# SamArgt/AudioSourceSep

Measured on AMD Instinct MI355X. Metric: Glow fwd+logdet passes/sec on 64×64×1 mel tiles (K=32,L=3), 1→8 MI355X, higher is better.
Workload: dtype f16x3

## Files before the change

__graft_entry__.py:

```python
import os
import subprocess
import sys

ROOT = os.path.dirname(os.path.abspath(__file__))
CSRC = os.path.join(ROOT, "audiosourcesep_amd", "csrc")
LIB = os.path.join(ROOT, "audiosourcesep_amd", "libglowk.so")


def _newer(target, sources):
    if not os.path.exists(target):
        return False
    t = os.path.getmtime(target)
    return all(os.path.getmtime(s) <= t for s in sources)


NET_SHAPES = [(ci, nf) for nf in (16, 12, 8, 4) for ci in (2, 4, 8, 16)]


def build(force=False, extra_flags=(), tag=None):
    from concurrent.futures import ThreadPoolExecutor
    hdr = os.path.join(ROOT, "include", "glowk.h")
    net_src = [os.path.join(CSRC, f) for f in ("glowk_act_scale.h", "glowk_kernels.h", "glowk_co.h", "glowk_q.h", "glowk_launch.h",
                                                "glowk_net_inst.hip")]
    eng_src = [os.path.join(CSRC, f) for f in sorted(os.listdir(CSRC)) if f.endswith((".hip", ".h")) and f != "glowk_net_inst.hip"] + [hdr]
    hipcc = os.environ.get("HIPCC", "/opt/rocm/bin/hipcc")
    objdir = os.path.join(CSRC, "_obj" + ("_" + tag if tag else ""))
    lib = LIB if not tag else LIB.replace("libglowk.so", "libglowk_%s.so" % tag)
    os.makedirs(objdir, exist_ok=True)
    flags = ["--offload-arch=gfx950", "-O3", "-std=c++17", "-fno-slp-vectorize", "-fPIC", "-pthread", "-Wno-unused-value"] + list(extra_flags)
    jobs, objs = [], []
    for unit in ("glowk", "glowk_training", "glowk_aux"):
        o = os.path.join(objdir, unit + ".o")
        objs.append(o)
        if force or not _newer(o, eng_src):
            jobs.append([hipcc] + flags + ["-c", os.path.join(CSRC, unit + ".hip"), "-o", o])
    for ci, nf in NET_SHAPES:
        o = os.path.join(objdir, "net_%d_%d.o" % (ci, nf))
        objs.append(o)
        if force or not _newer(o, net_src):
            jobs.append([hipcc] + flags + ["-DGLOWK_INST_CI=%d" % ci, "-DGLOWK_INST_NF=%d" % nf, "-c",
                                           os.path.join(CSRC, "glowk_net_inst.hip"), "-o", o])
    if jobs:
        workers = max(1, min(len(jobs), len(os.sched_getaffinity(0))))
        with ThreadPoolExecutor(workers) as pool:
            for r in pool.map(lambda c: subprocess.run(c, cwd=CSRC, capture_output=True, text=True), jobs):
                if r.returncode != 0:
                    sys.stderr.write(r.stderr)
                    raise RuntimeError("hipcc failed: " + " ".join(r.args[-4:]))
                if r.stderr.strip():
                    sys.stderr.write(r.stderr)
    if jobs or not _newer(lib, objs):
        subprocess.run([hipcc, "--offload-arch=gfx950", "-shared", "-fPIC", "-pthread"] + objs + ["-o", lib], check=True, cwd=CSRC)
    if tag:
        return lib
    if ROOT not in sys.path:
        sys.path.insert(0, ROOT)
    import audiosourcesep_amd
    from audiosourcesep_amd import _lib
    _lib.load()


def smoke():
    if ROOT not in sys.path:
        sys.path.insert(0, ROOT)
    import numpy as np
    import torch
    from audiosourcesep_amd.config import GlowConfig
    from audiosourcesep_amd.synthetic import calibrated_engine, synthetic_mel_tiles
    from oracle import glowref

    cfg = GlowConfig(H=16, W=16, C=1, L=2, K=2, F=128)
    eng, params = calibrated_engine(cfg, device=0)
    x = synthetic_mel_tiles(3, cfg)
    lp = eng.log_prob(torch.from_numpy(x).cuda()).cpu().numpy()
    ref = glowref.log_prob(x.astype(np.float64), glowref.cast_params(params, np.float64), cfg.as_dict())
    rel = np.max(np.abs(lp - ref) / np.abs(ref))
    print("smoke: log_prob", lp, "oracle", ref, "max rel err %.3e" % rel)
    assert rel < 1e-4, rel


if __name__ == "__main__":
    build()
    if len(sys.argv) > 1 and sys.argv[1] == "smoke":
        smoke()
```

audiosourcesep_amd/_lib.py:

```python
import ctypes
import os

_HERE = os.path.dirname(os.path.abspath(__file__))
LIB_PATH = os.environ.get("GLOWK_LIB") or os.path.join(_HERE, "libglowk.so")


class GlowkLibraryMissing(RuntimeError):
    pass


class GlowkError(RuntimeError):
    pass


class GlowkRangeError(GlowkError):
    """GLOWK_ERR_RANGE: a call in a split arithmetic (f16x3 / f16x2) left the fp16 range; its outputs are not usable."""


class GlowkConfigStruct(ctypes.Structure):
    _fields_ = [
        ("H", ctypes.c_int32), ("W", ctypes.c_int32), ("C", ctypes.c_int32),
        ("L", ctypes.c_int32), ("K", ctypes.c_int32), ("F", ctypes.c_int32),
        ("learntop", ctypes.c_int32), ("use_logit", ctypes.c_int32),
        ("minval", ctypes.c_float), ("maxval", ctypes.c_float), ("alpha", ctypes.c_float),
        ("bn_eps", ctypes.c_float),
    ]


class GlowkProfile(ctypes.Structure):
    _fields_ = [("net_ms", ctypes.c_double * 4), ("net_launches", ctypes.c_int64 * 4)]


STEP_TENSOR_IDS = {
    "actnorm/log_scale": 0, "actnorm/shift": 1,
    "inv1x1/P": 2, "inv1x1/sign_S": 3, "inv1x1/L": 4, "inv1x1/log_S": 5, "inv1x1/U": 6,
    "nn/conv1/kernel": 7, "nn/conv1/bias": 8,
    "nn/bn1/gamma": 9, "nn/bn1/beta": 10, "nn/bn1/mean": 11, "nn/bn1/var": 12,
    "nn/conv2/kernel": 13, "nn/conv2/bias": 14,
    "nn/bn2/gamma": 15, "nn/bn2/beta": 16, "nn/bn2/mean": 17, "nn/bn2/var": 18,
    "nn/conv3/kernel": 19, "nn/conv3/bias": 20,
    "inv1x1/P_inv": 21,
}
PRIOR_TENSOR_IDS = {"prior/loc": 100, "prior/log_scale": 101}
PREC_F32, PREC_F16X3, PREC_F16X2 = 0, 1, 2
OK, ERR, ERR_RANGE = 0, 1, 2
RANGE_IGNORE, RANGE_ERROR, RANGE_FALLBACK = 0, 1, 2
MIX_DB, MIX_MEAN = 0, 1

_vp, _i, _fp = ctypes.c_void_p, ctypes.c_int, ctypes.POINTER(ctypes.c_float)

SYMBOLS = {
    "glowk_version": (_i, []),
    "glowk_last_error": (ctypes.c_char_p, []),
    "glowk_reload_env": (None, []),
    "glowk_create": (_i, [ctypes.POINTER(GlowkConfigStruct), _i, ctypes.POINTER(_vp)]),
    "glowk_destroy": (_i, [_vp]),
    "glowk_tensor_size": (ctypes.c_size_t, [_vp, _i, _i]),
    "glowk_set_tensor": (_i, [_vp, _i, _i, _i, _fp, ctypes.c_size_t]),
    "glowk_get_tensor": (_i, [_vp, _i, _i, _i, _fp, ctypes.c_size_t]),
    "glowk_finalize_weights": (_i, [_vp]),
    "glowk_actnorm_data_init": (_i, [_vp, _vp, _i, _i, _i, _vp]),
    "glowk_set_precision": (_i, [_vp, _i]),
    "glowk_get_precision": (_i, [_vp]),
    "glowk_set_range_policy": (_i, [_vp, _i]),
    "glowk_get_range_policy": (_i, [_vp]),
    "glowk_range_status": (_i, [_vp, ctypes.POINTER(_i), ctypes.POINTER(ctypes.c_int64), _vp]),
    "glowk_range_probe_begin": (_i, [_vp]),
    "glowk_range_probe_end": (_i, [_vp, ctypes.POINTER(ctypes.c_float), ctypes.POINTER(ctypes.c_float), _vp]),
    "glowk_workspace_bytes": (ctypes.c_size_t, [_vp, _i, _i]),
    "glowk_reserve": (_i, [_vp, _i, _i]),
    "glowk_max_tiles": (_i, [_vp]),
    "glowk_forward": (_i, [_vp, _vp, _i, _vp, _vp, _vp]),
    "glowk_inverse": (_i, [_vp, _vp, _i, _vp, _vp]),
    "glowk_log_prob": (_i, [_vp, _vp, _i, _vp, _vp, _vp]),
    "glowk_log_prob_sum": (_i, [_vp, _vp, _i, _vp, _vp, _vp, _i, _vp]),
    "glowk_sum_f64": (_i, [_vp, ctypes.c_size_t, _vp, _i, ctypes.c_double, _vp]),
    "glowk_log_prob_grad": (_i, [_vp, _vp, _i, _vp, _vp, _vp]),
    "glowk_sample": (_i, [_vp, _vp, _i, _vp, _vp]),
    "glowk_prior_log_prob": (_i, [_vp, _vp, _i, _vp, _vp]),
    "glowk_fused_steps": (ctypes.c_int64, [_vp]),
    "glowk_kernel_families": (_i, [_vp, ctypes.POINTER(ctypes.c_int64)]),
    "glowk_profile_begin": (_i, [_vp]),
    "glowk_profile_end": (_i, [_vp, ctypes.POINTER(GlowkProfile)]),
    "glowk_squeeze": (_i, [_vp, _i, _i, _i, _i, _vp, _vp]),
    "glowk_unsqueeze": (_i, [_vp, _i, _i, _i, _i, _vp, _vp]),
    "glowk_preprocess_forward": (_i, [_vp, _vp, _i, _vp, _vp, _vp]),
    "glowk_preprocess_inverse": (_i, [_vp, _vp, _i, _vp, _vp]),
    "glowk_step_forward": (_i, [_vp, _i, _i, _vp, _i, _vp, _vp, _vp]),
    "glowk_step_inverse": (_i, [_vp, _i, _i, _vp, _i, _vp, _vp]),
    "glowk_coupling_net": (_i, [_vp, _i, _i, _vp, _i, _vp, _vp, _vp]),
    "glowk_param_vector_size": (ctypes.c_size_t, [_vp]),
    "glowk_param_offset": (_i, [_vp, _i, _i, _i, ctypes.POINTER(ctypes.c_size_t), ctypes.POINTER(ctypes.c_size_t)]),
    "glowk_param_grad": (_i, [_vp, _vp, _i, ctypes.c_float, _vp, _vp, _vp]),
    "glowk_apply_gradients": (_i, [_vp, _vp, _i, ctypes.c_float, _vp]),
    "glowk_crc32c": (ctypes.c_uint32, [_vp, ctypes.c_size_t]),
    "glowk_basis_update": (_i, [_vp, _vp, _vp, _vp, _vp, ctypes.c_size_t, ctypes.c_float, ctypes.c_float, _vp, _vp,
                                ctypes.c_uint64, ctypes.c_uint64, ctypes.c_uint64, _vp, _vp]),
    "glowk_basis_mix": (_i, [_vp, _vp, _vp, ctypes.c_size_t, _vp]),
    "glowk_basis_update_n": (_i, [_vp, _vp, _vp, _i, _vp, ctypes.c_size_t, _i, ctypes.c_float, ctypes.c_float,
                                  ctypes.c_uint64, ctypes.c_uint64, ctypes.c_uint64, _vp, _vp]),
    "glowk_basis_mix_n": (_i, [_vp, _i, _vp, ctypes.c_size_t, _i, _vp]),
    "glowk_random_source": (_i, [_vp, ctypes.c_size_t, ctypes.c_uint64, ctypes.c_uint64, _i, _i, _i, ctypes.c_uint64, _vp]),
    "glowk_random": (_i, [_vp, ctypes.c_size_t, ctypes.c_uint64, ctypes.c_uint64, _i, _i, ctypes.c_uint64, _vp]),
    "glowk_add_noise": (_i, [_vp, _vp, ctypes.c_size_t, ctypes.c_float, ctypes.c_uint64, ctypes.c_uint64, _i, ctypes.c_uint64, _vp]),
    "glowk_mel_filterbank": (_i, [_fp]),
    "glowk_mel_frontend": (_i, [_vp, _i, _i, ctypes.c_float, _vp, _vp, _vp]),
    "glowk_mel_to_power": (_i, [_vp, _i, _i, _i, _vp, _vp]),
    "glowk_masked_istft": (_i, [_vp, _i, _vp, _i, _i, _i, _vp, _vp]),
    "glowk_griffinlim": (_i, [_vp, _vp, _i, _i, _i, ctypes.c_float, _vp, _vp]),
    "glowk_resample_length": (ctypes.c_int64, [ctypes.c_int64, _i, _i]),
    "glowk_resample_filter": (_i, [ctypes.POINTER(ctypes.c_double)]),
    "glowk_resample": (_i, [_vp, _i, ctypes.c_int64, _i, _i, _vp, _vp]),
    "glowk_bss_xcorr":(_i, [_vp, _i, ctypes.c_int64, _vp, _i, ctypes.c_int64, _vp, _i, _i, _vp, _vp]),
    "glowk_bss_solve": (_i, [_vp, _i, _i, _i, _i, _i, _vp, _i, _vp, _vp, _vp]),
    "glowk_bss_project": (_i, [_vp, ctypes.c_int64, _i, _i, _i, _vp, _i, ctypes.c_int64, _vp, _i, _vp, _i, _vp, _vp]),
    "glowk_sp_stft": (_i, [_vp, _i, ctypes.c_int64, _vp, _vp]),
    "glowk_sp_istft": (_i, [_vp, _i, _i, ctypes.c_int64, _vp, _vp]),
    "glowk_oracle_mask": (_i, [_vp, _i, _i, _i, _i, ctypes.c_double, ctypes.c_double, _vp, _vp]),
    "glowk_mwf": (_i, [_vp, _i, _i, _vp]),
    "glowk_oracle_mel": (_i, [_vp, _vp, _i, ctypes.c_int64, _i, _i, ctypes.c_double, _vp, _vp]),
    "glowk_mwf_em": (_i, [_vp, _vp, _i, _i, _i, _i, _vp, _vp, _vp]),
}

_lib = None


def load():
    global _lib
    if _lib is not None:
        return _lib
    if not os.path.exists(LIB_PATH):
        raise GlowkLibraryMissing(
            "HIP library %s not found: build it first (python -c 'import __graft_entry__ as g; g.build()'). "
            "There is no CPU fallback for the compute path." % LIB_PATH)
    import torch
    lib = ctypes.CDLL(LIB_PATH)
    for name, (res, args) in SYMBOLS.items():
        fn = getattr(lib, name)
        fn.restype = res
        fn.argtypes = args
    _lib = lib
    return lib


def check(rc):
    if rc != 0:
        msg = load().glowk_last_error()
        raise (GlowkRangeError if rc == ERR_RANGE else GlowkError)(msg.decode() if msg else "glowk error %d" % rc)
```

audiosourcesep_amd/csrc/glowk.hip:

```cpp
#include "glowk_engine.h"
#include "glowk_light.h"

namespace glowk_eng {
thread_local std::string g_err;
}
using namespace glowk_eng;

namespace glowk_eng {

}

namespace glowk_detail {
int num_cus() {
  static int n = 0;
  if (n == 0) {
    int dev = 0; hipDeviceProp_t prop;
    if (hipGetDevice(&dev) == hipSuccess && hipGetDeviceProperties(&prop, dev) == hipSuccess) n = prop.multiProcessorCount;
    if (n <= 0) n = 256;
  }
  return n;
}
void launch_fail(const std::string& m) { fail(m); }
static EnvSwitches read_env() {
  auto on = [](const char* n) { return getenv(n) != nullptr; };
  return EnvSwitches{on("GLOWK_BWD_LIGHT_4"), on("GLOWK_NO_FUSE"), on("GLOWK_WGRAD_PLAIN"), on("GLOWK_CO_OFF"), on("GLOWK_Q_OFF"), on("GLOWK_CO_TRAIN_OFF"),
                     on("GLOWK_TRAIN_RECOMPUTE"), on("GLOWK_TRAIN_PERSTEP"), on("GLOWK_PG_JOIN")};
}
static EnvSwitches g_env = read_env();
const EnvSwitches& env() { return g_env; }
void reload_env() { g_env = read_env(); }
#define GLOWK_EXTERN_NET(CI_, NF_) extern template NetLaunch launch_net_t<CI_, NF_>(const NetArgs&, NetCall, hipStream_t, bool);
GLOWK_NET_SHAPES(GLOWK_EXTERN_NET)
#undef GLOWK_EXTERN_NET
}

namespace glowk_eng {
using glowk_detail::num_cus;
using glowk_detail::launch_net_t;

NetCall net_call(const glowk_handle* h, int dir, bool store, bool split) {
  if (h->precision == GLOWK_PREC_F32 || !split) return NetCall{dir, NET_EXACT, store};
  return NetCall{dir, h->precision == GLOWK_PREC_F16X2 && dir == NET_FWD && !store ? NET_SPLIT2 : NET_SPLIT3, store};
}

int* flagp(const glowk_handle* h) { return h->precision == GLOWK_PREC_F32 ? nullptr : h->d_flag; }

float bwd_norm_target(float xlim_b) {
  if (!(xlim_b >= 0.125f)) return 0.0f;
  int e = 0;
  std::frexp(xlim_b * 0.5f, &e);
  return std::ldexp(1.0f, std::min(e - 1, 10));
}

NetLaunch launch_net_raw(int c, int F, const NetArgs& a, NetCall call, hipStream_t s, bool dry) {
#define NETCASE(CI_, NF_) if (c == 2 * CI_ && F == 32 * NF_) return launch_net_t<CI_, NF_>(a, call, s, dry);
  GLOWK_NET_SHAPES(NETCASE)
#undef NETCASE
  return glowk_detail::net_failed("unsupported (channels, n_filters) combination: c=" + std::to_string(c) + " F=" + std::to_string(F));
}

int launch_net(glowk_handle* h, int level, int c, int F, const NetArgs& a, hipStream_t s, NetCall call, NetLaunch* out = nullptr) {
  if (h->profiling) {
    while (h->ev_pool.size() < h->ev_used + 2) {
      OwnedEvent e;
      HIPCHK(event_create(e, hipEventDefault));
      h->ev_pool.push_back(std::move(e));
    }
    HIPCHK(hipEventRecord(h->ev_pool[h->ev_used], s));
  }
  const NetLaunch r = launch_net_raw(c, F, a, call, s);
  if (!r.failed) {
    ++h->family_launches[r.family];
    if (r.co) ++h->family_launches[FAM_CO];
    if (r.q) ++h->family_launches[FAM_Q];
  }
  if (h->profiling) {
    HIPCHK(hipEventRecord(h->ev_pool[h->ev_used + 1], s));
    h->ev_used += 2;
    h->ev_level.push_back(level);
  }
  if (out) *out = r;
  return r.failed ? 1 : 0;
}


int launch_bwd_light(int c, const BwdArgs& a, int N, hipStream_t s) {
  const bool wide = c >= 8 && (a.Q + 15) / 16 <= 8 * num_cus() && !glowk_detail::env().bwd_light_4;
  auto al16 = [](const void* p) { return (reinterpret_cast<uintptr_t>(p) & 15) == 0; };
  const bool one = (a.Q + 255) / 256 >= 2 * num_cus() && al16(a.ghalf_in) && al16(a.v) && al16(a.osave) && al16(a.g_o) && al16(a.ghalf_out) &&
                   al16(a.gu_out) && al16(a.gv_out) && !glowk_detail::env().bwd_light_4;
  if (one) { CDISPATCH(c, hipLaunchKernelGGL((k_bwd_light<CC, 1>), dim3((a.Q + 255) / 256), dim3(256), 0, s, a)); }
  else if (wide) { CDISPATCH(c, hipLaunchKernelGGL((k_bwd_light<CC, 16>), dim3((a.Q + 15) / 16), dim3(256), 0, s, a)); }
  else { CDISPATCH(c, hipLaunchKernelGGL((k_bwd_light<CC, 4>), dim3((a.Q + 63) / 64), dim3(256), 0, s, a)); }
  LAUNCHCHK("k_bwd_light");
  return 0;
}

struct FlatLd { double* slot; int stride, base; };

int launch_couple(int c, const CoupleArgs& a, int N, hipStream_t s, const FlatLd* fl = nullptr, bool* flat_used = nullptr) {
  const int hw = a.h * a.w;
  if (N < 2 * num_cus() && hw % 64 == 0 && (!a.logdet || (fl && fl->slot))) {
    CoupleArgs b = a;
    b.logdet = nullptr;
    double* slots = a.logdet ? fl->slot : (double*)nullptr;
    const bool wide = c >= 8 && (a.Q + 15) / 16 <= 8 * num_cus();
    if (wide) { CDISPATCH(c, hipLaunchKernelGGL((k_couple_flat<CC, 16>), dim3((a.Q + 15) / 16), dim3(256), 0, s, b, slots, fl ? fl->stride : 0, fl ? fl->base : 0)); }
    else { CDISPATCH(c, hipLaunchKernelGGL((k_couple_flat<CC, 4>), dim3((a.Q + 63) / 64), dim3(256), 0, s, b, slots, fl ? fl->stride : 0, fl ? fl->base : 0)); }
    LAUNCHCHK("k_couple_flat");
    if (flat_used && a.logdet) *flat_used = true;
    return 0;
  }
  if (N >= 2 * num_cus()) {
    CDISPATCH(c, hipLaunchKernelGGL((k_couple<CC, false>), dim3(N), dim3(256), 0, s, a));
  } else {
    const int threads = hw >= 256 ? 1024 : hw > 64 ? 512 : 256;
    CDISPATCH(c, hipLaunchKernelGGL((k_couple<CC, true>), dim3(N), dim3(threads), 0, s, a));
  }
  LAUNCHCHK("k_couple");
  return 0;
}

bool fuse_geometry_ok(int h, int w, int pxw = 256) {
  const int hw = h * w;
  if (w < 4 || w > FUSE_EW || (w & (w - 1)) || pxw % w) return false;
  if (hw % pxw == 0) return true;
  return hw >= 32 && hw < pxw && (hw & (hw - 1)) == 0;
}

int net_and_couple(glowk_handle* h, int lvl, int c, int F, NetArgs na, CoupleArgs ca, int N, hipStream_t s, NetCall call, const FlatLd* fl = nullptr,
                   bool* flat_used = nullptr) {
  const bool no_fuse = glowk_detail::env().no_fuse;
  const bool fusable = call.arith != NET_EXACT && call.dir != NET_BWD && !call.store;
  const int hw = ca.h * ca.w;
  if (!no_fuse && c == 4 && fusable && na.RSp && ca.vin && !ca.log_s_out && ca.out && na.in_stride == 4 &&
      ca.out_stride % 4 == 0 && ca.out_off % 4 == 0 && fuse_geometry_ok(ca.h, ca.w) && na.P == h->bufP) {
    const size_t pxw = (na.co && fuse_geometry_ok(ca.h, ca.w, CO_PX)) ? CO_PX : 256;
    if (pxw == 256) na.co = 0;
    const size_t wgs = ((size_t)ca.Q + pxw - 1) / pxw;
    const size_t edge_floats = (wgs * 4 * FUSE_EW * 4 + 3) & ~(size_t)3;
    const size_t nld = wgs * (pxw / 32);
    if ((edge_floats + 2 * nld + 4) <= 4 * h->pstride) {
      na.fuse = 1;
      na.fz_b3 = ca.b3; na.fz_A = ca.A; na.fz_b = ca.b; na.fz_out = ca.out; na.fz_out_stride = ca.out_stride; na.fz_out_off = ca.out_off;
      na.fz_inverse = ca.inverse;
      na.fz_osave = ca.o_save;
      na.fz_edge = h->bufP;
      na.fz_ldpart = ca.logdet ? reinterpret_cast<double*>(h->bufP + edge_floats) : nullptr;
    }
  }
  NetLaunch r;
  if (int rc = launch_net(h, lvl, c, F, na, s, call, &r)) return rc;
  if (!r.fused_px) {
    ca.P = na.P; ca.np = r.np; ca.pstride = na.pstride;
    return launch_couple(c, ca, N, s, fl, flat_used);
  }
  ++h->fused_steps;
  const int pxw = r.fused_px;
  if (hw > pxw || ca.logdet) {
    EdgeArgs ea;
    ea.vin = ca.vin; ea.edge = na.fz_edge; ea.ldpart = na.fz_ldpart; ea.A = ca.A; ea.b = ca.b; ea.out = ca.out; ea.out_stride = ca.out_stride;
    ea.out_off = ca.out_off; ea.inverse = ca.inverse; ea.logdet = ca.logdet; ea.osave = ca.o_save; ea.h = ca.h; ea.w = ca.w; ea.flag = ca.flag; ea.pxw = pxw;
    hipLaunchKernelGGL(k_couple_edge, dim3(N), dim3(256), 0, s, ea);
    LAUNCHCHK("k_couple_edge");
  }
  return 0;
}

PreArgs pre_args(const glowk_config& cfg) {
  PreArgs p;
  p.minval = cfg.minval; p.maxval = cfg.maxval; p.alpha = cfg.alpha; p.use_logit = cfg.use_logit;
  return p;
}

struct WsSizes {
  size_t act, P, ld;
  size_t slots;
  size_t total() const { return 3 * act + P + ld + slots; }
};
int ld_slots_per_sample(const glowk_handle* h) {
  int n = 0;
  for (const Level& lv : h->levels) n += h->cfg.K * ((lv.h * lv.w + 15) / 16);
  return n;
}
WsSizes ws_sizes(const glowk_handle* h, size_t N) {
  const size_t E = (size_t)h->cfg.H * h->cfg.W * h->cfg.C;
  return WsSizes{N * E * 4, 4 * 9 * N * E * 4, N * 8, std::min(N, (size_t)2 * num_cus()) * ld_slots_per_sample(h) * 8};
}
size_t mask_blocks(const Level& lv, size_t Q) {
  const size_t b256 = ((Q + 255) / 256) * 8;
  if (lv.c == 32) return ((Q + 127) / 128) * 8;
  const size_t Qh = (size_t)256 * (size_t)(num_cus() / 8);
  return std::max(b256, ((std::min(Q, Qh) + 127) / 128) * 8);
}

struct SaveSizes {
  size_t v, p, m;
  int np;
  size_t gz, c;
  size_t total() const { return v * 4 + (size_t)np * p * 4 + m * 2 + gz + c; }
};
SaveSizes save_sizes(const glowk_handle* h, size_t N, std::vector<size_t>* offV = nullptr, std::vector<size_t>* offP = nullptr,
                     std::vector<size_t>* offM = nullptr) {
  const int K = h->cfg.K, L = h->cfg.L, NF = h->cfg.F / 32;
  SaveSizes S{0, 0, 0, 1, 0, 0};
  if (offV) { offV->assign((size_t)L * K, 0); offP->assign((size_t)L * K, 0); offM->assign((size_t)L * K, 0); }
  for (int lvl = 0; lvl < L; ++lvl) {
    const Level& lv = h->levels[lvl];
    const size_t Q = N * lv.h * lv.w;
    const size_t blocks = mask_blocks(lv, Q);
    for (int j = 0; j < K; ++j) {
      const size_t sidx = (size_t)lvl * K + j;
      if (offV) { (*offV)[sidx] = S.v; (*offP)[sidx] = S.p; (*offM)[sidx] = S.m; }
      S.v += Q * lv.c;
      S.p += Q * (lv.c / 2);
      S.m += 2 * blocks * NF * 64;
    }
  }
  const size_t E = (size_t)h->cfg.H * h->cfg.W * h->cfg.C;
  S.gz = N * E * 4;
  S.c = N * E * 4;
  return S;
}

int ensure_flag(glowk_handle* h) {
  if (h->d_flag) return 0;
  DeviceMem<int> d_flag;
  PinnedMem<int> h_flag;
  HIPCHK(dev_alloc(d_flag, 16));
  HIPCHK(hipMemset(d_flag, 0, 16));
  HIPCHK(pinned_alloc(h_flag, 16));
  h_flag[0] = 0;
  h->d_flag = std::move(d_flag);
  h->h_flag = std::move(h_flag);
  return 0;
}

int ensure_ws(glowk_handle* h, int N) {
  if (int rc = ensure_flag(h)) return rc;
  if (N <= h->wsN) return 0;
  HIPCHK(hipDeviceSynchronize());
  h->bufA.reset(); h->bufB.reset(); h->bufP.reset(); h->bufZ.reset(); h->bufLd.reset(); h->bufLdSlot.reset(); h->wsN = 0;
  const WsSizes W = ws_sizes(h, (size_t)N);
  HIPCHK(dev_alloc(h->bufA, W.act));
  HIPCHK(dev_alloc(h->bufB, W.act));
  h->pstride = W.P / 16;
  HIPCHK(dev_alloc(h->bufP, W.P));
  HIPCHK(dev_alloc(h->bufZ, W.act));
  HIPCHK(dev_alloc(h->bufLd, W.ld));
  HIPCHK(dev_alloc(h->bufLdSlot, W.slots));
  h->wsN = N;
  return 0;
}

int ensure_c(glowk_handle* h, int N) {
  if ((size_t)N <= h->cN) return 0;
  HIPCHK(hipDeviceSynchronize());
  h->bufC.reset(); h->cN = 0;
  HIPCHK(dev_alloc(h->bufC, (size_t)N * h->cfg.H * h->cfg.W * h->cfg.C * 4));
  h->cN = (size_t)N;
  return 0;
}

int max_tiles(const glowk_handle* h) {
  const long long E = (long long)h->cfg.H * h->cfg.W * h->cfg.C;
  const long long m = (1LL << 28) / E;
  return m < 1 ? 1 : (int)m;
}


int check_batch(const glowk_handle* h, int N) {
  if (N <= 0) return fail("batch size must be positive");
  if (N > max_tiles(h)) return fail("batch of " + std::to_string(N) + " tiles exceeds glowk_max_tiles() = " + std::to_string(max_tiles(h)) +
                                    " (32-bit indices within one call): split the batch");
  return 0;
}

int check_ready(glowk_handle* h, int N) {
  if (!h) return fail("null handle");
  if (h->finalized && h->split_stale && h->precision != GLOWK_PREC_F32)
    if (int rc = glowk_finalize_weights(h)) return rc;
  if (!h->finalized) return fail("glowk_finalize_weights has not been called");
  if (int rc = check_batch(h, N)) return rc;
  return ensure_ws(h, N);
}

NetArgs net_args(glowk_handle* h, const Level& lv, const StepDev& sd, const float* vin, int in_stride, int in_off, int N) {
  NetArgs a;
  a.vin = vin; a.in_stride = in_stride; a.in_off = in_off;
  a.Q = N * lv.h * lv.w; a.h = lv.h; a.w = lv.w;
  a.K1p = sd.K1p; a.ep = sd.ep; a.R0p = sd.R0p; a.mask1 = nullptr; a.mask2 = nullptr; a.P = h->bufP;
  a.RHp = sd.RHp; a.RSp = sd.RSp; a.fam16 = (sd.RSp && sd.RSBp) ? 1 : 0; a.eph = sd.epH; a.pstride = h->pstride; a.max_np = 4; a.sc1 = sd.sc1; a.sc2 = sd.sc2; a.sc3 = sd.sc3;
  a.flag = flagp(h); a.xlim = sd.xlim_f; a.st1 = nullptr; a.st2 = nullptr;
  a.bnorm = 1.0f;
  a.fuse = 0; a.co = glowk_detail::env().co_off ? 0 : 1; a.fz_osave = nullptr; a.fz_b3 = nullptr; a.fz_A = nullptr; a.fz_b = nullptr; a.fz_out = nullptr; a.fz_out_stride = 0; a.fz_out_off = 0; a.fz_inverse = 0;
  a.fz_edge = nullptr; a.fz_ldpart = nullptr;
  a.pad = nullptr;
  a.xmax_out = h->d_probe ? h->d_probe + ((&lv - h->levels.data()) * h->cfg.K + (&sd - lv.dev.data())) : nullptr;
  return a;
}

int ensure_save(glowk_handle* h, int N) {
  if (int rc = ensure_c(h, N)) return rc;
  if (N <= h->saveN) return 0;
  const int Na = std::max(N, h->saveN);
// ... 602 lines not shown
  std::vector<float> v((size_t)2 * LK);
  HIPCHK(hipStreamSynchronize((hipStream_t)stream));
  HIPCHK(hipMemcpy(v.data(), h->d_probe, v.size() * sizeof(float), hipMemcpyDeviceToHost));
  h->d_probe.reset();
  float rf = 0.f, rb = 0.f;
  for (int l = 0; l < h->cfg.L; ++l)
    for (int k = 0; k < h->cfg.K; ++k) {
      const StepDev& sd = h->levels[l].dev[k];
      const int i = l * h->cfg.K + k;
      if (sd.xlim_f > 0.f) rf = std::max(rf, v[i] / sd.xlim_f);
      if (sd.xlim_b > 0.f && v[LK + i] > 0.f) rb = std::max(rb, 0.125f / sd.xlim_b);
    }
  if (fwd_ratio) *fwd_ratio = rf;
  if (bwd_ratio) *bwd_ratio = rb;
  return 0;
}

size_t glowk_workspace_bytes(const glowk_handle* h, int N, int with_grad) {
  if (!h || N <= 0) return 0;
  size_t b = ws_sizes(h, (size_t)N).total() + 16 ;
  if (with_grad) b += save_sizes(h, (size_t)N).total();
  return b;
}

int glowk_max_tiles(const glowk_handle* h) { return h ? max_tiles(h) : 0; }

int glowk_reserve(glowk_handle* h, int N, int with_grad) {
  if (!h) return fail("null handle");
  DeviceGuard dg(h->device);
  if (int rc = check_batch(h, N)) return rc;
  if (int rc = ensure_ws(h, N)) return rc;
  if (with_grad) {
    if (!h->finalized) return fail("glowk_finalize_weights must run before reserving the gradient path (its size depends on the launch policy)");
    return ensure_save(h, N);
  }
  return 0;
}

int glowk_forward(glowk_handle* h, const float* x_dev, int N, float* z_dev, float* logdet_dev, void* stream) {
  if (!h) return fail("null handle");
  DeviceGuard dg(h->device);
  if (int rc = check_ready(h, N)) return rc;
  if (!x_dev || !z_dev) return fail("null tensor");
  hipStream_t s = (hipStream_t)stream;
  return guarded(h, s, [&]() -> int {
    if (int rc = run_forward(h, x_dev, N, z_dev, s)) return rc;
    if (logdet_dev) {
      hipLaunchKernelGGL(k_prior, dim3(N), dim3(256), 0, s, (const float*)nullptr, 0, (const float*)nullptr, (const float*)nullptr,
                         (const double*)h->bufLd, (float*)nullptr, logdet_dev);
      LAUNCHCHK("k_prior(logdet)");
    }
    return 0;
  });
}

int glowk_inverse(glowk_handle* h, const float* z_dev, int N, float* x_dev, void* stream) {
  if (!h) return fail("null handle");
  DeviceGuard dg(h->device);
  if (int rc = check_ready(h, N)) return rc;
  if (!x_dev || !z_dev) return fail("null tensor");
  hipStream_t s = (hipStream_t)stream;
  return guarded(h, s, [&]() -> int { return run_inverse(h, z_dev, N, x_dev, s); });
}

int glowk_log_prob(glowk_handle* h, const float* x_dev, int N, float* logp_dev, float* z_dev, void* stream) {
  if (!h) return fail("null handle");
  DeviceGuard dg(h->device);
  if (int rc = check_ready(h, N)) return rc;
  if (!x_dev || !logp_dev) return fail("null tensor");
  hipStream_t s = (hipStream_t)stream;
  float* z = z_dev ? z_dev : h->bufZ;
  return guarded(h, s, [&]() -> int {
    if (int rc = run_forward(h, x_dev, N, z, s)) return rc;
    hipLaunchKernelGGL(k_prior, dim3(N), dim3(256), 0, s, (const float*)z, h->Hl * h->Wl * h->Cl, h->d_loc, h->d_log_scale,
                       (const double*)h->bufLd, logp_dev, (float*)nullptr);
    LAUNCHCHK("k_prior");
    return 0;
  });
}

int glowk_log_prob_sum(glowk_handle* h, const float* x_dev, int N, float* logp_dev, float* z_dev, double* sum_dev, int accumulate, void* stream) {
  if (!h) return fail("null handle");
  DeviceGuard dg(h->device);
  if (int rc = check_ready(h, N)) return rc;
  if (!x_dev || !logp_dev || !sum_dev) return fail("null tensor");
  hipStream_t s = (hipStream_t)stream;
  float* z = z_dev ? z_dev : h->bufZ;
  const int rc = guarded(h, s, [&]() -> int {
    if (int rc = run_forward(h, x_dev, N, z, s)) return rc;
    hipLaunchKernelGGL(k_prior, dim3(N), dim3(256), 0, s, (const float*)z, h->Hl * h->Wl * h->Cl, h->d_loc, h->d_log_scale,
                       (const double*)h->bufLd, logp_dev, (float*)nullptr);
    LAUNCHCHK("k_prior");
    return 0;
  });
  if (rc) return rc;
  hipLaunchKernelGGL(k_sum_f64, dim3(1), dim3(1024), 0, s, (const float*)logp_dev, (size_t)N, sum_dev, accumulate, 1.0);
  LAUNCHCHK("k_sum_f64");
  return 0;
}

int glowk_sum_f64(const float* v_dev, size_t n, double* out_dev, int accumulate, double scale, void* stream) {
  if (!out_dev || (!v_dev && n)) return fail("null tensor");
  DeviceGuard dg(ptr_device(out_dev));
  hipLaunchKernelGGL(k_sum_f64, dim3(1), dim3(1024), 0, (hipStream_t)stream, v_dev, n, out_dev, accumulate, scale);
  LAUNCHCHK("k_sum_f64");
  return 0;
}

int glowk_log_prob_grad(glowk_handle* h, const float* x_dev, int N, float* logp_dev, float* dx_dev, void* stream) {
  if (!h) return fail("null handle");
  DeviceGuard dg(h->device);
  if (int rc = check_ready(h, N)) return rc;
  if (!x_dev || !logp_dev || !dx_dev) return fail("null tensor");
  if (int rc = ensure_save(h, N)) return rc;
  hipStream_t s = (hipStream_t)stream;
  float* z = h->bufGz;
  return guarded(h, s, [&]() -> int {
    if (int rc = run_forward(h, x_dev, N, z, s, true)) return rc;
    hipLaunchKernelGGL(k_prior, dim3(N), dim3(256), 0, s, (const float*)z, h->Hl * h->Wl * h->Cl, h->d_loc, h->d_log_scale,
                       (const double*)h->bufLd, logp_dev, (float*)nullptr);
    LAUNCHCHK("k_prior");
    return run_backward(h, x_dev, z, N, dx_dev, s);
  });
}

int glowk_sample(glowk_handle* h, const float* eps_dev, int N, float* x_dev, void* stream) {
  if (!h) return fail("null handle");
  DeviceGuard dg(h->device);
  if (int rc = check_ready(h, N)) return rc;
  if (!eps_dev || !x_dev) return fail("null tensor");
  hipStream_t s = (hipStream_t)stream;
  const int E = h->Hl * h->Wl * h->Cl;
  const size_t total = (size_t)N * E;
  return guarded(h, s, [&]() -> int {
    hipLaunchKernelGGL(k_prior_sample, dim3((unsigned)((total + 255) / 256)), dim3(256), 0, s, eps_dev, total, E, h->d_loc, h->d_log_scale,
                       h->bufZ);
    LAUNCHCHK("k_prior_sample");
    return run_inverse(h, h->bufZ, N, x_dev, s);
  });
}

int glowk_prior_log_prob(glowk_handle* h, const float* z_dev, int N, float* logp_dev, void* stream) {
  if (!h) return fail("null handle");
  DeviceGuard dg(h->device);
  if (int rc = check_ready(h, N)) return rc;
  if (!z_dev || !logp_dev) return fail("null tensor");
  hipLaunchKernelGGL(k_prior, dim3(N), dim3(256), 0, (hipStream_t)stream, z_dev, h->Hl * h->Wl * h->Cl, h->d_loc, h->d_log_scale,
                     (const double*)nullptr, logp_dev, (float*)nullptr);
  LAUNCHCHK("k_prior");
  return 0;
}

int64_t glowk_fused_steps(const glowk_handle* h) { return h ? h->fused_steps : -1; }

int glowk_kernel_families(const glowk_handle* h, int64_t* out7) {
  if (!h || !out7) return fail("null argument");
  for (int i = 0; i < FAM_COUNT; ++i) out7[i] = h->family_launches[i];
  return 0;
}

int glowk_profile_begin(glowk_handle* h) {
  if (!h) return fail("null handle");
  h->profiling = true;
  h->ev_used = 0;
  h->ev_level.clear();
  return 0;
}

int glowk_profile_end(glowk_handle* h, glowk_profile* out) {
  if (!h || !out) return fail("null argument");
  std::memset(out, 0, sizeof(*out));
  h->profiling = false;
  DeviceGuard dg(h->device);
  HIPCHK(hipDeviceSynchronize());
  for (size_t i = 0; i < h->ev_level.size(); ++i) {
    float ms = 0.0f;
    HIPCHK(hipEventElapsedTime(&ms, h->ev_pool[2 * i], h->ev_pool[2 * i + 1]));
    const int l = h->ev_level[i];
    if (l >= 0 && l < 4) { out->net_ms[l] += ms; out->net_launches[l] += 1; }
  }
  h->ev_used = 0;
  h->ev_level.clear();
  return 0;
}

int glowk_squeeze(const float* x_dev, int N, int H, int W, int C, float* y_dev, void* stream) {
  if (!x_dev || !y_dev) return fail("null tensor");
  if (N <= 0 || H <= 0 || W <= 0 || H % 2 || W % 2) return fail("squeeze needs even H and W");
  if ((long long)N * H * W * C > (1LL << 28)) return fail("squeeze: more than 2^28 elements in one call; split the batch");
  DeviceGuard dg(ptr_device(x_dev));
  PreArgs p = {0, 1, 0, 0};
  const int c = 4 * C;
  CDISPATCH(c, hipLaunchKernelGGL((k_in<CC>), dim3(N), dim3(256), 0, (hipStream_t)stream, x_dev, H, W, p, 0, (const float*)nullptr,
                                  (const float*)nullptr, y_dev, (double*)nullptr, 0.0));
  LAUNCHCHK("k_in(squeeze)");
  return 0;
}

int glowk_unsqueeze(const float* y_dev, int N, int hh, int ww, int c4, float* x_dev, void* stream) {
  if (!x_dev || !y_dev) return fail("null tensor");
  if (N <= 0 || hh <= 0 || ww <= 0 || c4 % 4) return fail("unsqueeze needs a channel count divisible by 4");
  if ((long long)N * hh * ww * c4 > (1LL << 28)) return fail("unsqueeze: more than 2^28 elements in one call; split the batch");
  DeviceGuard dg(ptr_device(y_dev));
  PreArgs p = {0, 1, 0, 0};
  CDISPATCH(c4, hipLaunchKernelGGL((k_out<CC>), dim3(N), dim3(256), 0, (hipStream_t)stream, y_dev, hh, ww, p, 0, x_dev));
  LAUNCHCHK("k_out(unsqueeze)");
  return 0;
}

int glowk_preprocess_forward(glowk_handle* h, const float* x_dev, int N, float* y_dev, float* logdet_dev, void* stream) {
  if (!h || !x_dev || !y_dev) return fail("null argument");
  DeviceGuard dg(h->device);
  if (int rc = check_batch(h, N)) return rc;
  const int E = h->cfg.H * h->cfg.W * h->cfg.C;
  double ldc = -(double)E * std::log((double)h->cfg.maxval - (double)h->cfg.minval);
  if (h->cfg.use_logit) ldc += (double)E * std::log(1.0 - 2.0 * (double)h->cfg.alpha);
  hipLaunchKernelGGL(k_pre_only, dim3(N), dim3(256), 0, (hipStream_t)stream, x_dev, E, pre_args(h->cfg), 0, y_dev, logdet_dev, ldc);
  LAUNCHCHK("k_pre_only");
  return 0;
}

int glowk_preprocess_inverse(glowk_handle* h, const float* y_dev, int N, float* x_dev, void* stream) {
  if (!h || !x_dev || !y_dev) return fail("null argument");
  DeviceGuard dg(h->device);
  if (int rc = check_batch(h, N)) return rc;
  const int E = h->cfg.H * h->cfg.W * h->cfg.C;
  hipLaunchKernelGGL(k_pre_only, dim3(N), dim3(256), 0, (hipStream_t)stream, y_dev, E, pre_args(h->cfg), 1, x_dev, (float*)nullptr, 0.0);
  LAUNCHCHK("k_pre_only");
  return 0;
}

int glowk_step_forward(glowk_handle* h, int level, int step, const float* u_dev, int N, float* y_dev, float* logdet_dev, void* stream) {
  if (!h) return fail("null handle");
  DeviceGuard dg(h->device);
  if (int rc = check_ready(h, N)) return rc;
  if (level < 0 || level >= h->cfg.L || step < 0 || step >= h->cfg.K) return fail("no such step");
  if (!u_dev || !y_dev) return fail("null tensor");
  hipStream_t s = (hipStream_t)stream;
  const Level& lv = h->levels[level];
  const StepDev& sd = lv.dev[step];
  const int Q = N * lv.h * lv.w;
  return guarded(h, s, [&]() -> int {
    CDISPATCH(lv.c, hipLaunchKernelGGL((k_affine<CC>), dim3((Q + 255) / 256), dim3(256), 0, s, u_dev, Q, sd.Afwd, sd.bfwd, h->bufA));
    LAUNCHCHK("k_affine");
    NetLaunch r;
    if (int rc = launch_net(h, level, lv.c, h->cfg.F, net_args(h, lv, sd, h->bufA, lv.c, lv.c / 2, N), s, net_call(h, NET_FWD), &r)) return rc;
    if (logdet_dev) {
      std::vector<double> init(N, h->ld_step[(size_t)level * h->cfg.K + step]);
      HIPCHK(hipMemcpyAsync(h->bufLd, init.data(), (size_t)N * 8, hipMemcpyHostToDevice, s));
      HIPCHK(hipStreamSynchronize(s));
    }
    CoupleArgs ca;
    ca.o_save = nullptr;
    ca.vin = h->bufA; ca.P = h->bufP; ca.np = r.np; ca.pstride = h->pstride; ca.b3 = sd.b3; ca.A = nullptr; ca.b = nullptr;
    ca.out = y_dev; ca.out_stride = lv.c; ca.out_off = 0;
    ca.logdet = logdet_dev ? h->bufLd : nullptr; ca.log_s_out = nullptr; ca.t_out = nullptr;
    ca.Q = Q; ca.h = lv.h; ca.w = lv.w; ca.inverse = 0; ca.flag = flagp(h);
    if (int rc = launch_couple(lv.c, ca, N, s)) return rc;
    if (logdet_dev) {
      hipLaunchKernelGGL(k_prior, dim3(N), dim3(256), 0, s, (const float*)nullptr, 0, (const float*)nullptr, (const float*)nullptr,
                         (const double*)h->bufLd, (float*)nullptr, logdet_dev);
      LAUNCHCHK("k_prior(logdet)");
    }
    return 0;
  });
}

int glowk_step_inverse(glowk_handle* h, int level, int step, const float* y_dev, int N, float* u_dev, void* stream) {
  if (!h) return fail("null handle");
  DeviceGuard dg(h->device);
  if (int rc = check_ready(h, N)) return rc;
  if (level < 0 || level >= h->cfg.L || step < 0 || step >= h->cfg.K) return fail("no such step");
  if (!u_dev || !y_dev) return fail("null tensor");
  hipStream_t s = (hipStream_t)stream;
  const Level& lv = h->levels[level];
  const StepDev& sd = lv.dev[step];
  return guarded(h, s, [&]() -> int {
    NetLaunch r;
    if (int rc = launch_net(h, level, lv.c, h->cfg.F, net_args(h, lv, sd, y_dev, lv.c, lv.c / 2, N), s, net_call(h, NET_FWD), &r)) return rc;
    CoupleArgs ca;
    ca.o_save = nullptr;
    ca.vin = y_dev; ca.P = h->bufP; ca.np = r.np; ca.pstride = h->pstride; ca.b3 = sd.b3; ca.A = sd.Ainv; ca.b = sd.binv;
    ca.out = u_dev; ca.out_stride = lv.c; ca.out_off = 0;
    ca.logdet = nullptr; ca.log_s_out = nullptr; ca.t_out = nullptr;
    ca.Q = N * lv.h * lv.w; ca.h = lv.h; ca.w = lv.w; ca.inverse = 1; ca.flag = flagp(h);
    return launch_couple(lv.c, ca, N, s);
  });
}

int glowk_coupling_net(glowk_handle* h, int level, int step, const float* xb_dev, int N, float* log_s_dev, float* t_dev, void* stream) {
  if (!h) return fail("null handle");
  DeviceGuard dg(h->device);
  if (int rc = check_ready(h, N)) return rc;
  if (level < 0 || level >= h->cfg.L || step < 0 || step >= h->cfg.K) return fail("no such step");
  if (!xb_dev || !log_s_dev || !t_dev) return fail("null tensor");
  hipStream_t s = (hipStream_t)stream;
  const Level& lv = h->levels[level];
  const StepDev& sd = lv.dev[step];
  return guarded(h, s, [&]() -> int {
    NetLaunch r;
    if (int rc = launch_net(h, level, lv.c, h->cfg.F, net_args(h, lv, sd, xb_dev, lv.c / 2, 0, N), s, net_call(h, NET_FWD), &r)) return rc;
    CoupleArgs ca;
    ca.o_save = nullptr;
    ca.vin = nullptr; ca.P = h->bufP; ca.np = r.np; ca.pstride = h->pstride; ca.b3 = sd.b3; ca.A = nullptr; ca.b = nullptr;
    ca.out = nullptr; ca.out_stride = 0; ca.out_off = 0;
    ca.logdet = nullptr; ca.log_s_out = log_s_dev; ca.t_out = t_dev;
// ... 8 lines not shown
```

audiosourcesep_amd/csrc/glowk_engine.h:

```cpp
#pragma once
#include "../../include/glowk.h"
#include "glowk_kernels.h"
#include "glowk_pack.h"
#include "glowk_launch.h"

#include <algorithm>
#include <atomic>
#include <cmath>
#include <cstdio>
#include <cstdlib>
#include <cstring>
#include <sched.h>
#include <string>
#include <thread>
#include <vector>

namespace glowk_eng {

extern thread_local std::string g_err;

inline int fail(const std::string& m) {
  g_err = m;
  return GLOWK_ERR;
}

struct DeviceGuard {
  int prev = -1;
  bool changed = false;
  explicit DeviceGuard(int dev) {
    if (hipGetDevice(&prev) == hipSuccess && prev != dev) changed = hipSetDevice(dev) == hipSuccess;
  }
  ~DeviceGuard() {
    if (changed) (void)hipSetDevice(prev);
  }
  DeviceGuard(const DeviceGuard&) = delete;
  DeviceGuard& operator=(const DeviceGuard&) = delete;
};

#define HIPCHK(expr)                                                                           \
  do {                                                                                         \
    hipError_t e_ = (expr);                                                                    \
    if (e_ != hipSuccess) return glowk_eng::fail(std::string(#expr) + ": " + hipGetErrorString(e_));      \
  } while (0)

#define LAUNCHCHK(name)                                                                        \
  do {                                                                                         \
    hipError_t e_ = hipGetLastError();                                                         \
    if (e_ != hipSuccess) return glowk_eng::fail(std::string("launch ") + name + ": " + hipGetErrorString(e_)); \
  } while (0)

template <class T, class Release>
class Owner {
 public:
  Owner() = default;
  explicit Owner(Release r) : r_(r) {}
  Owner(Owner&& o) noexcept : p_(o.release()), r_(o.r_) {}
  Owner& operator=(Owner&& o) noexcept { reset(o.release()); r_ = o.r_; return *this; }
  ~Owner() { reset(); }
  operator T() const { return p_; }
  const Release& releaser() const { return r_; }
  T release() { T p = p_; p_ = nullptr; return p; }
  void reset(T p = nullptr) { if (p_) r_(p_); p_ = p; }
 private:
  T p_ = nullptr;
  Release r_{};
};
struct HipFree { void operator()(void* p) const { (void)hipFree(p); } };
struct HipHostFree { void operator()(void* p) const { (void)hipHostFree(p); } };
struct HipFreeAsync { hipStream_t s; void operator()(void* p) const { (void)hipFreeAsync(p, s); } };
struct HipStreamDestroy { void operator()(hipStream_t s) const { (void)hipStreamDestroy(s); } };
struct HipEventDestroy { void operator()(hipEvent_t e) const { (void)hipEventDestroy(e); } };
template <class T> using DeviceMem = Owner<T*, HipFree>;
template <class T> using PinnedMem = Owner<T*, HipHostFree>;
template <class T> using Scratch = Owner<T*, HipFreeAsync>;
using OwnedStream = Owner<hipStream_t, HipStreamDestroy>;
using OwnedEvent = Owner<hipEvent_t, HipEventDestroy>;

template <class T, class R, class Create>
hipError_t create_into(Owner<T, R>& o, Create create) {
  o.reset();
  T p = nullptr;
  const hipError_t e = create(&p);
  if (e == hipSuccess) o.reset(p);
  return e;
}
template <class T> hipError_t dev_alloc(DeviceMem<T>& o, size_t bytes) { return create_into(o, [&](T** p) { return hipMalloc(p, bytes); }); }
template <class T> hipError_t pinned_alloc(PinnedMem<T>& o, size_t bytes) { return create_into(o, [&](T** p) { return hipHostMalloc(p, bytes); }); }
template <class T> hipError_t scratch_alloc(Scratch<T>& o, size_t bytes) {
  return create_into(o, [&](T** p) { return hipMallocAsync(reinterpret_cast<void**>(p), bytes, o.releaser().s); });
}
inline hipError_t stream_create(OwnedStream& o) { return create_into(o, [](hipStream_t* s) { return hipStreamCreateWithFlags(s, hipStreamNonBlocking); }); }
inline hipError_t event_create(OwnedEvent& o, unsigned flags) { return create_into(o, [&](hipEvent_t* e) { return hipEventCreateWithFlags(e, flags); }); }

}
using glowk_eng::DeviceMem; using glowk_eng::PinnedMem; using glowk_eng::OwnedStream; using glowk_eng::OwnedEvent;

struct glowk_handle {
  glowk_config cfg;
  int device = 0;
  int precision = GLOWK_PREC_F32;
  int range_policy = GLOWK_RANGE_ERROR;
  int64_t range_fallbacks = 0;
  int64_t family_launches[FAM_COUNT] = {};
  int64_t fused_steps = 0;
  DeviceMem<int> d_flag;
  PinnedMem<int> h_flag;
  DeviceMem<unsigned> d_probe;
  std::vector<Level> levels;
  int Hl = 0, Wl = 0, Cl = 0;
  std::vector<float> prior_loc, prior_log_scale;
  bool finalized = false;
  double ld_const = 0.0;
  double ld_pre_const = 0.0;
  std::vector<double> ld_step;
  DeviceMem<float> arena;
  const float* d_loc = nullptr;
  const float* d_log_scale = nullptr;
  int wsN = 0;
  DeviceMem<float> bufA, bufB, bufP, bufZ, bufC;
  size_t pstride = 0;
  DeviceMem<double> bufLd;
  DeviceMem<double> bufLdSlot;
  DeviceMem<double> bufStat;
  int saveN = 0;
  size_t cN = 0;
  DeviceMem<float> saveV, saveP, bufGz;
  DeviceMem<unsigned short> saveM;
  std::vector<size_t> offV, offP, offM;
  bool tr_active = false;
  bool host_stale = false;
  bool split_stale = false;
  DeviceMem<float> tr_params, tr_m, tr_v;
  size_t tr_n = 0;
  long tr_t = 0;
  std::vector<size_t> tr_level_off;
  size_t tr_prior_off = 0;
  std::vector<DeviceMem<int>> tr_map;
  std::vector<size_t> tr_map_n;
  std::vector<DeviceMem<int>> tr_map16;
  std::vector<size_t> tr_map16_n;
  DeviceMem<float> tr16_src;
  DeviceMem<int> tr16_S;
  DeviceMem<float> tr16_scales;
  size_t tr16_src_max = 0;
  PinnedMem<float> tr_pinned;
  std::vector<size_t> tr_pin_off;
  std::vector<OwnedStream> tr_streams;
  std::vector<OwnedEvent> tr_events;
  std::vector<float> tr_bfac;
  DeviceMem<unsigned> tr_gmax;
  PinnedMem<float> h_gmax;
  OwnedStream tr_side;
  OwnedEvent tr_ev_sums, tr_ev_up;
  PinnedMem<double> h_sums;
  PinnedMem<float> h_up;
  int trN = 0;
  DeviceMem<float> trR1, trM1, trM2, trXcol, trGcol, trCpart, trC1, trC2, trC3, trGv, trGo;
  int trNB = 1;
  DeviceMem<double> trAffPart, trAffSum;
  DeviceMem<float> trKeep;
  std::vector<size_t> trKeepOff;
  int trKeepN = 0;
  bool profiling = false;
  std::vector<OwnedEvent> ev_pool;
  size_t ev_used = 0;
  std::vector<int> ev_level;
};

#define CDISPATCH(c, CALL)                                                                     \
  switch (c) {                                                                                 \
    case 4: { constexpr int CC = 4; CALL; } break;                                             \
    case 8: { constexpr int CC = 8; CALL; } break;                                             \
    case 16: { constexpr int CC = 16; CALL; } break;                                           \
    case 32: { constexpr int CC = 32; CALL; } break;                                           \
    default: return glowk_eng::fail("unsupported channel count " + std::to_string(c));         \
  }

namespace glowk_eng {

struct TrainCtx {
  float* grad;
  float scale;
  bool split;
  hipEvent_t sums_ready = nullptr;
};

int check_ready(glowk_handle* h, int N);
int ensure_save(glowk_handle* h, int N);
NetArgs net_args(glowk_handle* h, const Level& lv, const StepDev& sd, const float* vin, int in_stride, int in_off, int N);
NetCall net_call(const glowk_handle* h, int dir, bool store = false, bool split = true);
NetLaunch launch_net_raw(int c, int F, const NetArgs& a, NetCall call, hipStream_t s, bool dry = false);
int run_forward(glowk_handle* h, const float* x, int N, float* z_dst, hipStream_t s, bool save = false, bool keep_hidden = false);
int run_backward(glowk_handle* h, const float* x, const float* z, int N, float* dx, hipStream_t s, TrainCtx* tc = nullptr);
int launch_prior(glowk_handle* h, const float* z, int N, float* logp_dev, hipStream_t s);
int ptr_device(const void* p);

int sync_host(glowk_handle* h);
int train_network_grads(glowk_handle* h, TrainCtx* tc, int lvl, int k0, int nb, const float* v, ptrdiff_t v_bs, const float* g_o, ptrdiff_t go_bs,
                        const float* R1, ptrdiff_t r_bs, const float* M1, const float* M2, ptrdiff_t m_bs, int N, hipStream_t s, float bfac = 1.0f);
int train_affine_sums(glowk_handle* h, int lvl, int k0, int nb, const float* v, ptrdiff_t v_bs, const float* gv, ptrdiff_t gv_bs, int N, hipStream_t s);

}
```

audiosourcesep_amd/csrc/glowk_kernels.h:

```cpp
#pragma once
#include "glowk_act_scale.h"

#include <hip/hip_runtime.h>
#include <utility>
#include <stdint.h>

typedef float f32x16 __attribute__((ext_vector_type(16)));

#define GLOWK_GPTR(p) ((const __attribute__((address_space(1))) void*)(p))
#define GLOWK_LPTR(p) ((__attribute__((address_space(3))) void*)(p))

__device__ __forceinline__ int mfma_row(int r, int hh) { return (r & 3) + 8 * (r >> 2) + 4 * hh; }

struct NetArgs {
  const float* vin;
  int in_stride, in_off;
  int Q, h, w;
  const float* K1p;
  const float* ep;
  const float4* R0p;
  unsigned short* mask1;
  unsigned short* mask2;
  float* P;
  size_t pstride;
  int max_np;
  const float4* RHp;
  const float* eph;
  const float4* RSp;
  int fam16;
  float sc1, sc2, sc3;
  int* flag;
  float xlim;
  float bnorm;
  int fuse;
  int co;
  const float* fz_b3;
  const float* fz_A;
  const float* fz_b;
  float* fz_out;
  int fz_out_stride, fz_out_off, fz_inverse;
  float* fz_osave;
  float* fz_edge;
  double* fz_ldpart;
  unsigned* xmax_out;
  float* st1;
  float* st2;
  void* pad;
};

#define GLOWK_ST_MOD " nt"
__device__ __forceinline__ void st_tile_planar(float* blk_base, unsigned lane_byte, unsigned row_bytes, const f32x16& v) {
  const unsigned long long base = reinterpret_cast<unsigned long long>(blk_base);
  unsigned off = lane_byte;
#pragma unroll
  for (int r = 0; r < 16; ++r) {
    asm volatile("global_store_dword %0, %1, %2" GLOWK_ST_MOD ::"v"(off), "v"(v[r]), "s"(base) : "memory");
    off += ((r & 3) == 3 ? 5u : 1u) * row_bytes;
  }
}

template <int C>
__device__ __forceinline__ void affine_cc(const float* __restrict__ A, const float* __restrict__ b, const float (&x)[C], float (&y)[C]) {
#pragma unroll
  for (int co = 0; co < C; ++co) y[co] = b[co];
#pragma unroll
  for (int ci = 0; ci < C; ++ci)
#pragma unroll
    for (int co = 0; co < C; ++co) y[co] = fmaf(x[ci], A[ci * C + co], y[co]);
}

__device__ __forceinline__ void glds16(const float4* src_lane, float4* lds_wave_base) {
  __builtin_amdgcn_global_load_lds(GLOWK_GPTR(src_lane), GLOWK_LPTR(lds_wave_base), 16, 0, 0);
}

__device__ __forceinline__ float* uniform_fptr(float* p) {
  const unsigned long long b = reinterpret_cast<unsigned long long>(p);
  const unsigned lo = __builtin_amdgcn_readfirstlane((unsigned)b);
  const unsigned hi = __builtin_amdgcn_readfirstlane((unsigned)(b >> 32));
  return reinterpret_cast<float*>(((unsigned long long)hi << 32) | lo);
}
__device__ __forceinline__ const char* uniform_ptr(const void* p) {
  const unsigned long long b = reinterpret_cast<unsigned long long>(p);
  const unsigned lo = __builtin_amdgcn_readfirstlane((unsigned)b);
  const unsigned hi = __builtin_amdgcn_readfirstlane((unsigned)(b >> 32));
  return reinterpret_cast<const char*>(((unsigned long long)hi << 32) | lo);
}

template <int P>
__device__ __forceinline__ float4* ring_slot(float4* s0, float4* s1) { return P ? s1 : s0; }

template <int KIN, int NF>
struct Ring1 {
  static constexpr int KS1 = (9 * KIN) / 2;
  static constexpr int MAIN4 = NF * 256;
  static constexpr int K1PIECES_FULL = (KS1 * 256 + 1023) / 1024;
  static constexpr bool K1_IN_RING = (size_t)2 * (MAIN4 + K1PIECES_FULL * 64) * 16 + (size_t)6 * NF * 32 * 4 <= 160 * 1024;
  static constexpr int K1PIECES = K1_IN_RING ? K1PIECES_FULL : 0;
  static constexpr bool K1_IN_BUF = !K1_IN_RING && (size_t)2 * MAIN4 * 16 + (size_t)6 * NF * 32 * 4 + (size_t)K1PIECES_FULL * 1024 <= 160 * 1024;
  static constexpr int K1HALF_KS = KS1 / 2;
  static constexpr int K1HALF_PIECES = (K1HALF_KS * 256 + 1023) / 1024;
  static constexpr bool K1_IN_HALF = !K1_IN_RING && !K1_IN_BUF && KS1 % 2 == 0 && (K1HALF_KS * 256) % 1024 == 0 &&
                                     (size_t)2 * MAIN4 * 16 + (size_t)6 * NF * 32 * 4 + (size_t)K1HALF_PIECES * 1024 <= 160 * 1024;
  static constexpr int K1BUF4 = K1_IN_BUF ? K1PIECES_FULL * 64 : K1_IN_HALF ? K1HALF_PIECES * 64 : 1;
  static constexpr int SLOT4 = MAIN4 + K1PIECES * 64;
  static constexpr int PIECES = NF * 4 + K1PIECES;
  static constexpr size_t LDS_BYTES = (size_t)2 * SLOT4 * 16 + (size_t)6 * NF * 32 * 4 + ((K1_IN_BUF || K1_IN_HALF) ? (size_t)K1BUF4 * 16 : 0);
  static constexpr bool FITS = LDS_BYTES <= 160 * 1024;
};

template <int P0, int N>
__device__ __forceinline__ void stage_range(const float4* __restrict__ src, float4* dst, int wave, unsigned voff) {
  const char* gb = uniform_ptr(src);
#pragma unroll
  for (int i = 0; i < (N + 3) / 4; ++i) {
    int p = i * 4 + wave;
    p = P0 + (p < N ? p : N - 1);
    glds16(reinterpret_cast<const float4*>(gb + (size_t)p * 1024 + voff), dst + p * 64);
  }
}

enum { NET_FWD = 0, NET_FWD_SAVE = 1, NET_BWD = 2,
       NET_FWD2 = 3 };
constexpr int NET_STORE = 8;
constexpr int NET_FUSE = 16;
constexpr int NET_HALF = 32;
template <int MODE>
constexpr int net_dir = MODE & 7;

template <int N>
__device__ __forceinline__ unsigned pick_word(const unsigned (&w)[N], int j) {
  unsigned r = 0;
#pragma unroll
  for (int i = 0; i < N; ++i) r = (j == i) ? w[i] : r;
  return r;
}

template <int KIN, int NF, int P, int MODE, bool STORE>
__device__ __forceinline__ void net_step(const NetArgs& a, int fi, bool first, const float4* nsrc, float4* s0, float4* s1, float4* k1buf,
                                         const float* epl, const float (&xcol)[(9 * KIN) / 2], f32x16 (&acc2)[NF],
                                         const unsigned (&mk)[NF / 2], size_t wblk, int wave, unsigned voff, int lane, int hh, int q, bool qok, bool wok) {
  using G = Ring1<KIN, NF>;
  constexpr int KS1 = G::KS1;
  constexpr int F = NF * 32;
  f32x16 h1;
#pragma unroll
  for (int r = 0; r < 16; ++r) h1[r] = 0.0f;
  if constexpr (G::K1_IN_HALF) {
    constexpr int KH = G::K1HALF_KS;
    if (!first) {
      asm volatile("s_waitcnt vmcnt(0)" ::: "memory");
      __syncthreads();
    }
    const float* k1 = reinterpret_cast<const float*>(k1buf) + lane;
#pragma unroll
    for (int ks = 0; ks < KH; ++ks) h1 = __builtin_amdgcn_mfma_f32_32x32x2f32(k1[ks * 64], xcol[ks], h1, 0, 0, 0);
    __syncthreads();
    stage_range<0, G::K1HALF_PIECES>(reinterpret_cast<const float4*>(a.K1p + ((size_t)fi * KS1 + KH) * 64), k1buf, wave, voff);
    asm volatile("s_waitcnt vmcnt(0)" ::: "memory");
    __syncthreads();
#pragma unroll
    for (int ks = 0; ks < KH; ++ks) h1 = __builtin_amdgcn_mfma_f32_32x32x2f32(k1[ks * 64], xcol[KH + ks], h1, 0, 0, 0);
  } else {
    if (G::K1_IN_BUF && !first) {
      asm volatile("s_waitcnt vmcnt(0)" ::: "memory");
      __syncthreads();
    }
    const float* k1 = G::K1_IN_RING ? reinterpret_cast<const float*>(ring_slot<P ^ 1>(s0, s1) + G::MAIN4) + lane
                      : G::K1_IN_BUF ? reinterpret_cast<const float*>(k1buf) + lane
                                     : a.K1p + (size_t)fi * KS1 * 64 + lane;
#pragma unroll
    for (int ks = 0; ks < KS1; ++ks) h1 = __builtin_amdgcn_mfma_f32_32x32x2f32(k1[ks * 64], xcol[ks], h1, 0, 0, 0);
  }
  float* st_blk = STORE ? uniform_fptr(a.st1 + (size_t)fi * 32 * a.Q) : nullptr;
  const unsigned st_lane = STORE ? ((unsigned)(4 * hh) * (unsigned)a.Q + (unsigned)q) * 4u : 0u;
  const unsigned st_row = (unsigned)a.Q * 4u;
  if (MODE == NET_BWD) {
    const unsigned w = pick_word<NF / 2>(mk, fi >> 1) >> ((fi & 1) * 16);
#pragma unroll
    for (int r = 0; r < 16; ++r) h1[r] = ((w >> r) & 1u) ? h1[r] : 0.0f;
    if (STORE && qok) st_tile_planar(st_blk, st_lane, st_row, h1);
#pragma unroll
    for (int r = 0; r < 16; ++r) h1[r] *= epl[4 * F + fi * 32 + mfma_row(r, hh)];
  } else {
    unsigned bits = 0;
#pragma unroll
    for (int r = 0; r < 16; ++r) {
      const int f = fi * 32 + mfma_row(r, hh);
      const float pre = h1[r] + epl[f];
      if (MODE == NET_FWD_SAVE) bits |= (pre > 0.0f ? 1u : 0u) << r;
      h1[r] = fmaxf(pre, 0.0f);
    }
    if (STORE && qok) st_tile_planar(st_blk, st_lane, st_row, h1);
#pragma unroll
    for (int r = 0; r < 16; ++r) {
      const int f = fi * 32 + mfma_row(r, hh);
      h1[r] = fmaf(epl[F + f], h1[r], epl[2 * F + f]);
    }
    if (MODE == NET_FWD_SAVE) a.mask1[(wblk * NF + fi) * 64 + lane] = (unsigned short)bits;
  }
  {
    constexpr int NST = (STORE ? 16 : 0) + (MODE == NET_FWD_SAVE ? 1 : 0);
    if (!first || G::K1_IN_BUF) {
      if (NST && wok) asm volatile("s_waitcnt vmcnt(%0)" ::"n"(NST) : "memory");
      else asm volatile("s_waitcnt vmcnt(0)" ::: "memory");
    }
    __syncthreads();
  }
  stage_range<0, G::PIECES>(nsrc, ring_slot<P ^ 1>(s0, s1), wave, voff);
  if (G::K1_IN_BUF && fi + 1 < NF)
    stage_range<0, G::K1PIECES_FULL>(reinterpret_cast<const float4*>(a.K1p + (size_t)(fi + 1) * KS1 * 64), k1buf, wave, voff);
  if constexpr (G::K1_IN_HALF) {
    if (fi + 1 < NF) stage_range<0, G::K1HALF_PIECES>(reinterpret_cast<const float4*>(a.K1p + (size_t)(fi + 1) * KS1 * 64), k1buf, wave, voff);
  }
  const float4* buf = ring_slot<P>(s0, s1);
#pragma unroll
  for (int r = 0; r < 16; ++r) {
#pragma unroll
    for (int g = 0; g < NF / 4; ++g) {
      const float4 wv = buf[(r * (NF / 4) + g) * 64 + lane];
      acc2[4 * g + 0] = __builtin_amdgcn_mfma_f32_32x32x2f32(wv.x, h1[r], acc2[4 * g + 0], 0, 0, 0);
      acc2[4 * g + 1] = __builtin_amdgcn_mfma_f32_32x32x2f32(wv.y, h1[r], acc2[4 * g + 1], 0, 0, 0);
      acc2[4 * g + 2] = __builtin_amdgcn_mfma_f32_32x32x2f32(wv.z, h1[r], acc2[4 * g + 2], 0, 0, 0);
      acc2[4 * g + 3] = __builtin_amdgcn_mfma_f32_32x32x2f32(wv.w, h1[r], acc2[4 * g + 3], 0, 0, 0);
    }
  }
}

template <int KIN, int MOUT, int NF, int MODE, bool STORE = false>
__global__ __launch_bounds__(256, 1) void k_net_f32(NetArgs a) {
  using G = Ring1<KIN, NF>;
  constexpr int KS1 = G::KS1;
  constexpr int NMT = (MOUT + 31) / 32;
  constexpr int F = NF * 32;
  constexpr int SLOT4 = G::SLOT4;
  constexpr int SGN = (MODE == NET_BWD) ? -1 : 1;
  static_assert(KIN % 2 == 0 && NF % 4 == 0 && G::FITS, "shape");

  __shared__ float4 slot0[SLOT4];
  __shared__ float4 slot1[SLOT4];
  __shared__ float epl[6 * F];
  __shared__ float4 k1buf[G::K1BUF4];

  const int tid = threadIdx.x;
  const int lane = tid & 63;
  const int wave = __builtin_amdgcn_readfirstlane(tid >> 6);
  const unsigned voff = (unsigned)lane * 16u;
  const int pix = lane & 31;
  const int hh = lane >> 5;
  const size_t wblk = (size_t)blockIdx.x * 4 + (tid >> 6);
  const int q = (int)wblk * 32 + pix;
  const bool qok = q < a.Q;
  const bool wok = (long)(blockIdx.x * 4 + wave) * 32 < a.Q;
  const float4* ring = a.R0p;

  float xcol[KS1];
  {
    const int hw = a.h * a.w;
    const int qq = qok ? q : 0;
    const int rem = qq % hw;
    const int i = rem / a.w, j = rem % a.w;
    const float* base = a.vin + (long)qq * a.in_stride + a.in_off;
#pragma unroll
    for (int ks = 0; ks < KS1; ++ks) {
      const int k = 2 * ks + hh;
      const int tap = k / KIN, cin = k % KIN;
      const int dy = SGN * (tap / 3 - 1), dx = SGN * (tap % 3 - 1);
      const int ii = i + dy, jj = j + dx;
      const bool ok = qok && ii >= 0 && ii < a.h && jj >= 0 && jj < a.w;
      const int off = ok ? ((dy * a.w + dx) * a.in_stride + cin) : 0;
      const float v = base[off];
      xcol[ks] = ok ? v : 0.0f;
    }
  }
  unsigned mk1[NF / 2], mk2[NF / 2];
#pragma unroll
  for (int j = 0; j < NF / 2; ++j) { mk1[j] = 0; mk2[j] = 0; }
  if (MODE == NET_BWD) {
#pragma unroll
// ... 475 lines not shown
                                        const h8 (&xh)[(RingH<KIN, MOUT, NF, MODE, NP>::KS)], const h8 (&xl)[(RingH<KIN, MOUT, NF, MODE, NP>::KS)],
                                        int g, int q, bool qok, int lane, int hh) {
  using G = RingH<KIN, MOUT, NF, MODE, NP>;
  constexpr int NFH = G::NFH, NMT = G::NMT;
  constexpr int f2base = PASS * NFH * 32;
  f32x16 acc2[NFH];
#pragma unroll
  for (int fo = 0; fo < NFH; ++fo)
#pragma unroll
    for (int r = 0; r < 16; ++r) acc2[fo][r] = net_dir<MODE> == NET_BWD ? 0.0f : epl[f2base + fo * 32 + mfma_row(r, hh)];

  h8 bh[2], bl[2];
#pragma nounroll
  for (int i0 = 0; i0 < NF; i0 += 2) {
    h3_X<KIN, MOUT, NF, MODE, NP, 0, PASS>(a, c, i0, xh, xl, lane, bh, bl);
    h3_x_end<MODE, PASS>(c);
    if (PASS >= 1 && !SOLO && NMT == 1 && i0 == 0 && !g)
      stage4<G::MAINP, 50>(G::out_chunk(c.img, PASS, 0), c.sD, c.w4, c.voff);
    h3_Y<KIN, MOUT, NF, MODE, NP, 1>(P0 ? c.sB : c.sA, bh, bl, acc2, lane, g, true, G::main_chunk(c.img, PASS, i0 + 1), P0 ? c.sA : c.sB,
                                     c.k1img + (size_t)((i0 + 2) % NF) * G::K14, c.k1s0, c.w4, c.voff);
    h3_barrier();
    h3_X<KIN, MOUT, NF, MODE, NP, 1, PASS>(a, c, i0 + 1, xh, xl, lane, bh, bl);
    h3_x_end<MODE, PASS>(c);
    h3_Y<KIN, MOUT, NF, MODE, NP, 2>(P0 ? c.sA : c.sB, bh, bl, acc2, lane, g, i0 + 2 < NF || NMT >= 2,
                                     i0 + 2 < NF ? G::main_chunk(c.img, PASS, i0 + 2) : G::out_chunk(c.img, PASS, 1), P0 ? c.sB : c.sA,
                                     c.k1img + (size_t)((i0 + 3) % NF) * G::K14, c.k1s1, c.w4, c.voff);
    h3_barrier();
  }

  f32x16 acc3[G::G0N];
  h3_tail<KIN, MOUT, NF, MODE, NP, P0, PASS, SOLO>(a, c, epl, acc2, acc3, bh, bl, g, q, qok, lane, hh, std::make_integer_sequence<int, 2 * NMT>());
}

template <int KIN, int MOUT, int NF, int MODE, int NP, int PASS, int P0>
__device__ __forceinline__ void h3_passes(const NetArgs& a, const H3Ctx& c, const float* epl,
                                          const h8 (&xh)[(RingH<KIN, MOUT, NF, MODE, NP>::KS)], const h8 (&xl)[(RingH<KIN, MOUT, NF, MODE, NP>::KS)],
                                          int g, int q, bool qok, int lane, int hh) {
  h3_pass<KIN, MOUT, NF, MODE, NP, P0, PASS, false>(a, c, epl, xh, xl, g, q, qok, lane, hh);
  if constexpr (PASS + 1 < NP)
    h3_passes<KIN, MOUT, NF, MODE, NP, PASS + 1, (RingH<KIN, MOUT, NF, MODE, NP>::NMT + 1 + P0) & 1>(a, c, epl, xh, xl, g, q, qok, lane, hh);
}

template <int KIN, int MOUT, int NF, int MODE, int NP, bool SPLIT>
__global__ __launch_bounds__(512, 2) void k_net_h3(NetArgs a) {
  using G = RingH<KIN, MOUT, NF, MODE, NP>;
  constexpr int K1 = G::K1;
  constexpr int KS = G::KS;
  constexpr int SGN = (net_dir<MODE> == NET_BWD) ? -1 : 1;
  static_assert(G::FITS, "shape");

  __shared__ float4 slotA[G::MAIN4];
  __shared__ float4 slotB[G::MAIN4];
  __shared__ float4 slotD[G::MAIN4];
  __shared__ float4 k1slot0[G::K14];
  __shared__ float4 k1slot1[G::K14];
  __shared__ float epl[G::EPN];
  __shared__ __attribute__((aligned(16))) unsigned short mkl[G::MASK2B / 2 + 8];

  const int tid = threadIdx.x;
  const int lane = tid & 63;
  const int wave = __builtin_amdgcn_readfirstlane(tid >> 6);
  const int g = wave >> 2;
  const int pix = lane & 31;
  const int hh = lane >> 5;
  const int q = (blockIdx.x * 8 + (tid >> 6)) * 32 + pix;
  const bool qok = q < a.Q;

  H3Ctx c;
  c.sA = slotA; c.sB = slotB; c.sD = slotD; c.k1s0 = k1slot0; c.k1s1 = k1slot1;
  c.k1img = a.RHp;
  const int solo_pass = SPLIT ? (int)blockIdx.y : 0;
  c.img = a.RHp;
  c.mkl = mkl;
  c.wblk = (size_t)blockIdx.x * 8 + wave;
  c.wok = (long)c.wblk * 32 < a.Q;
  c.w4 = wave & 3;
  c.voff = (unsigned)lane * 16u;
  c.ub[0] = c.ub[1] = 1.0f;

  if (!g) {
    stage4<G::MAINP, 60>(G::main_chunk(c.img, solo_pass, 0), slotA, c.w4, c.voff);
    stage4<G::MAINP, 61>(G::out_chunk(c.img, solo_pass, 0), slotD, c.w4, c.voff);
    if (net_dir<MODE> == NET_BWD)
      stage4<NF, 64>(reinterpret_cast<const float4*>(a.mask1 + (size_t)blockIdx.x * 8 * NF * 64), reinterpret_cast<float4*>(mkl), c.w4, c.voff);
  } else {
    stage4<G::K1P, 62>(c.k1img, k1slot0, c.w4, c.voff);
    stage4<G::K1P, 63>(c.k1img + G::K14, k1slot1, c.w4, c.voff);
    if (net_dir<MODE> == NET_BWD)
      stage4<NF, 65>(reinterpret_cast<const float4*>(a.mask2 + (size_t)blockIdx.x * 8 * NF * 64), reinterpret_cast<float4*>(mkl + 8 * NF * 64), c.w4, c.voff);
  }
  h8 xh[KS], xl[KS];
  float xmax = 0.0f;
  {
    const int hw = a.h * a.w;
    const int qq = qok ? q : 0;
    const int rem = qq % hw;
    const int i = rem / a.w, j0 = rem % a.w;
    const float* base = a.vin + (long)qq * a.in_stride + a.in_off;
    if constexpr (net_dir<MODE> == NET_BWD) {
      float v[KS][8];
#pragma unroll
      for (int s = 0; s < KS; ++s) {
        gather8<KIN, false, SGN>(base, i, j0, a.h, a.w, a.in_stride, qok, 16 * s + 8 * hh, v[s]);
        xmax = range8(xmax, v[s]);
      }
      xmax = nan_max(xmax, __shfl_xor(xmax, 32, 64));
      const float fac = (MODE & NET_STORE) ? 1.0f : pixel_norm(xmax, a.bnorm, c.ub[0]);
#pragma unroll
      for (int s = 0; s < KS; ++s) {
#pragma unroll
        for (int j = 0; j < 8; ++j) v[s][j] *= fac;
        split8(v[s], xh[s], xl[s]);
      }
    } else {
#pragma unroll
      for (int s = 0; s < KS; ++s) {
        float v[8];
        gather8<KIN, true, SGN>(base, i, j0, a.h, a.w, a.in_stride, qok, 16 * s + 8 * hh, v);
        xmax = range8(xmax, v);
        split8(v, xh[s], xl[s]);
      }
    }
  }
  if (net_dir<MODE> != NET_BWD)
    for (int i = tid; i < G::EPN; i += 512) epl[i] = a.eph[i];
  if (((net_dir<MODE> == NET_BWD && !(MODE & NET_STORE)) ? !(xmax <= 3.0e38f) : !(xmax <= a.xlim)) && a.flag) *a.flag = 1;
  if (a.xmax_out) range_probe(a.xmax_out, xmax);
  asm volatile("s_waitcnt vmcnt(0)" ::: "memory");
  __syncthreads();

  if (g) h3_barrier();
  if constexpr (SPLIT) {
    if (solo_pass == 0) h3_pass<KIN, MOUT, NF, MODE, NP, 0, 0, true>(a, c, epl, xh, xl, g, q, qok, lane, hh);
    else if (solo_pass == 1) h3_pass<KIN, MOUT, NF, MODE, NP, 0, 1, true>(a, c, epl, xh, xl, g, q, qok, lane, hh);
    else if constexpr (NP > 2) {
      if (solo_pass == 2) h3_pass<KIN, MOUT, NF, MODE, NP, 0, 2, true>(a, c, epl, xh, xl, g, q, qok, lane, hh);
      else h3_pass<KIN, MOUT, NF, MODE, NP, 0, 3, true>(a, c, epl, xh, xl, g, q, qok, lane, hh);
    }
  } else {
    h3_passes<KIN, MOUT, NF, MODE, NP, 0, 0>(a, c, epl, xh, xl, g, q, qok, lane, hh);
  }
  if (!g) h3_barrier();
}

typedef float f32x4 __attribute__((ext_vector_type(4)));

constexpr int FUSE_PSTR = 260;
constexpr int FUSE_EW = 64;

template <int KIN, int MOUT, int NF, int MODE, int NP>
struct RingS {
  static constexpr bool BWD = net_dir<MODE> == NET_BWD;
  static constexpr bool FUSE = (MODE & NET_FUSE) != 0;
  static constexpr int PXH = (MODE & NET_HALF) ? 1 : 2;
  static constexpr int NFH = NF / NP;
  static constexpr int NRB = 2 * NFH;
  static constexpr int K1 = 9 * KIN;
  static constexpr int KS = (K1 + (BWD ? 0 : 1) + 31) / 32;
  static constexpr int MAINP = NRB * 2;
  static constexpr int MAIN4 = MAINP * 64;
  static constexpr int K1P = KS * 4;
  static constexpr int K14 = K1P * 64;
  static constexpr bool STK = !BWD && glowk_conv1_stacked(K1);
  static constexpr int KSX = STK ? glowk_conv1_ks_stacked(K1) : KS;
  static constexpr int M3 = MOUT;
  static constexpr int NMT = (M3 + 15) / 16;
  static constexpr int TPC = MAINP / 2;
  static constexpr int NT = NFH * NMT;
  static constexpr int NCH = (NT + TPC - 1) / TPC;
  static constexpr int G0N = NMT < 6 ? NMT : 6;
  static constexpr int NGRP = (NMT + 5) / 6;
  static constexpr int GT = NFH * 6;
  static constexpr int grp_n(int gi) { return NMT - 6 * gi < 6 ? NMT - 6 * gi : 6; }
  static constexpr int EPN = (NF * 32 + 16 * NMT + 3) & ~3;
  static constexpr int MASK2B = BWD ? 2 * NF * 512 * 2 : 0;
  static constexpr size_t LDS_BYTES = (size_t)3 * MAIN4 * 16 + (size_t)2 * K14 * 16 + (size_t)EPN * 4 + MASK2B;
  static constexpr bool FITS = LDS_BYTES <= 160 * 1024 && NF % 4 == 0 && NFH >= 2 && KS <= (PXH == 1 ? (NP == 2 ? 5 : 9) : NP == 2 ? 3 : 5) && NGRP <= 3 &&
                               (NGRP == 1 || GT % TPC == 0) &&
                               (!FUSE || (MOUT == 36 && NP == 2 && PXH == 2 && LDS_BYTES + (size_t)36 * FUSE_PSTR * 4 + 4096 + 128 <= 160 * 1024));
  static constexpr int K1TOT4 = NF * K14;
  static constexpr int IMGH = NF / 2;
  static constexpr int IMG_MAIN4 = IMGH * 256;
  static constexpr int IMG_NCH = (IMGH * NMT + 2 * IMGH - 1) / (2 * IMGH);
  static constexpr int IMG_PASS4 = (NF + IMG_NCH) * IMG_MAIN4;
  static constexpr int SUBS = NP / 2;
  __device__ static const float4* main_chunk(const float4* img, int pass, int ch) {
    return img + K1TOT4 + (size_t)(pass / SUBS) * IMG_PASS4 + (size_t)ch * IMG_MAIN4 + (size_t)(pass % SUBS) * MAIN4;
  }
  __device__ static const float4* out_chunk(const float4* img, int pass, int s) {
    const int sub = pass % SUBS, t4 = s * TPC;
    const int gi = t4 / GT;
    const int t2 = IMGH * 6 * gi + sub * NFH * grp_n(gi) + (t4 - GT * gi);
    return img + K1TOT4 + (size_t)(pass / SUBS) * IMG_PASS4 + (size_t)NF * IMG_MAIN4 + (size_t)t2 * 128;
  }
  static constexpr int tile_fo(int t) { return (t - GT * (t / GT)) / grp_n(t / GT); }
  static constexpr int tile_mt(int t) { return 6 * (t / GT) + (t - GT * (t / GT)) % grp_n(t / GT); }
  static constexpr bool MERGE = PXH == 2 && NP == 2 && NGRP == 1 && NMT <= 3 &&
                                (net_dir<MODE> == NET_FWD || net_dir<MODE> == NET_FWD2 || (net_dir<MODE> == NET_BWD && NMT <= 2) || (net_dir<MODE> == NET_FWD_SAVE && FUSE));
};

template <bool TWO = false>
__device__ __forceinline__ f32x4 mfma3s(const h8& ahi, const h8& alo, const h8& bhi, const h8& blo, f32x4 acc) {
  acc = __builtin_amdgcn_mfma_f32_16x16x32_f16(alo, bhi, acc, 0, 0, 0);
  if (!TWO) acc = __builtin_amdgcn_mfma_f32_16x16x32_f16(ahi, blo, acc, 0, 0, 0);
  acc = __builtin_amdgcn_mfma_f32_16x16x32_f16(ahi, bhi, acc, 0, 0, 0);
  return acc;
}

template <int MODE>
__device__ __forceinline__ unsigned h3s_act_vals(const f32x4& r0, const f32x4& r1, float sc, unsigned mask8, float (&v)[8]) {
  unsigned bits = 0;
#pragma unroll
  for (int j = 0; j < 8; j += 2) {
    const f32x2 a2 = j < 4 ? f32x2{r0[j], r0[j + 1]} : f32x2{r1[j - 4], r1[j - 3]};
    const f32x2 t2 = a2 * f32x2{sc, sc};
    const float t[2] = {t2.x, t2.y}, av[2] = {a2.x, a2.y};
#pragma unroll
    for (int e = 0; e < 2; ++e) {
      if (MODE == NET_BWD) v[j + e] = __int_as_float(__float_as_int(t[e]) & __builtin_amdgcn_sbfe((int)mask8, j + e, 1));
      else {
        v[j + e] = fmaxf(t[e], 0.0f);
        if (MODE == NET_FWD_SAVE) bits |= (av[e] > 0.0f ? 1u : 0u) << (j + e);
      }
    }
  }
  return bits;
}
template <int MODE, bool ST = false>
__device__ __forceinline__ unsigned h3s_act(const f32x4& r0, const f32x4& r1, float sc, unsigned mask8, h8& bh, h8& bl, bool do_st = false,
                                            float* st_blk = nullptr, unsigned st_lane = 0, unsigned st_row = 0) {
  float v[8];
  const unsigned bits = h3s_act_vals<MODE>(r0, r1, sc, mask8, v);
  if constexpr (ST) {
    if (do_st) {
      const unsigned long long st_base = reinterpret_cast<unsigned long long>(st_blk);
#pragma unroll
      for (int j = 0; j < 8; ++j) {
        const unsigned off = st_lane + (unsigned)((j >> 2) * 16 + (j & 3)) * st_row;
        asm volatile("global_store_dword %0, %1, %2" GLOWK_ST_MOD ::"v"(off), "v"(v[j]), "s"(st_base) : "memory");
      }
    }
  }
  if (MODE == NET_FWD2) {
#pragma unroll
    for (int j = 0; j < 8; ++j) { bh[j] = (_Float16)v[j]; bl[j] = (_Float16)0.0f; }
  } else split8(v, bh, bl);
  return bits;
}
template <int MODE, bool ST>
__device__ __forceinline__ unsigned h3s_act_pair(const f32x4& r00, const f32x4& r10, const f32x4& r01, const f32x4& r11, float sc, unsigned mask16,
                                                 h8 (&bh)[2], h8 (&bl)[2], float* st_blk, unsigned st_lane, unsigned st_row) {
  float v0[8], v1[8];
  unsigned bits = h3s_act_vals<MODE>(r00, r10, sc, mask16, v0);
  bits |= h3s_act_vals<MODE>(r01, r11, sc, mask16 >> 8, v1) << 8;
  if constexpr (ST) {
    const unsigned long long st_base = reinterpret_cast<unsigned long long>(st_blk);
#pragma unroll
    for (int j = 0; j < 8; ++j) {
      const unsigned off = st_lane + (unsigned)((j >> 2) * 16 + (j & 3)) * st_row;
      const f32x2 pr = {v0[j], v1[j]};
      asm volatile("global_store_dwordx2 %0, %1, %2" GLOWK_ST_MOD ::"v"(off), "v"(pr), "s"(st_base) : "memory");
    }
  }
  split8(v0, bh[0], bl[0]);
  split8(v1, bh[1], bl[1]);
  return bits;
}

template <int KIN, int MOUT, int NF, int MODE, int NP, int KP, int PASS, bool PAIR = false>
__device__ __forceinline__ void h3s_X(const NetArgs& a, const H3Ctx& c, int fi, const h8 (&xh)[(RingS<KIN, MOUT, NF, MODE, NP>::KS)][2],
                                      const h8 (&xl)[(RingS<KIN, MOUT, NF, MODE, NP>::KS)][2], int lane, h8 (&bh)[2], h8 (&bl)[2]) {
  using G = RingS<KIN, MOUT, NF, MODE, NP>;
  unsigned mask = 0;
  if (net_dir<MODE> == NET_BWD) mask = c.mkl[c.mk2off + ((size_t)(threadIdx.x >> 6) * NF + fi) * 64 + lane];
  f32x4 h1[2][2];
#pragma unroll
  for (int i = 0; i < 4; ++i)
#pragma unroll
    for (int r = 0; r < 4; ++r) h1[i >> 1][i & 1][r] = 0.0f;
  const h8* k1 = reinterpret_cast<const h8*>(KP ? c.k1s1 : c.k1s0) + lane;
  if constexpr (G::STK) {
    static_assert(G::KSX <= 6, "operand reads in flight");
    h8 kf[G::KSX * 2];
#pragma unroll
    for (int i = 0; i < G::KSX * 2; ++i) kf[i] = k1[i * 64];
    __builtin_amdgcn_sched_barrier(0);
#pragma unroll
    for (int s = 0; s < G::KSX; ++s)
#pragma unroll
      for (int rb = 0; rb < 2; ++rb)
#pragma unroll
        for (int hf = 0; hf < G::PXH; ++hf)
          h1[rb][hf] = __builtin_amdgcn_mfma_f32_16x16x32_f16(kf[s * 2 + rb], x_frag(xh, xl, s, hf), h1[rb][hf], 0, 0, 0);
  } else if constexpr (G::KS <= 3) {
    h8 kf[G::K1P];
#pragma unroll
    for (int i = 0; i < G::K1P; ++i) kf[i] = k1[i * 64];
    __builtin_amdgcn_sched_barrier(0);
#pragma unroll
    for (int s = 0; s < G::KS; ++s)
#pragma unroll
      for (int rb = 0; rb < 2; ++rb)
#pragma unroll
        for (int hf = 0; hf < G::PXH; ++hf)
          h1[rb][hf] = mfma3s<net_dir<MODE> == NET_FWD2>(kf[(s * 2 + rb) * 2 + 0], kf[(s * 2 + rb) * 2 + 1], xh[s][hf], xl[s][hf], h1[rb][hf]);
  } else {
#pragma unroll
    for (int s = 0; s < G::KS; ++s)
#pragma unroll
      for (int rb = 0; rb < 2; ++rb) {
        const h8 ah = k1[((s * 2 + rb) * 2 + 0) * 64], al = k1[((s * 2 + rb) * 2 + 1) * 64];
#pragma unroll
        for (int hf = 0; hf < G::PXH; ++hf) h1[rb][hf] = mfma3s<net_dir<MODE> == NET_FWD2>(ah, al, xh[s][hf], xl[s][hf], h1[rb][hf]);
      }
  }
  unsigned bits = 0;
  if constexpr (PAIR) {
    static_assert(G::PXH == 2, "pairs: two pixel halves per wave");
    const int stq = (int)c.wblk * 32 + 2 * (lane & 15);
    if constexpr ((MODE & NET_STORE) && PASS == 0)
      bits = h3s_act_pair<net_dir<MODE>, true>(h1[0][0], h1[1][0], h1[0][1], h1[1][1], a.sc1, mask, bh, bl, uniform_fptr(a.st1 + (size_t)fi * 32 * a.Q),
                                            ((unsigned)(4 * (lane >> 4)) * (unsigned)a.Q + (unsigned)stq) * 4u, (unsigned)a.Q * 4u);
    else bits = h3s_act_pair<net_dir<MODE>, false>(h1[0][0], h1[1][0], h1[0][1], h1[1][1], a.sc1, mask, bh, bl, nullptr, 0u, 0u);
  } else {
#pragma unroll
    for (int hf = 0; hf < G::PXH; ++hf) {
      const int stq = (int)c.wblk * (16 * G::PXH) + 16 * hf + (lane & 15);
      bits |= h3s_act<net_dir<MODE>, (MODE & NET_STORE) != 0>(h1[0][hf], h1[1][hf], a.sc1, mask >> (8 * hf), bh[hf], bl[hf], (MODE & NET_STORE) && PASS == 0 && stq < a.Q,
                                                   (MODE & NET_STORE) ? uniform_fptr(a.st1 + (size_t)fi * 32 * a.Q) : nullptr,
                                                   ((unsigned)(4 * (lane >> 4)) * (unsigned)a.Q + (unsigned)stq) * 4u, (unsigned)a.Q * 4u) << (8 * hf);
    }
  }
// ... 99 lines not shown
      const h8 ah = buf[(tp * 2 + 0) * 64], al = buf[(tp * 2 + 1) * 64];
      acc3[ml][0] = mfma3s<net_dir<MODE> == NET_FWD2>(ah, al, bh[0], bl[0], acc3[ml][0]);
      if constexpr (G::PXH == 2) acc3[ml][1] = mfma3s<net_dir<MODE> == NET_FWD2>(ah, al, bh[1], bl[1], acc3[ml][1]);
      if (fo == NFH - 1) {
#pragma unroll
        for (int hf = 0; hf < G::PXH; ++hf)
#pragma unroll
          for (int r = 0; r < 4; ++r) {
            const int m = mt * 16 + 4 * kq + r;
            const float val = net_dir<MODE> == NET_BWD ? acc3[ml][hf][r] * (a.sc3 * c.ub[hf])
                              : PASS == 0 ? fmaf(acc3[ml][hf][r], a.sc3, pb[m]) : acc3[ml][hf][r] * a.sc3;
            if (MERGE && PASS == 0) { keep[ml][hf][r] = val; continue; }
            if constexpr (G::FUSE) {
              if (m < M3) c.pl[m * FUSE_PSTR + (int)(threadIdx.x >> 6) * 32 + 16 * hf + (lane & 15)] = val + keep[ml][hf][r];
              continue;
            }
            if (m < M3 && qok[hf]) Pp[(size_t)m * a.Q + q[hf]] = MERGE ? val + keep[ml][hf][r] : val;
          }
      }
    }
  }
  h3_wait_barrier();
}

template <int KIN, int MOUT, int NF, int MODE, int NP, int P0, int PASS, bool SOLO, int... Z>
__device__ __forceinline__ void h3s_tail(const NetArgs& a, const H3Ctx& c, const float* epl, f32x4 (&acc2)[(RingS<KIN, MOUT, NF, MODE, NP>::NRB)][2],
                                         f32x4 (&acc3)[(RingS<KIN, MOUT, NF, MODE, NP>::G0N)][2], h8 (&bh)[2], h8 (&bl)[2], int g, const int (&q)[2],
                                         const bool (&qok)[2], int lane, int kq, f32x4 (&keep)[(RingS<KIN, MOUT, NF, MODE, NP>::G0N)][2],
                                         std::integer_sequence<int, Z...>) {
  (h3s_Z<KIN, MOUT, NF, MODE, NP, P0, PASS, SOLO, Z>(a, c, epl, acc2, acc3, bh, bl, g, q, qok, lane, kq, keep), ...);
}

template <int KIN, int MOUT, int NF, int MODE, int NP, int P0, int PASS, bool SOLO>
__device__ __forceinline__ void h3s_pass(const NetArgs& a, const H3Ctx& c, const float* epl, const h8 (&xh)[(RingS<KIN, MOUT, NF, MODE, NP>::KS)][2],
                                         const h8 (&xl)[(RingS<KIN, MOUT, NF, MODE, NP>::KS)][2], int g, const int (&q)[2], const bool (&qok)[2], int lane, int kq,
                                         f32x4 (&keep)[(RingS<KIN, MOUT, NF, MODE, NP>::G0N)][2]) {
  using G = RingS<KIN, MOUT, NF, MODE, NP>;
  constexpr int NRB = G::NRB;
  constexpr int f2base = PASS * G::NFH * 32;
  f32x4 acc2[NRB][2];
#pragma unroll
  for (int ob = 0; ob < NRB; ++ob)
#pragma unroll
    for (int r = 0; r < 4; ++r) {
      const float b = net_dir<MODE> == NET_BWD ? 0.0f : epl[f2base + ob * 16 + 4 * kq + r];
      acc2[ob][0][r] = b;
      acc2[ob][1][r] = b;
    }
  h8 bh[2], bl[2];
#pragma nounroll
  for (int i0 = 0; i0 < NF; i0 += 2) {
    h3s_X<KIN, MOUT, NF, MODE, NP, 0, PASS>(a, c, i0, xh, xl, lane, bh, bl);
    h3_x_end<MODE, PASS, 8 * G::PXH>(c);
    if (PASS >= 1 && !SOLO && G::NCH == 1 && i0 == 0 && !g)
      stage4<G::MAINP, 50>(G::out_chunk(c.img, PASS, 0), c.sD, c.w4, c.voff);
    h3s_Y<KIN, MOUT, NF, MODE, NP, 1>(P0 ? c.sB : c.sA, bh, bl, acc2, lane, g, true, G::main_chunk(c.img, PASS, i0 + 1), P0 ? c.sA : c.sB,
                         c.k1img + (size_t)((i0 + 2) % NF) * G::K14, c.k1s0, c.w4, c.voff);
    h3_barrier();
    h3s_X<KIN, MOUT, NF, MODE, NP, 1, PASS>(a, c, i0 + 1, xh, xl, lane, bh, bl);
    h3_x_end<MODE, PASS, 8 * G::PXH>(c);
    h3s_Y<KIN, MOUT, NF, MODE, NP, 2>(P0 ? c.sA : c.sB, bh, bl, acc2, lane, g, i0 + 2 < NF || G::NCH >= 2,
                         i0 + 2 < NF ? G::main_chunk(c.img, PASS, i0 + 2) : G::out_chunk(c.img, PASS, 1),
                         P0 ? c.sB : c.sA, c.k1img + (size_t)((i0 + 3) % NF) * G::K14, c.k1s1, c.w4, c.voff);
    h3_barrier();
  }
  f32x4 acc3[G::G0N][2];
  h3s_tail<KIN, MOUT, NF, MODE, NP, P0, PASS, SOLO>(a, c, epl, acc2, acc3, bh, bl, g, q, qok, lane, kq, keep, std::make_integer_sequence<int, 2 * G::NCH>());
}

template <int KIN, int MOUT, int NF, int MODE, int NP, int PASS, int P0>
__device__ __forceinline__ void h3s_passes(const NetArgs& a, const H3Ctx& c, const float* epl, const h8 (&xh)[(RingS<KIN, MOUT, NF, MODE, NP>::KS)][2],
                                           const h8 (&xl)[(RingS<KIN, MOUT, NF, MODE, NP>::KS)][2], int g, const int (&q)[2], const bool (&qok)[2], int lane, int kq,
                                           f32x4 (&keep)[(RingS<KIN, MOUT, NF, MODE, NP>::G0N)][2]) {
  h3s_pass<KIN, MOUT, NF, MODE, NP, P0, PASS, false>(a, c, epl, xh, xl, g, q, qok, lane, kq, keep);
  if constexpr (PASS + 1 < NP) h3s_passes<KIN, MOUT, NF, MODE, NP, PASS + 1, (RingS<KIN, MOUT, NF, MODE, NP>::NCH + 1 + P0) & 1>(a, c, epl, xh, xl, g, q, qok, lane, kq, keep);
}

__device__ __forceinline__ bool fz_not_finite(float v) { return !(fabsf(v) <= 3.0e38f); }

template <int PXW = 256, int PSTR = FUSE_PSTR>
__device__ __forceinline__ void fused_couple(const NetArgs& a, const float* pl, const float4* vst, int tid) {
  const int wave = tid >> 6, lane = tid & 63;
  const int px = wave * 32 + (lane & 31), k = lane >> 5;
  const int q = (int)blockIdx.x * PXW + px;
  const bool qok = q < a.Q;
  const int w = a.w, hw = a.h * a.w, nrows = PXW / w;
  const int pp = (qok ? q : 0) % hw;
  const int i = pp / w, j = pp % w, r = px / w;
  float ols = 0.0f, ot = 0.0f;
  bool missing = false;
#pragma unroll
  for (int tap = 0; tap < 9; ++tap) {
    const int dy = tap / 3 - 1, dx = tap % 3 - 1;
    const int ii = i + dy, jj = j + dx;
    if (ii < 0 || ii >= a.h || jj < 0 || jj >= w) continue;
    const int rr = r + dy;
    if (rr < 0 || rr >= nrows) { missing = true; continue; }
    const int spx = px + dy * w + dx;
    ols += pl[(tap * 4 + k) * PSTR + spx];
    ot += pl[(tap * 4 + 2 + k) * PSTR + spx];
  }
  ols += a.fz_b3[k];
  ot += a.fz_b3[2 + k];
  float lsum = 0.0f;
  const float4 v4 = vst[px];
  const float vk = k ? v4.y : v4.x;
  const float log_s = tanhf(ols);
  const float sc = expf(log_s);
  const float yk = a.fz_inverse ? (vk - ot) / sc : sc * vk + ot;
  const float yo = __shfl_xor(yk, 32, 64);
  const float y[4] = {k ? yo : yk, k ? yk : yo, v4.z, v4.w};
  if (qok && a.fz_osave) a.fz_osave[(size_t)q * 2 + k] = ols;
  if (qok && !missing) {
    lsum = log_s;
    bool bad = fz_not_finite(ols) | fz_not_finite(ot) | fz_not_finite(yk);
    if (bad && a.flag) *a.flag = 1;
    float z0, z1;
    if (a.fz_A) {
      z0 = a.fz_b[2 * k]; z1 = a.fz_b[2 * k + 1];
#pragma unroll
      for (int ci = 0; ci < 4; ++ci) {
        z0 = fmaf(y[ci], a.fz_A[ci * 4 + 2 * k], z0);
        z1 = fmaf(y[ci], a.fz_A[ci * 4 + 2 * k + 1], z1);
      }
    } else {
      z0 = y[2 * k]; z1 = y[2 * k + 1];
    }
    *reinterpret_cast<float2*>(a.fz_out + (size_t)q * a.fz_out_stride + a.fz_out_off + 2 * k) = float2{z0, z1};
  } else if (qok) {
    float* e = a.fz_edge + (((size_t)blockIdx.x * 4 + (r == 0 ? 0 : 1)) * FUSE_EW + j) * 4;
    e[k] = ols;
    e[2 + k] = ot;
  }
  for (int te = tid; te < 2 * w * 4; te += 2 * PXW) {
    const int which = te / (4 * w), jt = (te / 4) % w, ch = te & 3;
    float hsum = 0.0f;
#pragma unroll
    for (int dx = -1; dx <= 1; ++dx) {
      const int js = jt + dx;
      if (js < 0 || js >= w) continue;
      const int tap = (which ? 0 : 6) + dx + 1;
      hsum += pl[(tap * 4 + ch) * PSTR + (which ? (nrows - 1) * w : 0) + js];
    }
    a.fz_edge[(((size_t)blockIdx.x * 4 + 2 + which) * FUSE_EW + jt) * 4 + ch] = hsum;
  }
  if (a.fz_ldpart) {
    double d = (double)lsum;
#pragma unroll
    for (int o = 32; o > 0; o >>= 1) d += __shfl_down(d, o, 64);
    if (lane == 0) a.fz_ldpart[(size_t)blockIdx.x * (PXW / 32) + wave] = d;
  }
}

template <int KIN, int MOUT, int NF, int MODE, int NP, bool SPLIT>
__global__ __launch_bounds__(512, 2) void k_net_h3s(NetArgs a) {
  using G = RingS<KIN, MOUT, NF, MODE, NP>;
  constexpr int KS = G::KS;
  constexpr int SGN = (net_dir<MODE> == NET_BWD) ? -1 : 1;
  static_assert(G::FITS, "shape");

  __shared__ float4 slotA[G::MAIN4];
  __shared__ float4 slotB[G::MAIN4];
  __shared__ float4 slotD[G::MAIN4];
  __shared__ float4 k1slot0[G::K14];
  __shared__ float4 k1slot1[G::K14];
  __shared__ float epl[G::EPN];
  __shared__ __attribute__((aligned(16))) unsigned short mkl[G::MASK2B / 2 + 8];
  __shared__ float plds[G::FUSE ? 36 * FUSE_PSTR : 1];
  __shared__ float4 vstash[G::FUSE ? 256 : 1];
  static_assert(!G::FUSE || (G::MERGE && !SPLIT && MOUT == 36), "the fused coupling needs both passes in one workgroup and a 4-channel level");
  static_assert(!(MODE & NET_STORE) || G::PXH == 1, "hidden stores (training): half-wave form only -- with two pixel halves a wave whose second half lies "
                                            "beyond Q would issue fewer stores than h3_x_end's counted wait assumes");

  const int tid = threadIdx.x;
  const int lane = tid & 63;
  const int wave = __builtin_amdgcn_readfirstlane(tid >> 6);
  const int g = wave >> 2;
  const int n16 = lane & 15;
  const int kq = lane >> 4;
  const int qbase = (blockIdx.x * 8 + (tid >> 6)) * (16 * G::PXH);
  const int q[2] = {qbase + n16, G::PXH == 2 ? qbase + 16 + n16 : qbase + n16};
  const bool qok[2] = {q[0] < a.Q, G::PXH == 2 && q[1] < a.Q};

  H3Ctx c;
  c.sA = slotA; c.sB = slotB; c.sD = slotD; c.k1s0 = k1slot0; c.k1s1 = k1slot1;
  const int solo_pass = SPLIT ? (int)blockIdx.y : 0;
  c.k1img = a.RSp;
  c.img = a.RSp;
  c.mkl = mkl;
  c.mk2off = 8 * NF * 64;
  c.pl = plds;
  c.wblk = (size_t)blockIdx.x * 8 + wave;
  c.wok = (long)c.wblk * (16 * G::PXH) < a.Q;
  c.w4 = wave & 3;
  c.voff = (unsigned)lane * 16u;
  c.ub[0] = c.ub[1] = 1.0f;

  if (!g) {
    stage4<G::MAINP, 60>(G::main_chunk(c.img, solo_pass, 0), slotA, c.w4, c.voff);
    stage4<G::MAINP, 61>(G::out_chunk(c.img, solo_pass, 0), slotD, c.w4, c.voff);
    if (net_dir<MODE> == NET_BWD)
      stage4<NF, 64>(reinterpret_cast<const float4*>(a.mask1 + (size_t)blockIdx.x * 8 * NF * 64), reinterpret_cast<float4*>(mkl), c.w4, c.voff);
  } else {
    stage4<G::K1P, 62>(c.k1img, k1slot0, c.w4, c.voff);
    stage4<G::K1P, 63>(c.k1img + G::K14, k1slot1, c.w4, c.voff);
    if (net_dir<MODE> == NET_BWD)
      stage4<NF, 65>(reinterpret_cast<const float4*>(a.mask2 + (size_t)blockIdx.x * 8 * NF * 64), reinterpret_cast<float4*>(mkl + 8 * NF * 64), c.w4, c.voff);
  }
  h8 xh[KS][2], xl[KS][2];
  float xmax = 0.0f;
  {
    const int hw = a.h * a.w;
#pragma unroll
    for (int hf = 0; hf < G::PXH; ++hf) {
      const int qq = qok[hf] ? q[hf] : 0;
      const int rem = qq % hw;
      const int i = rem / a.w, j0 = rem % a.w;
      const float* base = a.vin + (long)qq * a.in_stride + a.in_off;
      if constexpr (net_dir<MODE> == NET_BWD) {
        float v[KS][8];
        float pm = 0.0f;
#pragma unroll
        for (int s = 0; s < KS; ++s) {
          gather8<KIN, false, SGN>(base, i, j0, a.h, a.w, a.in_stride, qok[hf], 32 * s + 8 * kq, v[s]);
          pm = range8(pm, v[s]);
        }
        pm = nan_max(pm, __shfl_xor(pm, 16, 64));
        pm = nan_max(pm, __shfl_xor(pm, 32, 64));
        xmax = nan_max(xmax, pm);
        const float fac = (MODE & NET_STORE) ? 1.0f : pixel_norm(pm, a.bnorm, c.ub[hf]);
#pragma unroll
        for (int s = 0; s < KS; ++s) {
#pragma unroll
          for (int j = 0; j < 8; ++j) v[s][j] *= fac;
          split8(v[s], xh[s][hf], xl[s][hf]);
        }
      } else if constexpr (G::STK) {
        xmax = gather_stacked<KIN, SGN, net_dir<MODE> == NET_FWD2, KS, G::KSX>(base, i, j0, a.h, a.w, a.in_stride, qok[hf], kq, xh, xl, hf, xmax);
      } else {
#pragma unroll
        for (int s = 0; s < KS; ++s) {
          float v[8];
          gather8<KIN, true, SGN>(base, i, j0, a.h, a.w, a.in_stride, qok[hf], 32 * s + 8 * kq, v);
          xmax = range8(xmax, v);
          split8(v, xh[s][hf], xl[s][hf]);
        }
      }
    }
  }
  if constexpr (G::FUSE) {
    if (tid < 256) {
      const int qv = (int)blockIdx.x * 256 + tid;
      vstash[tid] = qv < a.Q ? *reinterpret_cast<const float4*>(a.vin + (size_t)qv * 4) : float4{0.f, 0.f, 0.f, 0.f};
    }
  }
  if (net_dir<MODE> != NET_BWD)
    for (int i = tid; i < G::EPN; i += 512) epl[i] = a.eph[i];
  if (((net_dir<MODE> == NET_BWD && !(MODE & NET_STORE)) ? !(xmax <= 3.0e38f) : !(xmax <= a.xlim)) && a.flag) *a.flag = 1;
  if (a.xmax_out) range_probe(a.xmax_out, xmax);
  asm volatile("s_waitcnt vmcnt(0)" ::: "memory");
  __syncthreads();

  f32x4 keep[G::G0N][2];
  if (g) h3_barrier();
  if constexpr (SPLIT) {
    if (solo_pass == 0) h3s_pass<KIN, MOUT, NF, MODE, NP, 0, 0, true>(a, c, epl, xh, xl, g, q, qok, lane, kq, keep);
    else if (solo_pass == 1) h3s_pass<KIN, MOUT, NF, MODE, NP, 0, 1, true>(a, c, epl, xh, xl, g, q, qok, lane, kq, keep);
    else if constexpr (NP > 2) {
      if (solo_pass == 2) h3s_pass<KIN, MOUT, NF, MODE, NP, 0, 2, true>(a, c, epl, xh, xl, g, q, qok, lane, kq, keep);
      else h3s_pass<KIN, MOUT, NF, MODE, NP, 0, 3, true>(a, c, epl, xh, xl, g, q, qok, lane, kq, keep);
    }
  } else {
    h3s_passes<KIN, MOUT, NF, MODE, NP, 0, 0>(a, c, epl, xh, xl, g, q, qok, lane, kq, keep);
  }
  if (!g) h3_barrier();
  if constexpr (G::FUSE) {
    __syncthreads();
    fused_couple(a, plds, vstash, tid);
  }
}
```

audiosourcesep_amd/csrc/glowk_launch.h:

```cpp
#pragma once
#include "glowk_kernels.h"
#include "glowk_co.h"
#include "glowk_q.h"

#include <cstdlib>
#include <string>

#define GLOWK_NET_SHAPES(X) X(2, 16) X(4, 16) X(8, 16) X(16, 16) X(2, 12) X(4, 12) X(8, 12) X(16, 12) \
                            X(2, 8) X(4, 8) X(8, 8) X(16, 8) X(2, 4) X(4, 4) X(8, 4) X(16, 4)

enum NetArith { NET_EXACT, NET_SPLIT3, NET_SPLIT2 };
struct NetCall { int dir; NetArith arith; bool store = false; };

enum NetFamily { FAM_F32, FAM_H3, FAM_H3S, FAM_H3S_HALF, FAM_FUSED, FAM_CO, FAM_Q, FAM_COUNT };

struct NetLaunch {
  int np = 0;
  int family = FAM_F32;
  bool co = false;
  bool q = false;
  int fused_px = 0;
  bool failed = false;
  explicit operator bool() const { return np > 0 || fused_px > 0; }
};

namespace glowk_detail {

int num_cus();
void launch_fail(const std::string&);

struct EnvSwitches {
  bool bwd_light_4;
  bool no_fuse;
  bool wgrad_plain;
  bool co_off;
  bool q_off;
  bool co_train_off;
  bool train_recompute;
  bool train_perstep;
  bool pg_join;
};
const EnvSwitches& env();

template <int CI, int DIR>
struct NetShape {
  static constexpr int KIN = DIR == NET_BWD ? 2 * CI : CI;
  static constexpr int MOUT = DIR == NET_BWD ? 9 * CI : 18 * CI;
};

template <int CI, int NF, int DIR, bool STORE>
NetLaunch launch_f32(const NetArgs& a, hipStream_t s, bool dry) {
  using Sh = NetShape<CI, DIR>;
  if (!dry) hipLaunchKernelGGL((k_net_f32<Sh::KIN, Sh::MOUT, NF, DIR, STORE>), dim3((a.Q + 127) / 128), dim3(256), 0, s, a);
  return {1, FAM_F32};
}

template <int KIN, int MOUT, int NF, int MODE>
NetLaunch launch_h3(const NetArgs& a, hipStream_t s, bool dry) {
  constexpr bool F2 = RingH<KIN, MOUT, NF, MODE, 2>::FITS, F4 = RingH<KIN, MOUT, NF, MODE, 4>::FITS;
  const int wgs = (a.Q + 255) / 256, cus = num_cus();
  if constexpr (F4) {
    if (a.max_np >= 4 && (4 * wgs <= cus || !F2)) {
      const bool split = 4 * wgs <= cus;
      if (!dry) {
        if (split) hipLaunchKernelGGL((k_net_h3<KIN, MOUT, NF, MODE, 4, true>), dim3(wgs, 4), dim3(512), 0, s, a);
        else hipLaunchKernelGGL((k_net_h3<KIN, MOUT, NF, MODE, 4, false>), dim3(wgs), dim3(512), 0, s, a);
      }
      return {4, FAM_H3};
    }
  }
  if constexpr (F2) {
    if (!dry) {
      if (2 * wgs <= cus) hipLaunchKernelGGL((k_net_h3<KIN, MOUT, NF, MODE, 2, true>), dim3(wgs, 2), dim3(512), 0, s, a);
      else hipLaunchKernelGGL((k_net_h3<KIN, MOUT, NF, MODE, 2, false>), dim3(wgs), dim3(512), 0, s, a);
    }
    return {2, FAM_H3};
  }
  return {};
}

template <class Kernel>
inline bool co_two_per_cu(Kernel kernel) {
  static int blocks = -1;
  if (blocks < 0) {
    int n = 0;
    if (hipOccupancyMaxActiveBlocksPerMultiprocessor(&n, kernel, 256, 0) != hipSuccess) { (void)hipGetLastError(); n = 0; }
    blocks = n;
  }
  return blocks >= 2;
}

template <int KIN, int MOUT, int NF, int MODE>
NetLaunch launch_h3s(const NetArgs& a, hipStream_t s, bool dry) {
  static_assert(!(MODE & NET_STORE), "no storing launches here: the co-resident branch does not check Q % 128 (launch_co_train does)");
  constexpr bool F2 = RingS<KIN, MOUT, NF, MODE, 2>::FITS, F4 = RingS<KIN, MOUT, NF, MODE, 4>::FITS;
  const int wgs = (a.Q + 255) / 256, cus = num_cus();
  if constexpr (F4) {
    if (a.max_np >= 4 && (4 * wgs <= cus || !F2)) {
      const bool split = 4 * wgs <= cus;
      if (!dry) {
        if (split) hipLaunchKernelGGL((k_net_h3s<KIN, MOUT, NF, MODE, 4, true>), dim3(wgs, 4), dim3(512), 0, s, a);
        else hipLaunchKernelGGL((k_net_h3s<KIN, MOUT, NF, MODE, 4, false>), dim3(wgs), dim3(512), 0, s, a);
      }
      return {4, FAM_H3S};
    }
  }
  if constexpr (F2) {
    const bool split = 2 * wgs <= cus;
    if constexpr (RingC<KIN, MOUT, NF, MODE>::FITS) {
      const int wgc = (a.Q + CO_PX - 1) / CO_PX;
      const bool co_ok = a.co && !env().co_off;
      if (co_ok && wgc > cus) {
        if constexpr (RingC<KIN, MOUT, NF, MODE | NET_FUSE>::FITS) {
          if (a.fuse && co_two_per_cu(k_net_h3c<KIN, MOUT, NF, MODE | NET_FUSE, false>)) {
            if (!dry) hipLaunchKernelGGL((k_net_h3c<KIN, MOUT, NF, MODE | NET_FUSE, false>), dim3(wgc), dim3(256), 0, s, a);
            return {0, FAM_FUSED, true, false, CO_PX};
          }
        }
        if (!a.fuse && co_two_per_cu(k_net_h3c<KIN, MOUT, NF, MODE, false>)) {
          if (!dry) hipLaunchKernelGGL((k_net_h3c<KIN, MOUT, NF, MODE, false>), dim3(wgc), dim3(256), 0, s, a);
          return {RingC<KIN, MOUT, NF, MODE>::MERGE ? 1 : 2, FAM_H3S, true};
        }
      }
      if (co_ok && split && wgc <= cus && a.max_np >= 2 && co_two_per_cu(k_net_h3c<KIN, MOUT, NF, MODE, true>)) {
        if (!dry) hipLaunchKernelGGL((k_net_h3c<KIN, MOUT, NF, MODE, true>), dim3(wgc, 2), dim3(256), 0, s, a);
        return {2, FAM_H3S, true};
      }
    }
    if constexpr ((MODE == NET_FWD || MODE == NET_FWD2 || MODE == NET_FWD_SAVE) && MOUT == 36) {
      if constexpr (RingS<KIN, MOUT, NF, MODE | NET_FUSE, 2>::FITS && RingS<KIN, MOUT, NF, MODE | NET_FUSE, 2>::MERGE) {
        if (a.fuse && !split) {
          if (!dry) hipLaunchKernelGGL((k_net_h3s<KIN, MOUT, NF, MODE | NET_FUSE, 2, false>), dim3(wgs), dim3(512), 0, s, a);
          return {0, FAM_FUSED, false, false, 256};
        }
      }
    }
    if (!dry) {
      if (split) hipLaunchKernelGGL((k_net_h3s<KIN, MOUT, NF, MODE, 2, true>), dim3(wgs, 2), dim3(512), 0, s, a);
      else hipLaunchKernelGGL((k_net_h3s<KIN, MOUT, NF, MODE, 2, false>), dim3(wgs), dim3(512), 0, s, a);
    }
    return {(!split && RingS<KIN, MOUT, NF, MODE, 2>::MERGE) ? 1 : 2, FAM_H3S};
  }
  return {};
}

inline bool half_wave_grid(const NetArgs& a) { return 8 * ((a.Q + 255) / 256) <= num_cus(); }

template <int KIN, int MOUT, int NF, int MODE>
NetLaunch launch_h3s_half(const NetArgs& a, hipStream_t s, bool dry) {
  if constexpr (RingS<KIN, MOUT, NF, MODE | NET_HALF, 4>::FITS) {
    if (a.max_np < 4) return {};
    const int wgs = (a.Q + 127) / 128;
    if constexpr (RingQ<KIN, MOUT, NF, MODE>::FITS) {
      if (4 * wgs <= num_cus() && !env().q_off) {
        if (!dry) hipLaunchKernelGGL((k_net_h3q<KIN, MOUT, NF, MODE>), dim3(wgs, 4), dim3(512), 0, s, a);
        return {4, FAM_H3S_HALF, false, true};
      }
    }
    if (!dry) {
      if (4 * wgs <= num_cus()) hipLaunchKernelGGL((k_net_h3s<KIN, MOUT, NF, MODE | NET_HALF, 4, true>), dim3(wgs, 4), dim3(512), 0, s, a);
      else hipLaunchKernelGGL((k_net_h3s<KIN, MOUT, NF, MODE | NET_HALF, 4, false>), dim3(wgs), dim3(512), 0, s, a);
    }
    return {4, FAM_H3S_HALF};
  }
  return {};
}

template <int CI, int NF, int STORE = 0>
constexpr bool half_ok() {
  return RingS<CI, 18 * CI, NF, NET_FWD_SAVE | STORE | NET_HALF, 4>::FITS && RingS<2 * CI, 9 * CI, NF, NET_BWD | STORE | NET_HALF, 4>::FITS;
}
template <int CI, int NF>
constexpr bool half_only() {
  return half_ok<CI, NF>() && !(RingS<2 * CI, 9 * CI, NF, NET_BWD, 2>::FITS || RingS<2 * CI, 9 * CI, NF, NET_BWD, 4>::FITS) &&
         !(RingH<2 * CI, 9 * CI, NF, NET_BWD, 2>::FITS || RingH<2 * CI, 9 * CI, NF, NET_BWD, 4>::FITS);
}
template <int CI, int NF>
constexpr bool half_train_only() {
  constexpr int FS = NET_FWD_SAVE | NET_STORE, BS = NET_BWD | NET_STORE;
  return half_ok<CI, NF, NET_STORE>() && !((RingH<CI, 18 * CI, NF, FS, 2>::FITS || RingH<CI, 18 * CI, NF, FS, 4>::FITS) &&
                                           (RingH<2 * CI, 9 * CI, NF, BS, 2>::FITS || RingH<2 * CI, 9 * CI, NF, BS, 4>::FITS));
}
template <int CI, int NF>
inline bool use_half_train(const NetArgs& a) {
  if constexpr (!half_ok<CI, NF, NET_STORE>()) return false;
  return a.fam16 && a.max_np >= 4 && (half_train_only<CI, NF>() || half_wave_grid(a));
}

template <int CI, int NF>
inline bool use_half(const NetArgs& a) {
  if constexpr (!half_ok<CI, NF>()) return false;
  return a.fam16 && a.max_np >= 4 && (half_only<CI, NF>() || half_wave_grid(a));
}

inline bool big_grid(const NetArgs& a) { return 2 * ((a.Q + 255) / 256) > num_cus(); }

template <int CI, int NF>
inline bool co_split_grad(const NetArgs& a) {
  if constexpr (RingC<CI, 18 * CI, NF, NET_FWD_SAVE>::FITS && RingC<2 * CI, 9 * CI, NF, NET_BWD>::FITS) {
    const int wgc = (a.Q + CO_PX - 1) / CO_PX, cus = num_cus();
    return a.co && !env().co_off && a.fam16 && a.max_np >= 2 && 2 * ((a.Q + 255) / 256) <= cus && wgc <= cus &&
           co_two_per_cu(k_net_h3c<CI, 18 * CI, NF, NET_FWD_SAVE, true>) && co_two_per_cu(k_net_h3c<2 * CI, 9 * CI, NF, NET_BWD, true>);
  }
  return false;
}

template <int CI, int NF>
constexpr bool fam16_ok() {
  return RingS<CI, 18 * CI, NF, NET_FWD_SAVE, 2>::FITS && (RingS<2 * CI, 9 * CI, NF, NET_BWD, 2>::FITS || RingS<2 * CI, 9 * CI, NF, NET_BWD, 4>::FITS);
}

template <int CI, int NF, int DIR>
NetLaunch launch_co_train(const NetArgs& a, hipStream_t s, bool dry) {
  constexpr int FS = NET_FWD_SAVE | NET_STORE, BS = NET_BWD | NET_STORE;
  if constexpr (RingC<CI, 18 * CI, NF, FS>::FITS && RingC<2 * CI, 9 * CI, NF, BS>::FITS) {
    const int wgc = (a.Q + CO_PX - 1) / CO_PX, cus = num_cus();
    if (!(a.co && !env().co_off && !env().co_train_off && a.fam16 && a.Q % CO_PX == 0 && a.max_np >= 2)) return {};
    using Sh = NetShape<CI, DIR>;
    if (wgc > cus) {
      if (!(co_two_per_cu(k_net_h3c<CI, 18 * CI, NF, FS, false>) && co_two_per_cu(k_net_h3c<2 * CI, 9 * CI, NF, BS, false>))) return {};
      if (!dry) hipLaunchKernelGGL((k_net_h3c<Sh::KIN, Sh::MOUT, NF, DIR | NET_STORE, false>), dim3(wgc), dim3(256), 0, s, a);
      return {1, FAM_H3S, true};
    }
    if (!(co_two_per_cu(k_net_h3c<CI, 18 * CI, NF, FS, true>) && co_two_per_cu(k_net_h3c<2 * CI, 9 * CI, NF, BS, true>))) return {};
    if (!dry) hipLaunchKernelGGL((k_net_h3c<Sh::KIN, Sh::MOUT, NF, DIR | NET_STORE, true>), dim3(wgc, 2), dim3(256), 0, s, a);
    return {2, FAM_H3S, true};
  }
  return {};
}

template <int CI, int NF>
NetLaunch launch_split3_fwd(const NetArgs& a, bool half, hipStream_t s, bool dry) {
  NetLaunch r;
  if (half && a.RSp && half_wave_grid(a) && !a.fuse) r = launch_h3s_half<CI, 18 * CI, NF, NET_FWD>(a, s, dry);
  if (!r && a.RSp) r = launch_h3s<CI, 18 * CI, NF, NET_FWD>(a, s, dry);
  if (!r && a.RHp) r = launch_h3<CI, 18 * CI, NF, NET_FWD>(a, s, dry);
  if (!r) r = launch_f32<CI, NF, NET_FWD, false>(a, s, dry);
  return r;
}
template <int CI, int NF>
NetLaunch launch_split2_fwd(const NetArgs& a, hipStream_t s, bool dry) {
  NetLaunch r;
  if (a.RSp) r = launch_h3s<CI, 18 * CI, NF, NET_FWD2>(a, s, dry);
  return r ? r : launch_split3_fwd<CI, NF>(a, false, s, dry);
}

template <int CI, int NF, int DIR>
NetLaunch launch_split_grad(const NetArgs& a, hipStream_t s, bool dry) {
  using Sh = NetShape<CI, DIR>;
  NetLaunch r;
  if (use_half<CI, NF>(a)) r = launch_h3s_half<Sh::KIN, Sh::MOUT, NF, DIR>(a, s, dry);
  if constexpr (fam16_ok<CI, NF>()) {
    if (!r && a.fam16 && (big_grid(a) || co_split_grad<CI, NF>(a))) r = launch_h3s<Sh::KIN, Sh::MOUT, NF, DIR>(a, s, dry);
  }
  if (!r && a.RHp) r = launch_h3<Sh::KIN, Sh::MOUT, NF, DIR>(a, s, dry);
  if (!r) r = launch_f32<CI, NF, DIR, false>(a, s, dry);
  return r;
}

inline NetLaunch net_failed(const std::string& m) { launch_fail(m); NetLaunch r; r.failed = true; return r; }

template <int CI, int NF, int DIR>
NetLaunch launch_split_train(const NetArgs& a, hipStream_t s, bool dry) {
  using Sh = NetShape<CI, DIR>;
  constexpr int MODE = DIR | NET_STORE;
  NetLaunch r;
  if (use_half_train<CI, NF>(a)) r = launch_h3s_half<Sh::KIN, Sh::MOUT, NF, MODE>(a, s, dry);
  if (!r) r = launch_co_train<CI, NF, DIR>(a, s, dry);
  if (!r && a.RHp) r = launch_h3<Sh::KIN, Sh::MOUT, NF, MODE>(a, s, dry);
  if (!r && !dry) return net_failed("no split-arithmetic training instance for this shape");
  return r;
}

template <int CI, int NF, bool STORE>
NetLaunch launch_exact(const NetArgs& a, int dir, hipStream_t s, bool dry) {
  if (dir == NET_FWD) return launch_f32<CI, NF, NET_FWD, STORE>(a, s, dry);
  if (dir == NET_FWD_SAVE) return launch_f32<CI, NF, NET_FWD_SAVE, STORE>(a, s, dry);
  return launch_f32<CI, NF, NET_BWD, STORE>(a, s, dry);
}

template <int CI, int NF>
NetLaunch launch_net_t(const NetArgs& a, NetCall call, hipStream_t s, bool dry) {
  const bool save = call.dir == NET_FWD_SAVE;
  if (call.dir != NET_FWD && !save && call.dir != NET_BWD) return net_failed("bad k_net mode");
// ... 21 lines not shown
```

audiosourcesep_amd/csrc/glowk_light.h:

```cpp
#pragma once
#include "glowk_kernels.h"

__device__ __forceinline__ double block_sum_any(double v, double* red ) {
#pragma unroll
  for (int o = 32; o > 0; o >>= 1) v += __shfl_down(v, o, 64);
  __syncthreads();
  if ((threadIdx.x & 63) == 0) red[threadIdx.x >> 6] = v;
  __syncthreads();
  double t = 0.0;
  const int nw = (int)blockDim.x >> 6;
  for (int w = 0; w < nw; ++w) t += red[w];
  return t;
}

__device__ __forceinline__ double block_sum_256(double v, double* red ) {
#pragma unroll
  for (int o = 32; o > 0; o >>= 1) v += __shfl_down(v, o, 64);
  __syncthreads();
  if ((threadIdx.x & 63) == 0) red[threadIdx.x >> 6] = v;
  __syncthreads();
  return red[0] + red[1] + red[2] + red[3];
}


struct PreArgs {
  float minval, maxval, alpha;
  int use_logit;
};

__device__ __forceinline__ float pre_fwd(float x, const PreArgs& p, float& ld) {
  float u = (x - p.minval) / (p.maxval - p.minval);
  if (p.use_logit) {
    u = (1.0f - 2.0f * p.alpha) * u + p.alpha;
    const float lp = logf(u), lq = logf(1.0f - u);
    ld += -lp - lq;
    return lp - lq;
  }
  return u - 0.5f;
}

__device__ __forceinline__ float pre_inv(float y, const PreArgs& p) {
  if (p.use_logit) {
    y = 1.0f / (1.0f + expf(-y));
    y = (y - p.alpha) / (1.0f - 2.0f * p.alpha);
  } else {
    y += 0.5f;
  }
  return y * (p.maxval - p.minval) + p.minval;
}

template <int C>
__global__ __launch_bounds__(256) void k_in(const float* __restrict__ x, int H, int W, PreArgs pre, int do_pre,
                                           const float* __restrict__ A, const float* __restrict__ b,
                                           float* __restrict__ v, double* __restrict__ logdet, double ld_const) {
  __shared__ double red[4];
  constexpr int Cin = C / 4;
  const int n = blockIdx.x, h = H / 2, w = W / 2;
  float ld = 0.0f;
  for (int pp = threadIdx.x; pp < h * w; pp += 256) {
    const int i = pp / w, j = pp % w;
    float u[C], y[C];
#pragma unroll
    for (int cc = 0; cc < C; ++cc) {
      const int cin = cc >> 2, da = (cc >> 1) & 1, db = cc & 1;
      const float xv = x[((size_t)(n * H + 2 * i + da) * W + (2 * j + db)) * Cin + cin];
      u[cc] = do_pre ? pre_fwd(xv, pre, ld) : xv;
    }
    float* dst = v + ((size_t)n * h * w + pp) * C;
    if (A) {
      affine_cc<C>(A, b, u, y);
#pragma unroll
      for (int cc = 0; cc < C; ++cc) dst[cc] = y[cc];
    } else {
#pragma unroll
      for (int cc = 0; cc < C; ++cc) dst[cc] = u[cc];
    }
  }
  if (logdet) {
    const double tot = block_sum_256((double)ld, red);
    if (threadIdx.x == 0) logdet[n] = ld_const + tot;
  }
}

template <int C>
__global__ __launch_bounds__(256) void k_out(const float* __restrict__ u, int h, int w, PreArgs pre, int do_pre,
                                            float* __restrict__ x) {
  constexpr int Cin = C / 4;
  const int n = blockIdx.x, H = 2 * h, W = 2 * w;
  for (int pp = threadIdx.x; pp < h * w; pp += 256) {
    const int i = pp / w, j = pp % w;
    const float* src = u + ((size_t)n * h * w + pp) * C;
#pragma unroll
    for (int cc = 0; cc < C; ++cc) {
      const int cin = cc >> 2, da = (cc >> 1) & 1, db = cc & 1;
      const float val = src[cc];
      x[((size_t)(n * H + 2 * i + da) * W + (2 * j + db)) * Cin + cin] = do_pre ? pre_inv(val, pre) : val;
    }
  }
}

__global__ __launch_bounds__(256) void k_pre_only(const float* __restrict__ x, int E, PreArgs pre, int inverse,
                                                 float* __restrict__ y, float* __restrict__ logdet, double ld_const) {
  __shared__ double red[4];
  const int n = blockIdx.x;
  float ld = 0.0f;
  for (int e = threadIdx.x; e < E; e += 256) {
    const float xv = x[(size_t)n * E + e];
    y[(size_t)n * E + e] = inverse ? pre_inv(xv, pre) : pre_fwd(xv, pre, ld);
  }
  if (logdet) {
    const double tot = block_sum_256((double)ld, red);
    if (threadIdx.x == 0) logdet[n] = (float)(ld_const + tot);
  }
}

struct CoupleArgs {
  const float* vin;
  const float* P;
  int np;
  size_t pstride;
  const float* b3;
  const float* A;
  const float* b;
  float* out;
  int out_stride, out_off;
  double* logdet;
  float* log_s_out;
  float* t_out;
  float* o_save;
  int Q, h, w;
  int inverse;
  int* flag;
};

__device__ __forceinline__ bool not_finite(float v) { return !(fabsf(v) <= 3.0e38f); }

template <int C, int LPP>
__device__ __forceinline__ float couple_pixel(const CoupleArgs& a, int q, int i, int j, bool live, int r4) {
  constexpr int CI = C / 2;
  constexpr bool QUAD = LPP == 4;
  float v[C], o[C];
#pragma unroll
  for (int c = 0; c < C; ++c) o[c] = 0.0f;
  if constexpr (LPP == 16) {
    for (int idx = r4; idx < 9 * a.np; idx += 16) {
      const int tap = idx / a.np, part = idx % a.np;
      const int dy = tap / 3 - 1, dx = tap % 3 - 1;
      const int ii = i + dy, jj = j + dx;
      if (ii >= 0 && ii < a.h && jj >= 0 && jj < a.w) {
        const float* src = a.P + (size_t)part * a.pstride + (size_t)(tap * C) * a.Q + (q + dy * a.w + dx);
#pragma unroll
        for (int c = 0; c < C; ++c) o[c] += src[(size_t)c * a.Q];
      }
    }
  } else {
#pragma unroll
  for (int u = 0; u < (QUAD ? 3 : 9); ++u) {
    const int tap = QUAD ? r4 + 4 * u : u;
    const int dy = tap / 3 - 1, dx = tap % 3 - 1;
    const int ii = i + dy, jj = j + dx;
    if (tap < 9 && ii >= 0 && ii < a.h && jj >= 0 && jj < a.w) {
      const size_t off = (size_t)(tap * C) * a.Q + (q + dy * a.w + dx);
#pragma unroll
      for (int part = 0; part < 4; ++part)
        if (part < a.np) {
          const float* src = a.P + (size_t)part * a.pstride + off;
#pragma unroll
          for (int c = 0; c < C; ++c) o[c] += src[(size_t)c * a.Q];
        }
    }
  }
  }
#pragma unroll
  for (int c = 0; c < C; ++c) {
#pragma unroll
    for (int m = 1; m < LPP; m <<= 1) o[c] += __shfl_xor(o[c], m, 64);
    o[c] += a.b3[c];
  }
  if constexpr (LPP == 16) {
    constexpr int CPL = (C + 15) / 16;
    float yo[CPL], ls_sum = 0.0f;
    bool bad = false;
#pragma unroll
    for (int e = 0; e < CPL; ++e) {
      const int ch = r4 + 16 * e;
      float oc = 0.0f, ot = 0.0f;
#pragma unroll
      for (int c = 0; c < C; ++c) oc = (c == ch) ? o[c] : oc;
#pragma unroll
      for (int c = 0; c < CI; ++c) ot = (c == ch) ? o[CI + c] : ot;
      const bool mine = ch < C, first = ch < CI;
      const float vch = (a.vin && mine) ? a.vin[(size_t)q * C + ch] : 0.0f;
      float y = vch;
      if (first) {
        const float log_s = tanhf(oc);
        if (a.log_s_out && live) { a.log_s_out[(size_t)q * CI + ch] = log_s; a.t_out[(size_t)q * CI + ch] = ot; }
        if (a.o_save && live) a.o_save[(size_t)q * CI + ch] = oc;
        if (a.vin) {
          const float sc = expf(log_s);
          y = a.inverse ? (vch - ot) / sc : sc * vch + ot;
        }
        if (live) ls_sum += log_s;
      }
      bad |= mine && (not_finite(oc) | not_finite(y));
      yo[e] = y;
    }
    if (bad && live && a.flag) *a.flag = 1;
    if (a.out) {
      float z[CPL];
      const int lane0 = (int)(threadIdx.x & 63) & ~15;
      if (a.A) {
#pragma unroll
        for (int e = 0; e < CPL; ++e) z[e] = (r4 + 16 * e < C) ? a.b[r4 + 16 * e] : 0.0f;
#pragma unroll
        for (int ci = 0; ci < C; ++ci) {
          const float yc = __shfl(yo[ci / 16], lane0 + (ci & 15), 64);
#pragma unroll
          for (int e = 0; e < CPL; ++e)
            if (r4 + 16 * e < C) z[e] = fmaf(yc, a.A[ci * C + r4 + 16 * e], z[e]);
        }
      } else {
#pragma unroll
        for (int e = 0; e < CPL; ++e) z[e] = yo[e];
      }
      if (live) {
        float* dst = a.out + (size_t)q * a.out_stride + a.out_off;
#pragma unroll
        for (int e = 0; e < CPL; ++e)
          if (r4 + 16 * e < C) dst[r4 + 16 * e] = z[e];
      }
    }
    return ls_sum;
  }
  if (r4 != 0 || !live) return 0.0f;
  if (a.flag) {
    bool bad = false;
#pragma unroll
    for (int c = 0; c < C; ++c) bad |= not_finite(o[c]);
    if (bad) *a.flag = 1;
  }
  if (a.o_save) {
#pragma unroll
    for (int k = 0; k < CI; ++k) a.o_save[(size_t)q * CI + k] = o[k];
  }
  if (a.vin) {
#pragma unroll
    for (int c = 0; c < C; ++c) v[c] = a.vin[(size_t)q * C + c];
  }
  float y[C];
  float lsum = 0.0f;
#pragma unroll
  for (int k = 0; k < CI; ++k) {
    const float log_s = tanhf(o[k]);
    const float t = o[CI + k];
    if (a.log_s_out) { a.log_s_out[(size_t)q * CI + k] = log_s; a.t_out[(size_t)q * CI + k] = t; }
    if (a.vin) {
      const float s = expf(log_s);
      y[k] = a.inverse ? (v[k] - t) / s : s * v[k] + t;
      y[CI + k] = v[CI + k];
    }
    lsum += log_s;
  }
  if (a.flag && a.vin) {
    bool bad = false;
#pragma unroll
    for (int c = 0; c < C; ++c) bad |= not_finite(y[c]);
    if (bad) *a.flag = 1;
  }
  if (a.out) {
    float* dst = a.out + (size_t)q * a.out_stride + a.out_off;
    if (a.A) {
      float z[C];
      affine_cc<C>(a.A, a.b, y, z);
#pragma unroll
      for (int c = 0; c < C; ++c) dst[c] = z[c];
    } else {
#pragma unroll
      for (int c = 0; c < C; ++c) dst[c] = y[c];
    }
  }
  return lsum;
}

template <int C, bool QUAD>
__global__ __launch_bounds__(1024) void k_couple(CoupleArgs a) {
  __shared__ double red[16];
  const int n = blockIdx.x;
  const int hw = a.h * a.w;
  float lsum = 0.0f;
  const int r4 = QUAD ? (threadIdx.x & 3) : 0;
  const int qpb = QUAD ? (int)blockDim.x >> 2 : (int)blockDim.x;
  for (int pp0 = QUAD ? threadIdx.x >> 2 : threadIdx.x; pp0 < (hw + qpb - 1) / qpb * qpb; pp0 += qpb) {
    const bool live = pp0 < hw;
    const int pp = live ? pp0 : hw - 1;
    lsum += couple_pixel<C, QUAD ? 4 : 1>(a, n * hw + pp, pp / a.w, pp % a.w, live, r4);
  }
  if (a.logdet) {
    const double tot = block_sum_any((double)lsum, red);
    if (threadIdx.x == 0) a.logdet[n] += tot;
  }
}

template <int C, int LPP>
__global__ __launch_bounds__(256) void k_couple_flat(CoupleArgs a, double* slot, int sample_stride, int slot_base) {
  __shared__ double red[4];
  constexpr int PPB = 256 / LPP;
  const int hw = a.h * a.w;
  const int q0 = (int)blockIdx.x * PPB + ((int)threadIdx.x / LPP);
  const bool live = q0 < a.Q;
  const int q = live ? q0 : a.Q - 1;
  const int pp = q % hw;
  const float lsum = couple_pixel<C, LPP>(a, q, pp / a.w, pp % a.w, live, threadIdx.x & (LPP - 1));
  if (slot) {
    const double tot = block_sum_256((double)lsum, red);
    const int first = (int)blockIdx.x * PPB;
    if (threadIdx.x == 0) slot[(size_t)(first / hw) * sample_stride + slot_base + (first % hw) / 16] = tot;
  }
}

__global__ __launch_bounds__(64) void k_ld_fold(double* __restrict__ logdet, const double* __restrict__ slot, int nslots) {
  const int n = blockIdx.x;
  double acc = 0.0;
  for (int i = threadIdx.x; i < nslots; i += 64) acc += slot[(size_t)n * nslots + i];
#pragma unroll
  for (int o = 32; o > 0; o >>= 1) acc += __shfl_down(acc, o, 64);
  if (threadIdx.x == 0) logdet[n] += acc;
}

struct EdgeArgs {
  const float* vin;
  const float* edge;
  const double* ldpart;
  const float *A, *b;
  float* out;
  int out_stride, out_off, inverse;
  double* logdet;
  float* osave;
  int h, w;
  int* flag;
  int pxw;
};

__global__ __launch_bounds__(256) void k_couple_edge(EdgeArgs a) {
  __shared__ double red[4];
  const int n = blockIdx.x, w = a.w, hw = a.h * a.w;
  const int pxw = a.pxw;
  const int nb = hw >= pxw ? hw / pxw : 1, rows = pxw / w;
  float lsum = 0.0f;
  const int nedge = hw > pxw ? 2 * w * (nb - 1) : 0;
  for (int t = threadIdx.x; t < nedge; t += 256) {
    const int b = 1 + t / (2 * w), lower = (t / w) & 1, j = t % w;
    const size_t wgA = (size_t)n * nb + b - 1, wgB = wgA + 1;
    const float4 part = *reinterpret_cast<const float4*>(a.edge + (((lower ? wgB : wgA) * 4 + (lower ? 0 : 1)) * FUSE_EW + j) * 4);
    const float4 halo = *reinterpret_cast<const float4*>(a.edge + (((lower ? wgA : wgB) * 4 + (lower ? 3 : 2)) * FUSE_EW + j) * 4);
    const size_t q = (size_t)n * hw + (size_t)(b * rows - 1 + lower) * w + j;
    const float o[4] = {part.x + halo.x, part.y + halo.y, part.z + halo.z, part.w + halo.w};
    const float4 v4 = *reinterpret_cast<const float4*>(a.vin + q * 4);
    const float v[4] = {v4.x, v4.y, v4.z, v4.w};
    if (a.osave) { a.osave[q * 2] = o[0]; a.osave[q * 2 + 1] = o[1]; }
    float y[4];
    bool bad = false;
#pragma unroll
    for (int k = 0; k < 2; ++k) {
      const float log_s = tanhf(o[k]), sc = expf(log_s), tt = o[2 + k];
      y[k] = a.inverse ? (v[k] - tt) / sc : sc * v[k] + tt;
      y[2 + k] = v[2 + k];
      lsum += log_s;
      bad |= fz_not_finite(o[k]) | fz_not_finite(tt) | fz_not_finite(y[k]);
    }
    if (bad && a.flag) *a.flag = 1;
    float z[4];
    if (a.A) {
#pragma unroll
      for (int co = 0; co < 4; ++co) z[co] = a.b[co];
#pragma unroll
      for (int ci = 0; ci < 4; ++ci)
#pragma unroll
        for (int co = 0; co < 4; ++co) z[co] = fmaf(y[ci], a.A[ci * 4 + co], z[co]);
    } else {
#pragma unroll
      for (int co = 0; co < 4; ++co) z[co] = y[co];
    }
    *reinterpret_cast<float4*>(a.out + q * a.out_stride + a.out_off) = float4{z[0], z[1], z[2], z[3]};
  }
  if (a.logdet) {
    double d = (double)lsum;
#pragma unroll
    for (int o = 32; o > 0; o >>= 1) d += __shfl_down(d, o, 64);
    if ((threadIdx.x & 63) == 0) red[threadIdx.x >> 6] = d;
    __syncthreads();
    if (threadIdx.x == 0) {
      double tot = red[0] + red[1] + red[2] + red[3];
      const size_t i0 = (size_t)n * (hw / 32);
      for (int x = 0; x < hw / 32; ++x) tot += a.ldpart[i0 + x];
      a.logdet[n] += tot;
    }
  }
}

template <int C>
__global__ __launch_bounds__(256) void k_affine(const float* __restrict__ in, int Q, const float* __restrict__ A,
                                               const float* __restrict__ b, float* __restrict__ out) {
  const int q = blockIdx.x * 256 + threadIdx.x;
  if (q >= Q) return;
  float x[C], y[C];
#pragma unroll
  for (int c = 0; c < C; ++c) x[c] = in[(size_t)q * C + c];
  affine_cc<C>(A, b, x, y);
#pragma unroll
  for (int c = 0; c < C; ++c) out[(size_t)q * C + c] = y[c];
}

template <int C>
__global__ __launch_bounds__(256) void k_split(const float* __restrict__ o, int h, int w,
                                              float* __restrict__ latent, int HWl, int Cl, int off, int Cz,
                                              const float* __restrict__ A, const float* __restrict__ b,
                                              float* __restrict__ vnext) {
  constexpr int CH = C / 2;
  constexpr int C2 = 2 * C;
  const int n = blockIdx.x, hw = h * w;
  const float* on = o + (size_t)n * hw * C;
  if (latent) {
    for (int e = threadIdx.x; e < hw * CH; e += 256) {
      const int pp = e / CH, k = e % CH;
      latent[((size_t)n * HWl + e / Cz) * Cl + off + e % Cz] = on[(size_t)pp * C + k];
    }
  }
  const int h2 = h / 2, w2 = w / 2;
  for (int pp = threadIdx.x; pp < h2 * w2; pp += 256) {
    const int i = pp / w2, j = pp % w2;
    float u[C2], y[C2];
#pragma unroll
    for (int cc = 0; cc < C2; ++cc) {
      const int cin = cc >> 2, da = (cc >> 1) & 1, db = cc & 1;
// ... 419 lines not shown
```

audiosourcesep_amd/engine.py:

```python
import ctypes
import os
import warnings

import numpy as np
import torch

from . import _lib
from .config import GlowConfig


def _stream_ptr(device):
    return ctypes.c_void_p(torch.cuda.current_stream(device).cuda_stream)


def _ptr(t):
    return ctypes.c_void_p(t.data_ptr()) if t is not None else ctypes.c_void_p(0)


class GlowEngine:
    _reserved_grad = 0
    _grad_cap = None
    _ran_grad = 0
    _grad_chunk = (None, 0)

# ... 19 lines not shown
    def close(self):
        if getattr(self, "h", None):
            self.lib.glowk_destroy(self.h)
            self.h = None

    def __del__(self):
        try:
            self.close()
        except Exception:
            pass

    @staticmethod
    def _split_name(name):
        if name in _lib.PRIOR_TENSOR_IDS:
            return -1, 0, _lib.PRIOR_TENSOR_IDS[name]
        lvl, stp, rest = name.split("/", 2)
        return int(lvl[1:]), int(stp[1:]), _lib.STEP_TENSOR_IDS[rest]

    def set_tensor(self, name, value):
        level, step, tid = self._split_name(name)
        a = np.ascontiguousarray(np.asarray(value, dtype=np.float32)).ravel()
        _lib.check(self.lib.glowk_set_tensor(self.h, level, step, tid, a.ctypes.data_as(_lib._fp), a.size))
        self._finalized = False

    def get_tensor(self, name):
        level, step, tid = self._split_name(name)
        n = self.lib.glowk_tensor_size(self.h, level, tid)
        a = np.empty(n, dtype=np.float32)
        _lib.check(self.lib.glowk_get_tensor(self.h, level, step, tid, a.ctypes.data_as(_lib._fp), a.size))
        return a

    def load_params(self, params):
        for name, value in params.items():
            self.set_tensor(name, value)
        self.finalize()

    def finalize(self):
        _lib.check(self.lib.glowk_finalize_weights(self.h))
        self._finalized = True

    def actnorm_data_init(self, minibatch, runtime_order=False, raw_minibatch_quirk=True):
        x = self._in(minibatch, self.data_shape)
        _lib.check(self.lib.glowk_actnorm_data_init(self.h, _ptr(x), x.shape[0], int(runtime_order), int(raw_minibatch_quirk),
                                                    self._stream()))

    def actnorm_params(self):
        out = {}
        for lvl in range(self.cfg.L):
            for k in range(self.cfg.K):
                for t in ("actnorm/log_scale", "actnorm/shift"):
                    name = "b%d/s%d/%s" % (lvl, k, t)
                    out[name] = self.get_tensor(name)
        return out

    def set_precision(self, mode):
        _lib.check(self.lib.glowk_set_precision(self.h, int(mode)))

    def get_precision(self):
        return int(self.lib.glowk_get_precision(self.h))

    def set_range_policy(self, policy):
        modes = {"ignore": _lib.RANGE_IGNORE, "error": _lib.RANGE_ERROR, "fallback": _lib.RANGE_FALLBACK}
        _lib.check(self.lib.glowk_set_range_policy(self.h, modes[policy] if isinstance(policy, str) else int(policy)))

    def range_status(self, sync=True):
        tripped, n = ctypes.c_int(0), ctypes.c_int64(0)
        _lib.check(self.lib.glowk_range_status(self.h, ctypes.byref(tripped) if sync else None, ctypes.byref(n), self._stream()))
        return bool(tripped.value), int(n.value)

    def range_probe_begin(self):
        _lib.check(self.lib.glowk_range_probe_begin(self.h))

    def range_probe_end(self):
        f, b = ctypes.c_float(0), ctypes.c_float(0)
        _lib.check(self.lib.glowk_range_probe_end(self.h, ctypes.byref(f), ctypes.byref(b), self._stream()))
        return float(f.value), float(b.value)

    def _after_call(self):
        if self.get_precision() == _lib.PREC_F32:
            return
        n = self.range_status(sync=False)[1]
        if n > self._fallbacks_seen:
            if self._fallbacks_seen == 0:
                warnings.warn("glowk: a hidden activation left the fp16 range of the split arithmetic; the call was re-run on the "
                              "exact fp32 kernels (slower). Consider set_precision(PREC_F32) for this checkpoint.", RuntimeWarning,
                              stacklevel=3)
            self._fallbacks_seen = n

    def reserve(self, n, with_grad=False):
        m = min(int(n), self.grad_max_tiles if with_grad else self.max_tiles)
        self._reserve_or_shrink(m, with_grad)

    def _reserve_or_shrink(self, m, with_grad):
        while True:
            try:
                _lib.check(self.lib.glowk_reserve(self.h, int(m), int(with_grad)))
                break
            except _lib.GlowkError as e:
                if not with_grad or m <= 1 or "out of memory" not in str(e).lower():
                    raise
                torch.cuda.empty_cache()
                m = max(1, m // 2)
                self._reserved_grad = 0
                self._ran_grad = 0
                self._grad_cap = m
        if with_grad:
            self._reserved_grad = max(self._reserved_grad, int(m))

    @property
    def max_tiles(self):
        m = int(self.lib.glowk_max_tiles(self.h))
        return min(m, self._max_tiles_cap) if self._max_tiles_cap else m

    def _chunks(self, n, m=None):
        m = m or self.max_tiles
        return [(i, min(i + m, n)) for i in range(0, n, m)]

    @property
    def grad_max_tiles(self):
        if not self._finalized:
            self.finalize()
        free = self._free_bytes()
        own = self.workspace_bytes(self._reserved_grad, True) if self._reserved_grad else 0
        key = (self.get_precision(), self._max_tiles_cap, (free + own) >> 30)
        key = key + (self._grad_cap,)
        if self._grad_chunk[0] == key:
            return self._grad_chunk[1]
        budget = min(0.6 * (free + own), float(os.environ.get("GLOWK_GRAD_BUDGET_GB", "64")) * 2 ** 30)
        top = min(self.max_tiles, self._grad_cap or self.max_tiles)
        lo, hi = 1, top
        if self.workspace_bytes(hi, True) > budget:
            while lo < hi:
                mid = (lo + hi + 1) // 2
                if self.workspace_bytes(mid, True) <= budget:
                    lo = mid
                else:
                    hi = mid - 1
        else:
            lo = hi
        lo = max(lo, min(self._ran_grad, top))
        self._grad_chunk = (key, lo)
        return lo

    def _free_bytes(self):
        return torch.cuda.mem_get_info(self.device)[0]

    def workspace_bytes(self, n, with_grad=False):
        return int(self.lib.glowk_workspace_bytes(self.h, int(n), int(with_grad)))

    @property
    def fused_steps(self):
        return int(self.lib.glowk_fused_steps(self.h))

    def kernel_families(self):
        out = (ctypes.c_int64 * 7)()
        _lib.check(self.lib.glowk_kernel_families(self.h, out))
        return dict(zip(("f32", "h3_32x32x16", "h3s_16x16x32", "h3s_half", "fused", "co_resident", "small_grid_q"), [int(v) for v in out]))

    def profile_begin(self):
        _lib.check(self.lib.glowk_profile_begin(self.h))

    def profile_end(self):
        p = _lib.GlowkProfile()
        _lib.check(self.lib.glowk_profile_end(self.h, ctypes.byref(p)))
        return [(p.net_ms[i], int(p.net_launches[i])) for i in range(self.cfg.L)]

    def _in(self, x, shape_tail):
        if not torch.is_tensor(x):
            x = torch.as_tensor(np.asarray(x, dtype=np.float32))
        x = x.to(device=self.device, dtype=torch.float32).contiguous()
        if tuple(x.shape[1:]) != tuple(shape_tail):
            raise ValueError("expected a [N, %s] tensor, got %s" % (", ".join(map(str, shape_tail)), tuple(x.shape)))
        if not self._finalized:
            self.finalize()
        return x

    def _new(self, *shape):
        return torch.empty(shape, device=self.device, dtype=torch.float32)

    @property
    def data_shape(self):
        return (self.cfg.H, self.cfg.W, self.cfg.C)

    def _compute(self, rc):
        _lib.check(rc)
        self._after_call()

    def forward(self, x, with_logdet=True):
        x = self._in(x, self.data_shape)
        n = x.shape[0]
        z = self._new(n, *self.cfg.latent_shape())
        ld = self._new(n) if with_logdet else None
        if n == 0:
            return (z, ld) if with_logdet else z
        for a, b in self._chunks(n):
            self._compute(self.lib.glowk_forward(self.h, _ptr(x[a:b]), b - a, _ptr(z[a:b]), _ptr(ld[a:b] if with_logdet else None),
                                              self._stream()))
        return (z, ld) if with_logdet else z

    def inverse(self, z):
        z = self._in(z, self.cfg.latent_shape())
        n = z.shape[0]
        x = self._new(n, *self.data_shape)
        if n == 0:
            return x
        for a, b in self._chunks(n):
            self._compute(self.lib.glowk_inverse(self.h, _ptr(z[a:b]), b - a, _ptr(x[a:b]), self._stream()))
        return x

    def log_prob(self, x, return_latent=False, out=None):
        x = self._in(x, self.data_shape)
        n = x.shape[0]
        lp = out if out is not None else self._new(n)
        z = self._new(n, *self.cfg.latent_shape()) if return_latent else None
        if n == 0:
            return (lp, z) if return_latent else lp
        for a, b in self._chunks(n):
            self._compute(self.lib.glowk_log_prob(self.h, _ptr(x[a:b]), b - a, _ptr(lp[a:b]), _ptr(z[a:b] if return_latent else None),
                                               self._stream()))
        return (lp, z) if return_latent else lp

    def log_prob_sum(self, x, out=None, total=None):
        x = self._in(x, self.data_shape)
        n = x.shape[0]
        lp = out if out is not None else self._new(n)
        if total is None:
            total = torch.empty(1, device=self.device, dtype=torch.float64)
        if n == 0:
            _lib.check(self.lib.glowk_sum_f64(_ptr(None), 0, _ptr(total), 0, 1.0, self._stream()))
            return lp, total
        for i, (a, b) in enumerate(self._chunks(n)):
            self._compute(self.lib.glowk_log_prob_sum(self.h, _ptr(x[a:b]), b - a, _ptr(lp[a:b]), _ptr(None), _ptr(total), int(i > 0),
                                                   self._stream()))
        return lp, total

    def sum_f64(self, v, scale=1.0, out=None):
        v = v.contiguous()
        if out is None:
            out = torch.empty(1, device=v.device, dtype=torch.float64)
        _lib.check(self.lib.glowk_sum_f64(_ptr(v), v.numel(), _ptr(out), 0, float(scale), _stream_ptr(v.device)))
        return out

    def log_prob_grad(self, x):
        x = self._in(x, self.data_shape)
        n = x.shape[0]
        lp, dx = self._new(n), torch.empty_like(x)
        if n == 0:
            return lp, dx
        chunk = self.grad_max_tiles
        if min(n, chunk) > self._reserved_grad:
            self._reserve_or_shrink(min(n, chunk), True)
            chunk = min(chunk, self.grad_max_tiles)
        for a, b in self._chunks(n, chunk):
            self._compute(self.lib.glowk_log_prob_grad(self.h, _ptr(x[a:b]), b - a, _ptr(lp[a:b]), _ptr(dx[a:b]), self._stream()))
        self._ran_grad = max(self._ran_grad, min(n, chunk))
        return lp, dx

    @property
    def param_vector_size(self):
        return int(self.lib.glowk_param_vector_size(self.h))

    def param_slice(self, name):
        level, step, tid = self._split_name(name)
        off, cnt = ctypes.c_size_t(0), ctypes.c_size_t(0)
        _lib.check(self.lib.glowk_param_offset(self.h, level, step, tid, ctypes.byref(off), ctypes.byref(cnt)))
        return int(off.value), int(cnt.value)

    def param_grad(self, x, scale, grad=None):
        x = self._in(x, self.data_shape)
        n = x.shape[0]
        if n > self.grad_max_tiles:
            raise ValueError("param_grad takes at most %d tiles per call (split the batch and add the gradients)" % self.grad_max_tiles)
        lp = self._new(n)
        if grad is None:
            grad = self._new(self.param_vector_size)
        self._compute(self.lib.glowk_param_grad(self.h, _ptr(x), n, float(scale), _ptr(lp), _ptr(grad), self._stream()))
        if n > self._ran_grad:
            self._ran_grad = n
            self._grad_chunk = (None, 0)
        return lp, grad

    def apply_gradients(self, grad, optimizer="adamax", lr=1e-3):
        opt = {"adam": 0, "adamax": 1}
        if optimizer not in opt:
            raise ValueError("optimizer argument should be adam or adamax")
        _lib.check(self.lib.glowk_apply_gradients(self.h, _ptr(grad), opt[optimizer], float(lr), self._stream()))
        self._finalized = True

    def sample_from_eps(self, eps):
        eps = self._in(eps, self.cfg.latent_shape())
        n = eps.shape[0]
        x = self._new(n, *self.data_shape)
        if n == 0:
            return x
        for a, b in self._chunks(n):
            self._compute(self.lib.glowk_sample(self.h, _ptr(eps[a:b]), b - a, _ptr(x[a:b]), self._stream()))
        return x

    def prior_log_prob(self, z):
        z = self._in(z, self.cfg.latent_shape())
        lp = self._new(z.shape[0])
        for a, b in self._chunks(z.shape[0]):
            _lib.check(self.lib.glowk_prior_log_prob(self.h, _ptr(z[a:b]), b - a, _ptr(lp[a:b]), self._stream()))
        return lp

    def preprocess_forward(self, x):
# ... 48 lines not shown
```

include/glowk.h:

```cpp
#ifndef GLOWK_H
#define GLOWK_H

#include <stddef.h>
#include <stdint.h>

#ifdef __cplusplus
extern "C" {
#endif

#define GLOWK_VERSION 480

typedef struct glowk_config {
  int32_t H, W, C;
  int32_t L, K, F;
  int32_t learntop;
  int32_t use_logit;
  float minval, maxval, alpha;
  float bn_eps;
} glowk_config;

typedef struct glowk_handle glowk_handle;

enum glowk_tensor_id {
  GLOWK_ACTNORM_LOG_SCALE = 0,
  GLOWK_ACTNORM_SHIFT = 1,
  GLOWK_INV1X1_P = 2,
  GLOWK_INV1X1_SIGN_S = 3,
  GLOWK_INV1X1_L = 4,
  GLOWK_INV1X1_LOG_S = 5,
  GLOWK_INV1X1_U = 6,
  GLOWK_CONV1_KERNEL = 7,
  GLOWK_CONV1_BIAS = 8,
  GLOWK_BN1_GAMMA = 9,
  GLOWK_BN1_BETA = 10,
  GLOWK_BN1_MEAN = 11,
  GLOWK_BN1_VAR = 12,
  GLOWK_CONV2_KERNEL = 13,
  GLOWK_CONV2_BIAS = 14,
  GLOWK_BN2_GAMMA = 15,
  GLOWK_BN2_BETA = 16,
  GLOWK_BN2_MEAN = 17,
  GLOWK_BN2_VAR = 18,
  GLOWK_CONV3_KERNEL = 19,
  GLOWK_CONV3_BIAS = 20,
  GLOWK_INV1X1_P_INV = 21,
  GLOWK_NUM_STEP_TENSORS = 22,
  GLOWK_PRIOR_LOC = 100,
  GLOWK_PRIOR_LOG_SCALE = 101
};

enum glowk_precision {
  GLOWK_PREC_F32 = 0,
  GLOWK_PREC_F16X3 = 1,
  GLOWK_PREC_F16X2 = 2
};

enum glowk_status {
  GLOWK_OK = 0,
  GLOWK_ERR = 1,
  GLOWK_ERR_RANGE = 2
};

enum glowk_range_policy { GLOWK_RANGE_IGNORE = 0, GLOWK_RANGE_ERROR = 1, GLOWK_RANGE_FALLBACK = 2 };

int glowk_version(void);
const char* glowk_last_error(void);
void glowk_reload_env(void);

int glowk_create(const glowk_config* cfg, int device, glowk_handle** out);
int glowk_destroy(glowk_handle* h);
size_t glowk_tensor_size(const glowk_handle* h, int level, int tensor_id);
int glowk_set_tensor(glowk_handle* h, int level, int step, int tensor_id, const float* host, size_t n);
int glowk_get_tensor(const glowk_handle* h, int level, int step, int tensor_id, float* host, size_t n);
int glowk_finalize_weights(glowk_handle* h);
int glowk_actnorm_data_init(glowk_handle* h, const float* x_dev, int N, int runtime_order, int raw_minibatch_quirk, void* stream);
int glowk_set_precision(glowk_handle* h, int precision);
int glowk_get_precision(const glowk_handle* h);
int glowk_set_range_policy(glowk_handle* h, int policy);
int glowk_get_range_policy(const glowk_handle* h);
int glowk_range_status(glowk_handle* h, int* tripped, int64_t* fallbacks, void* stream);
int glowk_range_probe_begin(glowk_handle* h);
int glowk_range_probe_end(glowk_handle* h, float* fwd_ratio, float* bwd_ratio, void* stream);
size_t glowk_workspace_bytes(const glowk_handle* h, int N, int with_grad);
int glowk_reserve(glowk_handle* h, int N, int with_grad);
int glowk_max_tiles(const glowk_handle* h);

int glowk_forward(glowk_handle* h, const float* x_dev, int N, float* z_dev, float* logdet_dev, void* stream);
int glowk_inverse(glowk_handle* h, const float* z_dev, int N, float* x_dev, void* stream);
int glowk_log_prob(glowk_handle* h, const float* x_dev, int N, float* logp_dev, float* z_dev, void* stream);
int glowk_log_prob_sum(glowk_handle* h, const float* x_dev, int N, float* logp_dev, float* z_dev, double* sum_dev, int accumulate,
                       void* stream);
int glowk_sum_f64(const float* v_dev, size_t n, double* out_dev, int accumulate, double scale, void* stream);
int glowk_log_prob_grad(glowk_handle* h, const float* x_dev, int N, float* logp_dev, float* dx_dev, void* stream);
int glowk_sample(glowk_handle* h, const float* eps_dev, int N, float* x_dev, void* stream);
int glowk_prior_log_prob(glowk_handle* h, const float* z_dev, int N, float* logp_dev, void* stream);

typedef struct glowk_profile {
  double net_ms[4];
  int64_t net_launches[4];
} glowk_profile;
int glowk_profile_begin(glowk_handle* h);
int64_t glowk_fused_steps(const glowk_handle* h);
int glowk_kernel_families(const glowk_handle* h, int64_t* out7);
int glowk_profile_end(glowk_handle* h, glowk_profile* out);

int glowk_squeeze(const float* x_dev, int N, int H, int W, int C, float* y_dev, void* stream);
int glowk_unsqueeze(const float* y_dev, int N, int h, int w, int c4, float* x_dev, void* stream);
int glowk_preprocess_forward(glowk_handle* h, const float* x_dev, int N, float* y_dev, float* logdet_dev, void* stream);
int glowk_preprocess_inverse(glowk_handle* h, const float* y_dev, int N, float* x_dev, void* stream);
int glowk_step_forward(glowk_handle* h, int level, int step, const float* u_dev, int N, float* y_dev, float* logdet_dev, void* stream);
int glowk_step_inverse(glowk_handle* h, int level, int step, const float* y_dev, int N, float* u_dev, void* stream);
int glowk_coupling_net(glowk_handle* h, int level, int step, const float* xb_dev, int N, float* log_s_dev, float* t_dev, void* stream);

size_t glowk_param_vector_size(glowk_handle* h);
int glowk_param_offset(glowk_handle* h, int level, int step, int tensor_id, size_t* offset, size_t* count);
int glowk_param_grad(glowk_handle* h, const float* x_dev, int N, float scale, float* logp_dev, float* grad_dev, void* stream);
int glowk_apply_gradients(glowk_handle* h, const float* grad_dev, int optimizer, float lr, void* stream);

int glowk_basis_update(float* x1_dev, float* x2_dev, const float* g1_dev, const float* g2_dev, const float* mixed_dev, size_t n,
                       float eta, float lambda_recon, const float* eps1_dev, const float* eps2_dev, uint64_t seed, uint64_t step,
                       uint64_t offset, int* nonfinite_dev, void* stream);
int glowk_basis_mix(const float* x1_dev, const float* x2_dev, float* out_dev, size_t n, void* stream);
enum glowk_mixing {
  GLOWK_MIX_DB = 0,
  GLOWK_MIX_MEAN = 1
};
int glowk_basis_update_n(float* const* x, const float* const* g, const float* const* eps, int nsrc, const float* mixed_dev, size_t n,
                         int mixing, float eta, float lambda_recon, uint64_t seed, uint64_t step, uint64_t offset,
                         int* nonfinite_dev, void* stream);
int glowk_basis_mix_n(const float* const* x, int nsrc, float* out_dev, size_t n, int mixing, void* stream);
int glowk_random(float* out_dev, size_t n, uint64_t seed, uint64_t step, int which, int uniform, uint64_t offset, void* stream);
int glowk_random_source(float* out_dev, size_t n, uint64_t seed, uint64_t step, int which, int pair, int uniform, uint64_t offset,
                        void* stream);
int glowk_add_noise(const float* x_dev, float* out_dev, size_t n, float sigma, uint64_t seed, uint64_t step, int which, uint64_t offset,
                    void* stream);

int glowk_mel_filterbank(float* host_out);
int glowk_mel_frontend(const float* audio_dev, int N, int n_samples, float top_db, float* mel_db_dev, float* stft_dev, void* stream);
int glowk_mel_to_power(const float* mel_db_dev, int N, int frames, int iters, float* power_dev, void* stream);
int glowk_masked_istft(const float* power_dev, int S, const float* stft_mix_dev, int N, int frames, int wiener, float* audio_dev,
                       void* stream);
int glowk_griffinlim(const float* mag_dev, const float* angles0_dev, int N, int frames, int n_iter, float momentum, float* audio_dev,
                     void* stream);

int64_t glowk_resample_length(int64_t n_in, int sr_in, int sr_out);
int glowk_resample_filter(double* host_out);
int glowk_resample(const float* x_dev, int nsig, int64_t n_in, int sr_in, int sr_out, float* y_dev, void* stream);

int glowk_bss_xcorr(const double* sig_dev, int nsig, int64_t nsampl, const int64_t* win_dev, int nwin, int64_t max_len, const int* pairs_dev,
                    int npairs, int filters_len, double* corr_dev, void* stream);
int glowk_bss_solve(const double* corr_dev, int nwin, int npairs, int nref, int filters_len, int nchan_sys, const int* sys_dev, int nsys,
                    double* coef_dev, int* status_dev, void* stream);
int glowk_bss_project(const double* sig_dev, int64_t nsampl, int nsrc, int nchan, int filters_len, const int64_t* items_dev, int nitems,
                      int64_t max_len, const double* coef_c_dev, int nsys_c, const double* coef_j_dev, int nsys_j, double* energy_dev,
                      void* stream);

int glowk_sp_stft(const float* x_dev, int nsig, int64_t n, float* spec_dev, void* stream);
int glowk_sp_istft(const float* spec_dev, int nsig, int frames, int64_t length, float* out_dev, void* stream);
int glowk_oracle_mask(float* spec_dev, int nsrc, int nchan, int frames, int irm, double alpha, double theta, uint8_t* mask_dev,
                      void* stream);
int glowk_mwf(float* spec_dev, int nsrc, int frames, void* stream);
int glowk_oracle_mel(const double* mix_dev, const void* src_dev, int nsrc, int64_t n, int src_f64, int irm, double theta, void* out_dev,
                     void* stream);

int glowk_mwf_em(const float* x_dev, float* v_dev, int nsrc, int nprob, int frames, int n_iter, float* y_dev, double* r_dev,
                 void* stream);

uint32_t glowk_crc32c(const void* host_data, size_t n);

#ifdef __cplusplus
}
#endif
#endif
```

Measured before the change: 16660.

## Fuse affine coupling tail into split-conv net kernel for 8/16-channel levels

```diff
diff --git a/__graft_entry__.py b/__graft_entry__.py
--- a/__graft_entry__.py
+++ b/__graft_entry__.py
@@ -20,7 +20,7 @@
 def build(force=False, extra_flags=(), tag=None):
     from concurrent.futures import ThreadPoolExecutor
     hdr = os.path.join(ROOT, "include", "glowk.h")
-    net_src = [os.path.join(CSRC, f) for f in ("glowk_act_scale.h", "glowk_kernels.h", "glowk_co.h", "glowk_q.h", "glowk_launch.h",
+    net_src = [os.path.join(CSRC, f) for f in ("glowk_act_scale.h", "glowk_couple.h", "glowk_kernels.h", "glowk_co.h", "glowk_q.h", "glowk_launch.h",
                                                 "glowk_net_inst.hip")]
     eng_src = [os.path.join(CSRC, f) for f in sorted(os.listdir(CSRC)) if f.endswith((".hip", ".h")) and f != "glowk_net_inst.hip"] + [hdr]
     hipcc = os.environ.get("HIPCC", "/opt/rocm/bin/hipcc")
diff --git a/audiosourcesep_amd/_lib.py b/audiosourcesep_amd/_lib.py
--- a/audiosourcesep_amd/_lib.py
+++ b/audiosourcesep_amd/_lib.py
@@ -79,6 +79,7 @@
     "glowk_sample": (_i, [_vp, _vp, _i, _vp, _vp]),
     "glowk_prior_log_prob": (_i, [_vp, _vp, _i, _vp, _vp]),
     "glowk_fused_steps": (ctypes.c_int64, [_vp]),
+    "glowk_coupled_tail_steps": (ctypes.c_int64, [_vp]),
     "glowk_kernel_families": (_i, [_vp, ctypes.POINTER(ctypes.c_int64)]),
     "glowk_profile_begin": (_i, [_vp]),
     "glowk_profile_end": (_i, [_vp, ctypes.POINTER(GlowkProfile)]),
diff --git a/audiosourcesep_amd/csrc/glowk.hip b/audiosourcesep_amd/csrc/glowk.hip
--- a/audiosourcesep_amd/csrc/glowk.hip
+++ b/audiosourcesep_amd/csrc/glowk.hip
@@ -141,7 +141,7 @@
     const size_t edge_floats = (wgs * 4 * FUSE_EW * 4 + 3) & ~(size_t)3;
     const size_t nld = wgs * (pxw / 32);
     if ((edge_floats + 2 * nld + 4) <= 4 * h->pstride) {
-      na.fuse = 1;
+      na.fuse = NET_ASK_FUSE;
       na.fz_b3 = ca.b3; na.fz_A = ca.A; na.fz_b = ca.b; na.fz_out = ca.out; na.fz_out_stride = ca.out_stride; na.fz_out_off = ca.out_off;
       na.fz_inverse = ca.inverse;
       na.fz_osave = ca.o_save;
@@ -149,8 +149,20 @@
       na.fz_ldpart = ca.logdet ? reinterpret_cast<double*>(h->bufP + edge_floats) : nullptr;
     }
   }
+  if (!no_fuse && (c == 8 || c == 16) && call.arith != NET_EXACT && call.dir == NET_FWD && !call.store && na.RSp && ca.vin && ca.vin == na.vin &&
+      na.in_stride == c && ca.out && !ca.o_save && !ca.log_s_out && 256 % hw == 0 && N >= 2 * num_cus() && 2 * (((size_t)ca.Q + 255) / 256) > (size_t)num_cus() &&
+      na.P == h->bufP && na.max_np >= 2) {
+    na.fuse = NET_ASK_TAIL;
+    na.fz_b3 = ca.b3; na.fz_A = ca.A; na.fz_b = ca.b; na.fz_out = ca.out; na.fz_out_stride = ca.out_stride; na.fz_out_off = ca.out_off;
+    na.fz_inverse = ca.inverse;
+    na.fz_ldpart = ca.logdet;
+  }
   NetLaunch r;
   if (int rc = launch_net(h, lvl, c, F, na, s, call, &r)) return rc;
+  if (r.tail) {
+    ++h->coupled_tail_steps;
+    return 0;
+  }
   if (!r.fused_px) {
     ca.P = na.P; ca.np = r.np; ca.pstride = na.pstride;
     return launch_couple(c, ca, N, s, fl, flat_used);
@@ -1059,6 +1071,7 @@
 }
 
 int64_t glowk_fused_steps(const glowk_handle* h) { return h ? h->fused_steps : -1; }
+int64_t glowk_coupled_tail_steps(const glowk_handle* h) { return h ? h->coupled_tail_steps : -1; }
 
 int glowk_kernel_families(const glowk_handle* h, int64_t* out7) {
   if (!h || !out7) return fail("null argument");
diff --git a/audiosourcesep_amd/csrc/glowk_couple.h b/audiosourcesep_amd/csrc/glowk_couple.h
--- /dev/null
+++ b/audiosourcesep_amd/csrc/glowk_couple.h
@@ -0,0 +1,180 @@
+#pragma once
+#include <hip/hip_runtime.h>
+
+template <int C>
+__device__ __forceinline__ void affine_cc(const float* __restrict__ A, const float* __restrict__ b, const float (&x)[C], float (&y)[C]) {
+#pragma unroll
+  for (int co = 0; co < C; ++co) y[co] = b[co];
+#pragma unroll
+  for (int ci = 0; ci < C; ++ci)
+#pragma unroll
+    for (int co = 0; co < C; ++co) y[co] = fmaf(x[ci], A[ci * C + co], y[co]);
+}
+
+struct CoupleArgs {
+  const float* vin;
+  const float* P;
+  int np;
+  size_t pstride;
+  const float* b3;
+  const float* A;
+  const float* b;
+  float* out;
+  int out_stride, out_off;
+  double* logdet;
+  float* log_s_out;
+  float* t_out;
+  float* o_save;
+  int Q, h, w;
+  int inverse;
+  int* flag;
+};
+
+__device__ __forceinline__ bool not_finite(float v) { return !(fabsf(v) <= 3.0e38f); }
+
+template <int C, int LPP>
+__device__ __forceinline__ float couple_pixel(const CoupleArgs& a, int q, int i, int j, bool live, int r4) {
+  constexpr int CI = C / 2;
+  constexpr bool QUAD = LPP == 4;
+  float v[C], o[C];
+#pragma unroll
+  for (int c = 0; c < C; ++c) o[c] = 0.0f;
+  if constexpr (LPP == 16) {
+    for (int idx = r4; idx < 9 * a.np; idx += 16) {
+      const int tap = idx / a.np, part = idx % a.np;
+      const int dy = tap / 3 - 1, dx = tap % 3 - 1;
+      const int ii = i + dy, jj = j + dx;
+      if (ii >= 0 && ii < a.h && jj >= 0 && jj < a.w) {
+        const float* src = a.P + (size_t)part * a.pstride + (size_t)(tap * C) * a.Q + (q + dy * a.w + dx);
+#pragma unroll
+        for (int c = 0; c < C; ++c) o[c] += src[(size_t)c * a.Q];
+      }
+    }
+  } else {
+#pragma unroll
+  for (int u = 0; u < (QUAD ? 3 : 9); ++u) {
+    const int tap = QUAD ? r4 + 4 * u : u;
+    const int dy = tap / 3 - 1, dx = tap % 3 - 1;
+    const int ii = i + dy, jj = j + dx;
+    if (tap < 9 && ii >= 0 && ii < a.h && jj >= 0 && jj < a.w) {
+      const size_t off = (size_t)(tap * C) * a.Q + (q + dy * a.w + dx);
+#pragma unroll
+      for (int part = 0; part < 4; ++part)
+        if (part < a.np) {
+          const float* src = a.P + (size_t)part * a.pstride + off;
+#pragma unroll
+          for (int c = 0; c < C; ++c) o[c] += src[(size_t)c * a.Q];
+        }
+    }
+  }
+  }
+#pragma unroll
+  for (int c = 0; c < C; ++c) {
+#pragma unroll
+    for (int m = 1; m < LPP; m <<= 1) o[c] += __shfl_xor(o[c], m, 64);
+    o[c] += a.b3[c];
+  }
+  if constexpr (LPP == 16) {
+    constexpr int CPL = (C + 15) / 16;
+    float yo[CPL], ls_sum = 0.0f;
+    bool bad = false;
+#pragma unroll
+    for (int e = 0; e < CPL; ++e) {
+      const int ch = r4 + 16 * e;
+      float oc = 0.0f, ot = 0.0f;
+#pragma unroll
+      for (int c = 0; c < C; ++c) oc = (c == ch) ? o[c] : oc;
+#pragma unroll
+      for (int c = 0; c < CI; ++c) ot = (c == ch) ? o[CI + c] : ot;
+      const bool mine = ch < C, first = ch < CI;
+      const float vch = (a.vin && mine) ? a.vin[(size_t)q * C + ch] : 0.0f;
+      float y = vch;
+      if (first) {
+        const float log_s = tanhf(oc);
+        if (a.log_s_out && live) { a.log_s_out[(size_t)q * CI + ch] = log_s; a.t_out[(size_t)q * CI + ch] = ot; }
+        if (a.o_save && live) a.o_save[(size_t)q * CI + ch] = oc;
+        if (a.vin) {
+          const float sc = expf(log_s);
+          y = a.inverse ? (vch - ot) / sc : sc * vch + ot;
+        }
+        if (live) ls_sum += log_s;
+      }
+      bad |= mine && (not_finite(oc) | not_finite(y));
+      yo[e] = y;
+    }
+    if (bad && live && a.flag) *a.flag = 1;
+    if (a.out) {
+      float z[CPL];
+      const int lane0 = (int)(threadIdx.x & 63) & ~15;
+      if (a.A) {
+#pragma unroll
+        for (int e = 0; e < CPL; ++e) z[e] = (r4 + 16 * e < C) ? a.b[r4 + 16 * e] : 0.0f;
+#pragma unroll
+        for (int ci = 0; ci < C; ++ci) {
+          const float yc = __shfl(yo[ci / 16], lane0 + (ci & 15), 64);
+#pragma unroll
+          for (int e = 0; e < CPL; ++e)
+            if (r4 + 16 * e < C) z[e] = fmaf(yc, a.A[ci * C + r4 + 16 * e], z[e]);
+        }
+      } else {
+#pragma unroll
+        for (int e = 0; e < CPL; ++e) z[e] = yo[e];
+      }
+      if (live) {
+        float* dst = a.out + (size_t)q * a.out_stride + a.out_off;
+#pragma unroll
+        for (int e = 0; e < CPL; ++e)
+          if (r4 + 16 * e < C) dst[r4 + 16 * e] = z[e];
+      }
+    }
+    return ls_sum;
+  }
+  if (r4 != 0 || !live) return 0.0f;
+  if (a.flag) {
+    bool bad = false;
+#pragma unroll
+    for (int c = 0; c < C; ++c) bad |= not_finite(o[c]);
+    if (bad) *a.flag = 1;
+  }
+  if (a.o_save) {
+#pragma unroll
+    for (int k = 0; k < CI; ++k) a.o_save[(size_t)q * CI + k] = o[k];
+  }
+  if (a.vin) {
+#pragma unroll
+    for (int c = 0; c < C; ++c) v[c] = a.vin[(size_t)q * C + c];
+  }
+  float y[C];
+  float lsum = 0.0f;
+#pragma unroll
+  for (int k = 0; k < CI; ++k) {
+    const float log_s = tanhf(o[k]);
+    const float t = o[CI + k];
+    if (a.log_s_out) { a.log_s_out[(size_t)q * CI + k] = log_s; a.t_out[(size_t)q * CI + k] = t; }
+    if (a.vin) {
+      const float s = expf(log_s);
+      y[k] = a.inverse ? (v[k] - t) / s : s * v[k] + t;
+      y[CI + k] = v[CI + k];
+    }
+    lsum += log_s;
+  }
+  if (a.flag && a.vin) {
+    bool bad = false;
+#pragma unroll
+    for (int c = 0; c < C; ++c) bad |= not_finite(y[c]);
+    if (bad) *a.flag = 1;
+  }
+  if (a.out) {
+    float* dst = a.out + (size_t)q * a.out_stride + a.out_off;
+    if (a.A) {
+      float z[C];
+      affine_cc<C>(a.A, a.b, y, z);
+#pragma unroll
+      for (int c = 0; c < C; ++c) dst[c] = z[c];
+    } else {
+#pragma unroll
+      for (int c = 0; c < C; ++c) dst[c] = y[c];
+    }
+  }
+  return lsum;
+}
diff --git a/audiosourcesep_amd/csrc/glowk_engine.h b/audiosourcesep_amd/csrc/glowk_engine.h
--- a/audiosourcesep_amd/csrc/glowk_engine.h
+++ b/audiosourcesep_amd/csrc/glowk_engine.h
@@ -103,6 +103,7 @@
   int64_t range_fallbacks = 0;
   int64_t family_launches[FAM_COUNT] = {};
   int64_t fused_steps = 0;
+  int64_t coupled_tail_steps = 0;
   DeviceMem<int> d_flag;
   PinnedMem<int> h_flag;
   DeviceMem<unsigned> d_probe;
diff --git a/audiosourcesep_amd/csrc/glowk_kernels.h b/audiosourcesep_amd/csrc/glowk_kernels.h
--- a/audiosourcesep_amd/csrc/glowk_kernels.h
+++ b/audiosourcesep_amd/csrc/glowk_kernels.h
@@ -1,5 +1,6 @@
 #pragma once
 #include "glowk_act_scale.h"
+#include "glowk_couple.h"
 
 #include <hip/hip_runtime.h>
 #include <utility>
@@ -11,6 +12,8 @@
 #define GLOWK_LPTR(p) ((__attribute__((address_space(3))) void*)(p))
 
 __device__ __forceinline__ int mfma_row(int r, int hh) { return (r & 3) + 8 * (r >> 2) + 4 * hh; }
+
+enum { NET_ASK_FUSE = 1, NET_ASK_TAIL = 2 };
 
 struct NetArgs {
   const float* vin;
@@ -59,16 +62,6 @@
   }
 }
 
-template <int C>
-__device__ __forceinline__ void affine_cc(const float* __restrict__ A, const float* __restrict__ b, const float (&x)[C], float (&y)[C]) {
-#pragma unroll
-  for (int co = 0; co < C; ++co) y[co] = b[co];
-#pragma unroll
-  for (int ci = 0; ci < C; ++ci)
-#pragma unroll
-    for (int co = 0; co < C; ++co) y[co] = fmaf(x[ci], A[ci * C + co], y[co]);
-}
-
 __device__ __forceinline__ void glds16(const float4* src_lane, float4* lds_wave_base) {
   __builtin_amdgcn_global_load_lds(GLOWK_GPTR(src_lane), GLOWK_LPTR(lds_wave_base), 16, 0, 0);
 }
@@ -124,6 +117,7 @@
 constexpr int NET_STORE = 8;
 constexpr int NET_FUSE = 16;
 constexpr int NET_HALF = 32;
+constexpr int NET_TAIL = 64;
 template <int MODE>
 constexpr int net_dir = MODE & 7;
 
@@ -905,6 +899,7 @@
 struct RingS {
   static constexpr bool BWD = net_dir<MODE> == NET_BWD;
   static constexpr bool FUSE = (MODE & NET_FUSE) != 0;
+  static constexpr bool TAIL = (MODE & NET_TAIL) != 0;
   static constexpr int PXH = (MODE & NET_HALF) ? 1 : 2;
   static constexpr int NFH = NF / NP;
   static constexpr int NRB = 2 * NFH;
@@ -930,7 +925,9 @@
   static constexpr size_t LDS_BYTES = (size_t)3 * MAIN4 * 16 + (size_t)2 * K14 * 16 + (size_t)EPN * 4 + MASK2B;
   static constexpr bool FITS = LDS_BYTES <= 160 * 1024 && NF % 4 == 0 && NFH >= 2 && KS <= (PXH == 1 ? (NP == 2 ? 5 : 9) : NP == 2 ? 3 : 5) && NGRP <= 3 &&
                                (NGRP == 1 || GT % TPC == 0) &&
-                               (!FUSE || (MOUT == 36 && NP == 2 && PXH == 2 && LDS_BYTES + (size_t)36 * FUSE_PSTR * 4 + 4096 + 128 <= 160 * 1024));
+                               (!FUSE || (MOUT == 36 && NP == 2 && PXH == 2 && LDS_BYTES + (size_t)36 * FUSE_PSTR * 4 + 4096 + 128 <= 160 * 1024)) &&
+                               (!TAIL || (MODE == (NET_FWD | NET_TAIL) || MODE == (NET_FWD2 | NET_TAIL)) && NP == 2 && PXH == 2 &&
+                                             ((KIN == 4 && MOUT == 72) || (KIN == 8 && MOUT == 144)));
   static constexpr int K1TOT4 = NF * K14;
   static constexpr int IMGH = NF / 2;
   static constexpr int IMG_MAIN4 = IMGH * 256;
@@ -1336,6 +1333,44 @@
   }
 }
 
+template <int C>
+__device__ __forceinline__ void coupled_tail(double* red , int tid) {
+  typedef const __attribute__((address_space(4))) NetArgs* KernArgs;
+  unsigned long long kp = (unsigned long long)__builtin_amdgcn_kernarg_segment_ptr();
+  asm volatile("" : "+s"(kp));
+  const KernArgs a = (KernArgs)kp;
+  CoupleArgs ca;
+  ca.vin = a->vin; ca.P = a->P; ca.np = 2; ca.pstride = a->pstride; ca.b3 = a->fz_b3; ca.A = a->fz_A; ca.b = a->fz_b;
+  ca.out = a->fz_out; ca.out_stride = a->fz_out_stride; ca.out_off = a->fz_out_off;
+  ca.logdet = a->fz_ldpart; ca.log_s_out = nullptr; ca.t_out = nullptr; ca.o_save = nullptr;
+  ca.Q = a->Q; ca.h = a->h; ca.w = a->w; ca.inverse = a->fz_inverse; ca.flag = a->flag;
+  const int hw = ca.h * ca.w;
+  const int q0 = (int)blockIdx.x * 256 + tid;
+  const bool live = tid < 256 && q0 < ca.Q;
+  float lsum = 0.0f;
+  if (tid < 256) {
+    const int q = q0 < ca.Q ? q0 : ca.Q - 1;
+    const int pp = q % hw;
+    lsum = couple_pixel<C, 1>(ca, q, pp / ca.w, pp % ca.w, live, 0);
+  }
+  if (!ca.logdet) return;
+  double d = (double)lsum;
+  const int gs = hw < 64 ? hw : 64;
+  for (int o = gs >> 1; o > 0; o >>= 1) d += __shfl_down(d, o, 64);
+  if (hw <= 64) {
+    if (live && (tid & (gs - 1)) == 0) ca.logdet[q0 / hw] += 0.0 + d;
+    return;
+  }
+  if ((tid & 63) == 0 && tid < 256) red[tid >> 6] = d;
+  __syncthreads();
+  const int wps = hw >> 6;
+  if (tid < 256 / hw && (int)blockIdx.x * 256 + tid * hw < ca.Q) {
+    double t = 0.0;
+    for (int w = 0; w < wps; ++w) t += red[tid * wps + w];
+    ca.logdet[((int)blockIdx.x * 256 + tid * hw) / hw] += t;
+  }
+}
+
 template <int KIN, int MOUT, int NF, int MODE, int NP, bool SPLIT>
 __global__ __launch_bounds__(512, 2) void k_net_h3s(NetArgs a) {
   using G = RingS<KIN, MOUT, NF, MODE, NP>;
@@ -1352,6 +1387,8 @@
   __shared__ __attribute__((aligned(16))) unsigned short mkl[G::MASK2B / 2 + 8];
   __shared__ float plds[G::FUSE ? 36 * FUSE_PSTR : 1];
   __shared__ float4 vstash[G::FUSE ? 256 : 1];
+  __shared__ double tail_red[G::TAIL ? 4 : 1];
+  static_assert(!G::TAIL || !SPLIT, "the coupling tail needs both passes in one workgroup");
   static_assert(!G::FUSE || (G::MERGE && !SPLIT && MOUT == 36), "the fused coupling needs both passes in one workgroup and a 4-channel level");
   static_assert(!(MODE & NET_STORE) || G::PXH == 1, "hidden stores (training): half-wave form only -- with two pixel halves a wave whose second half lies "
                                             "beyond Q would issue fewer stores than h3_x_end's counted wait assumes");
@@ -1462,4 +1499,9 @@
     __syncthreads();
     fused_couple(a, plds, vstash, tid);
   }
-}
+  if constexpr (G::TAIL) {
+    asm volatile("s_waitcnt vmcnt(0)" ::: "memory");
+    __syncthreads();
+    coupled_tail<2 * KIN>(tail_red, wave * 64 + (int)__builtin_amdgcn_mbcnt_hi(~0u, __builtin_amdgcn_mbcnt_lo(~0u, 0u)));
+  }
+}
diff --git a/audiosourcesep_amd/csrc/glowk_launch.h b/audiosourcesep_amd/csrc/glowk_launch.h
--- a/audiosourcesep_amd/csrc/glowk_launch.h
+++ b/audiosourcesep_amd/csrc/glowk_launch.h
@@ -21,6 +21,7 @@
   bool q = false;
   int fused_px = 0;
   bool failed = false;
+  bool tail = false;
   explicit operator bool() const { return np > 0 || fused_px > 0; }
 };
 
@@ -107,17 +108,25 @@
   }
   if constexpr (F2) {
     const bool split = 2 * wgs <= cus;
+    if constexpr ((MODE == NET_FWD || MODE == NET_FWD2) && RingS<KIN, MOUT, NF, MODE | NET_TAIL, 2>::FITS) {
+      if (a.fuse == NET_ASK_TAIL && !split) {
+        if (!dry) hipLaunchKernelGGL((k_net_h3s<KIN, MOUT, NF, MODE | NET_TAIL, 2, false>), dim3(wgs), dim3(512), 0, s, a);
+        NetLaunch r{2, FAM_H3S};
+        r.tail = true;
+        return r;
+      }
+    }
     if constexpr (RingC<KIN, MOUT, NF, MODE>::FITS) {
       const int wgc = (a.Q + CO_PX - 1) / CO_PX;
       const bool co_ok = a.co && !env().co_off;
       if (co_ok && wgc > cus) {
         if constexpr (RingC<KIN, MOUT, NF, MODE | NET_FUSE>::FITS) {
-          if (a.fuse && co_two_per_cu(k_net_h3c<KIN, MOUT, NF, MODE | NET_FUSE, false>)) {
+          if (a.fuse == NET_ASK_FUSE && co_two_per_cu(k_net_h3c<KIN, MOUT, NF, MODE | NET_FUSE, false>)) {
             if (!dry) hipLaunchKernelGGL((k_net_h3c<KIN, MOUT, NF, MODE | NET_FUSE, false>), dim3(wgc), dim3(256), 0, s, a);
             return {0, FAM_FUSED, true, false, CO_PX};
           }
         }
-        if (!a.fuse && co_two_per_cu(k_net_h3c<KIN, MOUT, NF, MODE, false>)) {
+        if (a.fuse != NET_ASK_FUSE && co_two_per_cu(k_net_h3c<KIN, MOUT, NF, MODE, false>)) {
           if (!dry) hipLaunchKernelGGL((k_net_h3c<KIN, MOUT, NF, MODE, false>), dim3(wgc), dim3(256), 0, s, a);
           return {RingC<KIN, MOUT, NF, MODE>::MERGE ? 1 : 2, FAM_H3S, true};
         }
@@ -129,7 +138,7 @@
     }
     if constexpr ((MODE == NET_FWD || MODE == NET_FWD2 || MODE == NET_FWD_SAVE) && MOUT == 36) {
       if constexpr (RingS<KIN, MOUT, NF, MODE | NET_FUSE, 2>::FITS && RingS<KIN, MOUT, NF, MODE | NET_FUSE, 2>::MERGE) {
-        if (a.fuse && !split) {
+        if (a.fuse == NET_ASK_FUSE && !split) {
           if (!dry) hipLaunchKernelGGL((k_net_h3s<KIN, MOUT, NF, MODE | NET_FUSE, 2, false>), dim3(wgs), dim3(512), 0, s, a);
           return {0, FAM_FUSED, false, false, 256};
         }
diff --git a/audiosourcesep_amd/csrc/glowk_light.h b/audiosourcesep_amd/csrc/glowk_light.h
--- a/audiosourcesep_amd/csrc/glowk_light.h
+++ b/audiosourcesep_amd/csrc/glowk_light.h
@@ -112,174 +112,6 @@
     const double tot = block_sum_256((double)ld, red);
     if (threadIdx.x == 0) logdet[n] = (float)(ld_const + tot);
   }
-}
-
-struct CoupleArgs {
-  const float* vin;
-  const float* P;
-  int np;
-  size_t pstride;
-  const float* b3;
-  const float* A;
-  const float* b;
-  float* out;
-  int out_stride, out_off;
-  double* logdet;
-  float* log_s_out;
-  float* t_out;
-  float* o_save;
-  int Q, h, w;
-  int inverse;
-  int* flag;
-};
-
-__device__ __forceinline__ bool not_finite(float v) { return !(fabsf(v) <= 3.0e38f); }
-
-template <int C, int LPP>
-__device__ __forceinline__ float couple_pixel(const CoupleArgs& a, int q, int i, int j, bool live, int r4) {
-  constexpr int CI = C / 2;
-  constexpr bool QUAD = LPP == 4;
-  float v[C], o[C];
-#pragma unroll
-  for (int c = 0; c < C; ++c) o[c] = 0.0f;
-  if constexpr (LPP == 16) {
-    for (int idx = r4; idx < 9 * a.np; idx += 16) {
-      const int tap = idx / a.np, part = idx % a.np;
-      const int dy = tap / 3 - 1, dx = tap % 3 - 1;
-      const int ii = i + dy, jj = j + dx;
-      if (ii >= 0 && ii < a.h && jj >= 0 && jj < a.w) {
-        const float* src = a.P + (size_t)part * a.pstride + (size_t)(tap * C) * a.Q + (q + dy * a.w + dx);
-#pragma unroll
-        for (int c = 0; c < C; ++c) o[c] += src[(size_t)c * a.Q];
-      }
-    }
-  } else {
-#pragma unroll
-  for (int u = 0; u < (QUAD ? 3 : 9); ++u) {
-    const int tap = QUAD ? r4 + 4 * u : u;
-    const int dy = tap / 3 - 1, dx = tap % 3 - 1;
-    const int ii = i + dy, jj = j + dx;
-    if (tap < 9 && ii >= 0 && ii < a.h && jj >= 0 && jj < a.w) {
-      const size_t off = (size_t)(tap * C) * a.Q + (q + dy * a.w + dx);
-#pragma unroll
-      for (int part = 0; part < 4; ++part)
-        if (part < a.np) {
-          const float* src = a.P + (size_t)part * a.pstride + off;
-#pragma unroll
-          for (int c = 0; c < C; ++c) o[c] += src[(size_t)c * a.Q];
-        }
-    }
-  }
-  }
-#pragma unroll
-  for (int c = 0; c < C; ++c) {
-#pragma unroll
-    for (int m = 1; m < LPP; m <<= 1) o[c] += __shfl_xor(o[c], m, 64);
-    o[c] += a.b3[c];
-  }
-  if constexpr (LPP == 16) {
-    constexpr int CPL = (C + 15) / 16;
-    float yo[CPL], ls_sum = 0.0f;
-    bool bad = false;
-#pragma unroll
-    for (int e = 0; e < CPL; ++e) {
-      const int ch = r4 + 16 * e;
-      float oc = 0.0f, ot = 0.0f;
-#pragma unroll
-      for (int c = 0; c < C; ++c) oc = (c == ch) ? o[c] : oc;
-#pragma unroll
-      for (int c = 0; c < CI; ++c) ot = (c == ch) ? o[CI + c] : ot;
-      const bool mine = ch < C, first = ch < CI;
-      const float vch = (a.vin && mine) ? a.vin[(size_t)q * C + ch] : 0.0f;
-      float y = vch;
-      if (first) {
-        const float log_s = tanhf(oc);
-        if (a.log_s_out && live) { a.log_s_out[(size_t)q * CI + ch] = log_s; a.t_out[(size_t)q * CI + ch] = ot; }
-        if (a.o_save && live) a.o_save[(size_t)q * CI + ch] = oc;
-        if (a.vin) {
-          const float sc = expf(log_s);
-          y = a.inverse ? (vch - ot) / sc : sc * vch + ot;
-        }
-        if (live) ls_sum += log_s;
-      }
-      bad |= mine && (not_finite(oc) | not_finite(y));
-      yo[e] = y;
-    }
-    if (bad && live && a.flag) *a.flag = 1;
-    if (a.out) {
-      float z[CPL];
-      const int lane0 = (int)(threadIdx.x & 63) & ~15;
-      if (a.A) {
-#pragma unroll
-        for (int e = 0; e < CPL; ++e) z[e] = (r4 + 16 * e < C) ? a.b[r4 + 16 * e] : 0.0f;
-#pragma unroll
-        for (int ci = 0; ci < C; ++ci) {
-          const float yc = __shfl(yo[ci / 16], lane0 + (ci & 15), 64);
-#pragma unroll
-          for (int e = 0; e < CPL; ++e)
-            if (r4 + 16 * e < C) z[e] = fmaf(yc, a.A[ci * C + r4 + 16 * e], z[e]);
-        }
-      } else {
-#pragma unroll
-        for (int e = 0; e < CPL; ++e) z[e] = yo[e];
-      }
-      if (live) {
-        float* dst = a.out + (size_t)q * a.out_stride + a.out_off;
-#pragma unroll
-        for (int e = 0; e < CPL; ++e)
-          if (r4 + 16 * e < C) dst[r4 + 16 * e] = z[e];
-      }
-    }
-    return ls_sum;
-  }
-  if (r4 != 0 || !live) return 0.0f;
-  if (a.flag) {
-    bool bad = false;
-#pragma unroll
-    for (int c = 0; c < C; ++c) bad |= not_finite(o[c]);
-    if (bad) *a.flag = 1;
-  }
-  if (a.o_save) {
-#pragma unroll
-    for (int k = 0; k < CI; ++k) a.o_save[(size_t)q * CI + k] = o[k];
-  }
-  if (a.vin) {
-#pragma unroll
-    for (int c = 0; c < C; ++c) v[c] = a.vin[(size_t)q * C + c];
-  }
-  float y[C];
-  float lsum = 0.0f;
-#pragma unroll
-  for (int k = 0; k < CI; ++k) {
-    const float log_s = tanhf(o[k]);
-    const float t = o[CI + k];
-    if (a.log_s_out) { a.log_s_out[(size_t)q * CI + k] = log_s; a.t_out[(size_t)q * CI + k] = t; }
-    if (a.vin) {
-      const float s = expf(log_s);
-      y[k] = a.inverse ? (v[k] - t) / s : s * v[k] + t;
-      y[CI + k] = v[CI + k];
-    }
-    lsum += log_s;
-  }
-  if (a.flag && a.vin) {
-    bool bad = false;
-#pragma unroll
-    for (int c = 0; c < C; ++c) bad |= not_finite(y[c]);
-    if (bad) *a.flag = 1;
-  }
-  if (a.out) {
-    float* dst = a.out + (size_t)q * a.out_stride + a.out_off;
-    if (a.A) {
-      float z[C];
-      affine_cc<C>(a.A, a.b, y, z);
-#pragma unroll
-      for (int c = 0; c < C; ++c) dst[c] = z[c];
-    } else {
-#pragma unroll
-      for (int c = 0; c < C; ++c) dst[c] = y[c];
-    }
-  }
-  return lsum;
 }
 
 template <int C, bool QUAD>
diff --git a/audiosourcesep_amd/engine.py b/audiosourcesep_amd/engine.py
--- a/audiosourcesep_amd/engine.py
+++ b/audiosourcesep_amd/engine.py
@@ -195,6 +195,10 @@
     def fused_steps(self):
         return int(self.lib.glowk_fused_steps(self.h))
 
+    @property
+    def coupled_tail_steps(self):
+        return int(self.lib.glowk_coupled_tail_steps(self.h))
+
     def kernel_families(self):
         out = (ctypes.c_int64 * 7)()
         _lib.check(self.lib.glowk_kernel_families(self.h, out))
diff --git a/include/glowk.h b/include/glowk.h
--- a/include/glowk.h
+++ b/include/glowk.h
@@ -101,6 +101,7 @@
 } glowk_profile;
 int glowk_profile_begin(glowk_handle* h);
 int64_t glowk_fused_steps(const glowk_handle* h);
+int64_t glowk_coupled_tail_steps(const glowk_handle* h);
 int glowk_kernel_families(const glowk_handle* h, int64_t* out7);
 int glowk_profile_end(glowk_handle* h, glowk_profile* out);
 
```

After: 16490. 1.0% lower.
